# ArthurBrussee/brush

Measured on AMD Instinct MI355X. Metric: train views/sec @ 1M Gaussians, 1080p (fwd + L1/SSIM loss + bwd + Adam per view), higher is better.
Workload: dtype f32

## Files before the change

brush_amd/csrc/api.hip:

```cpp
#include <cmath>
#include <cstdlib>
#include <cstdio>
#include <algorithm>
#include <cstring>
#include <new>

#include "context.h"
#include "device_rng.h"

namespace bh {

int launch_image_loss_forward_strided(bh_ctx* ctx, const float* pred, uint32_t pix_stride, uint32_t ch_stride, const uint32_t* gt,
                                      uint32_t channels, uint32_t h, uint32_t w, const BhLossConfig& cfg, float* loss_map);
int launch_image_loss_backward_strided(bh_ctx* ctx, const float* pred, uint32_t pix_stride, uint32_t ch_stride, const uint32_t* gt,
                                       const float* dl_dmap, float dl_rgb, float dl_alpha, uint32_t channels, uint32_t h, uint32_t w,
                                       const BhLossConfig& cfg, float* dl_dpred);

int launch_image_loss_fused(bh_ctx* ctx, const float* img_hwc4, const uint32_t* gt, uint32_t h, uint32_t w, const BhLossConfig& cfg,
                            bool alpha_match, float dl_rgb, float dl_alpha, float* loss_out, float* v_output, float* loss_host = nullptr,
                            uint32_t* started_host = nullptr, uint32_t started_tag = 0);
int launch_image_loss_fused_window(bh_ctx* ctx, const float* img_hwc4, const uint32_t* gt, uint32_t h, uint32_t w, const BhLossConfig& cfg,
                                   bool alpha_match, float dl_rgb, float dl_alpha, uint32_t tile_y0, uint32_t tile_y1, float* loss_out,
                                   float* v_output, float* loss_host = nullptr, uint32_t* started_host = nullptr, uint32_t started_tag = 0);

// ... 19 lines not shown
}

static inline void cpu_relax() {
#if defined(__x86_64__) || defined(__i386__)
    __builtin_ia32_pause();
#elif defined(__aarch64__)
    __asm__ __volatile__("yield");
#endif
}
int wait_host_tag(bh_ctx* ctx, const volatile uint32_t* word, uint32_t want, const char* what) {
    for (uint64_t it = 1; it < (1ull << 21); ++it) {
        if (*word == want) return 0;
        if ((it & 0x3FFFull) == 0ull) {
            const hipError_t q = hipStreamQuery(ctx->stream);
            if (q == hipSuccess) break;
            if (q != hipErrorNotReady) return check_hip(ctx, q, what);
        }
        cpu_relax();
    }
    if (*word == want) return 0;
    BH_HIP(ctx, hipEventRecord(ctx->readback_ev, ctx->stream));
    BH_HIP(ctx, hipEventSynchronize(ctx->readback_ev));
    if (*word == want) return 0;
    return set_error(ctx, BH_ERR_STATE, std::string(what) + ": the kernel that signals the host never stored its tag");
}

void* ensure(bh_ctx* ctx, Slot s, size_t bytes) {
    Buffer& b = ctx->slots[s];
    if (bytes == 0) bytes = 16;
    if (b.cap >= bytes) return b.ptr;
    if (b.ptr) {
        (void)hipStreamSynchronize(ctx->stream);
        (void)hipFree(b.ptr);
        b.ptr = nullptr;
        b.cap = 0;
    }
    {
        int best = -1;
        for (size_t i = 0; i < ctx->pool.size(); ++i)
            if (ctx->pool[i].cap >= bytes && ctx->pool[i].cap <= 2 * bytes + 4096 && (best < 0 || ctx->pool[i].cap < ctx->pool[(size_t)best].cap)) best = (int)i;
        if (best >= 0) {
            b = ctx->pool[(size_t)best];
            ctx->pool.erase(ctx->pool.begin() + best);
            return b.ptr;
        }
    }
    size_t cap = bytes + bytes / 4;
    cap = (cap + 255) & ~(size_t)255;
    void* p = nullptr;
    hipError_t e = hipMalloc(&p, cap);
    if (e != hipSuccess) {
        (void)hipGetLastError();
        cap = (bytes + 255) & ~(size_t)255;
        e = hipMalloc(&p, cap);
    }
    if (e != hipSuccess) {
        char msg[160];
        snprintf(msg, sizeof msg, "hipMalloc(%zu bytes) for scratch slot %d failed: %s", cap, (int)s, hipGetErrorString(e));
        (void)hipGetLastError();
        set_error(ctx, BH_ERR_OOM, msg);
        return nullptr;
    }
    b.ptr = p;
    b.cap = cap;
    return p;
}

ViewUniforms make_uniforms(const BhCamera& c) {
    ViewUniforms u;
    for (int i = 0; i < 12; ++i) u.vm[i] = c.vm[i];
    u.fx = c.fx; u.fy = c.fy; u.cx = c.cx; u.cy = c.cy;
    u.lim_pos_x = c.lim_pos_x; u.lim_pos_y = c.lim_pos_y; u.lim_neg_x = c.lim_neg_x; u.lim_neg_y = c.lim_neg_y;
    u.cam_x = c.cam_pos[0]; u.cam_y = c.cam_pos[1]; u.cam_z = c.cam_pos[2];
    u.img_w = c.img_w; u.img_h = c.img_h;
    u.tile_bw = (c.img_w + TILE_WIDTH - 1) / TILE_WIDTH;
    u.tile_bh = (c.img_h + TILE_WIDTH - 1) / TILE_WIDTH;
    const bool whole = c.tile_row_begin == 0 && c.tile_row_end == 0;
    u.tile_y0 = whole ? 0u : c.tile_row_begin;
    u.tile_y1 = whole ? u.tile_bh : c.tile_row_end;
    u.model = c.model;
    for (int i = 0; i < 8; ++i) u.dist[i] = c.dist[i];
    u.half_fov = c.half_max_render_fov;
    return u;
}

static int prof_index(Profiler& p, const char* name) {
    for (int i = 0; i < p.count; ++i)
        if (p.names[i] == name || std::strcmp(p.names[i], name) == 0) return i;
    if (p.count >= MAX_PROF) return -1;
    p.names[p.count] = name;
    p.ms[p.count] = 0.0f;
    p.calls[p.count] = 0;
    return p.count++;
}
static hipEvent_t prof_event(Profiler& p) {
    if (!p.pool.empty()) {
        hipEvent_t e = p.pool.back();
        p.pool.pop_back();
        return e;
    }
    hipEvent_t e = nullptr;
    (void)hipEventCreate(&e);
    return e;
}
static void prof_resolve(bh_ctx* ctx) {
    Profiler& p = ctx->prof;
    for (auto& pe : p.pending) {
        (void)hipEventSynchronize(pe.b);
        float ms = 0.0f;
        if (hipEventElapsedTime(&ms, pe.a, pe.b) == hipSuccess && pe.idx >= 0) {
            p.ms[pe.idx] += ms;
            p.calls[pe.idx] += 1;
        }
        p.pool.push_back(pe.a);
        p.pool.push_back(pe.b);
    }
    p.pending.clear();
}

ProfScope::ProfScope(bh_ctx* c, const char* name, bool dominant) : ctx(c) {
    if (c->prof.level == 0 || (c->prof.level == 2 && !dominant)) return;
    idx = prof_index(c->prof, name);
    a = prof_event(c->prof);
    b = prof_event(c->prof);
    if (c->prof.level == 2) {
        c->prof.ext_a = a;
        c->prof.ext_b = b;
        return;
    }
    (void)hipEventRecord(a, c->stream);
}
ProfScope::~ProfScope() {
    if (!a) return;
    if (ctx->prof.level == 2) {
        const bool used = ctx->prof.ext_a == nullptr;
        ctx->prof.ext_a = ctx->prof.ext_b = nullptr;
        if (!used) {
            ctx->prof.pool.push_back(a);
            ctx->prof.pool.push_back(b);
            return;
        }
    } else {
        (void)hipEventRecord(b, ctx->stream);
    }
    ctx->prof.pending.push_back({idx, a, b});
}


}

using namespace bh;

extern "C" {

const char* bh_version(void) { return "brush_hip 0.1 (gfx950)"; }

uint32_t bh_abi_version(void) { return BH_ABI_VERSION; }

uint32_t bh_struct_size(uint32_t which) {
    switch (which) {
        case BH_STRUCT_CAMERA: return (uint32_t)sizeof(BhCamera);
        case BH_STRUCT_RENDER_OUT: return (uint32_t)sizeof(BhRenderOut);
        case BH_STRUCT_LOSS_CONFIG: return (uint32_t)sizeof(BhLossConfig);
        case BH_STRUCT_TRAIN_CONFIG: return (uint32_t)sizeof(BhTrainConfig);
        case BH_STRUCT_TRAIN_STATE: return (uint32_t)sizeof(BhTrainState);
        case BH_STRUCT_TRAIN_BATCH: return (uint32_t)sizeof(BhTrainBatch);
        case BH_STRUCT_TRAIN_STATS: return (uint32_t)sizeof(BhTrainStats);
        case BH_STRUCT_REFINE_CONFIG: return (uint32_t)sizeof(BhRefineConfig);
        case BH_STRUCT_REFINE_STATS: return (uint32_t)sizeof(BhRefineStats);
        case BH_STRUCT_PLY_INFO: return (uint32_t)sizeof(BhPlyInfo);
        default: return 0u;
    }
}

bh_ctx* bh_create(int device, void* stream, int own_stream) {
    bh_ctx* ctx = new (std::nothrow) bh_ctx();
    if (!ctx) return nullptr;
    ctx->device = device;
    if (hipSetDevice(device) != hipSuccess) {
        (void)hipGetLastError();
        delete ctx;
        return nullptr;
    }
    if (!own_stream) {
        ctx->stream = (hipStream_t)stream;
        ctx->owns_stream = false;
    } else {
        if (hipStreamCreateWithFlags(&ctx->stream, hipStreamNonBlocking) != hipSuccess) {
            (void)hipGetLastError();
            delete ctx;
            return nullptr;
        }
        ctx->owns_stream = true;
    }
    if (hipHostMalloc((void**)&ctx->host_counters, bh::HOST_COUNTERS_BYTES, hipHostMallocCoherent)    != hipSuccess) {
        (void)hipGetLastError();
        if (ctx->owns_stream) (void)hipStreamDestroy(ctx->stream);
        delete ctx;
        return nullptr;
    }
    std::memset(ctx->host_counters, 0, bh::HOST_COUNTERS_BYTES);
#ifdef BH_TEST_HOOKS
    ctx->knob_break_allreduce = getenv("BH_BREAK_ALLREDUCE") != nullptr;
    if (ctx->knob_break_allreduce)
        fprintf(stderr, "brush_hip: BH_BREAK_ALLREDUCE is set - every all-reduce of this context's communicator is deliberately CORRUPTED (test hook)\n");
    if (const char* e = getenv("BH_TEST_FAIL_LOSS_AT")) {
        ctx->knob_fail_loss_at = (uint32_t)atoi(e);
        if (ctx->knob_fail_loss_at) fprintf(stderr, "brush_hip: BH_TEST_FAIL_LOSS_AT=%u - that train step of this context will FAIL on purpose (test hook)\n", ctx->knob_fail_loss_at);
    }
#endif
    if (hipEventCreateWithFlags(&ctx->readback_ev, hipEventDisableTiming) != hipSuccess ||
        hipEventCreateWithFlags(&ctx->gate_ev, hipEventDisableTiming) != hipSuccess) {
        if (ctx->readback_ev) (void)hipEventDestroy(ctx->readback_ev);
        (void)hipGetLastError();
        (void)hipHostFree(ctx->host_counters);
        if (ctx->owns_stream) (void)hipStreamDestroy(ctx->stream);
        delete ctx;
        return nullptr;
    }
    return ctx;
}

void bh_destroy(bh_ctx* ctx) {
    if (!ctx) return;
    (void)hipSetDevice(ctx->device);
    (void)hipStreamSynchronize(ctx->stream);
    prof_resolve(ctx);
    for (hipEvent_t e : ctx->prof.pool) (void)hipEventDestroy(e);
    for (auto& b : ctx->slots)
        if (b.ptr) (void)hipFree(b.ptr);
    for (auto& kv : ctx->views)
        if (kv.second.zcut) (void)hipFree(kv.second.zcut);
    for (auto& rt : ctx->retained)
        for (auto& b : rt.blocks)
            if (b.ptr) (void)hipFree(b.ptr);
    for (auto& b : ctx->pool)
        if (b.ptr) (void)hipFree(b.ptr);
    if (ctx->host_counters) (void)hipHostFree(ctx->host_counters);
    if (ctx->dsort_spl) (void)hipFree(ctx->dsort_spl);
    if (ctx->readback_ev) (void)hipEventDestroy(ctx->readback_ev);
    if (ctx->gate_ev) (void)hipEventDestroy(ctx->gate_ev);
    if (ctx->image_tab_host) (void)hipHostFree(ctx->image_tab_host);
    if (ctx->image_tab_ev) (void)hipEventDestroy(ctx->image_tab_ev);
    if (ctx->comm) (void)bh_comm_destroy(ctx);
    if (ctx->owns_stream) (void)hipStreamDestroy(ctx->stream);
    delete ctx;
}

const char* bh_last_error(bh_ctx* ctx) { return ctx ? ctx->last_error.c_str() : "null context"; }

int bh_sync(bh_ctx* ctx) {
    if (!ctx) return BH_ERR_INVALID_ARG;
    if (ctx->far_job.pending) {
        BH_HIP(ctx, hipSetDevice(ctx->device));
        BH_TRY(finish_far_slice(ctx, nullptr));
    }
    BH_HIP(ctx, hipStreamSynchronize(ctx->stream));
    deliver_pending_loss(ctx);
    return 0;
}

int bh_profile_enable(bh_ctx* ctx, int on) {
    if (!ctx) return BH_ERR_INVALID_ARG;
    ctx->prof.level = on < 0 ? 0 : (on > 2 ? 1 : on);
    return 0;
}

int bh_profile_fetch(bh_ctx* ctx, const char** names, float* ms, uint32_t* calls, int cap) {
    if (!ctx) return BH_ERR_INVALID_ARG;
    prof_resolve(ctx);
    Profiler& p = ctx->prof;
    const int n = p.count < cap ? p.count : cap;
    for (int i = 0; i < n; ++i) {
        names[i] = p.names[i];
        ms[i] = p.ms[i];
        calls[i] = p.calls[i];
    }
    p.count = 0;
    return n;
}

namespace {
struct OptionKey { const char* name; const char* help; };
const OptionKey kOptionKeys[] = {
    {"cut_min_pairs", "u32: a view whose last frame had fewer pairs keeps complete lists (= bh_set_list_cut_threshold)"},
    {"cut_margin_pct", "0..10000: base margin behind a tile's last useful splat, % of its depth rank (default 150)"},
    {"cut_margin_fixed", "0|1: the margin is cut_margin_pct for every frame instead of adaptive"},
    {"cut_ctrl", "up:down:floor:gap_exp — the margin controller's constants (default 1.5:0.998:0.5:0.3333)"},
    {"cut_sort_all", "0|1: with per-tile cuts, still depth-sort every visible splat"},
    {"auto_exact_share", "0..1: a view whose last cut frame listed more than this share of its pairs renders complete lists (default 0.9; 0 = never)"},
    {"no_view_hash", "0|1: frames without a view id share ONE table instead of being keyed by their camera"},
    {"k16_order", "0 index order | 1 by the view's last per-tile work | 2 dealt: the forward blend's tile order"},
    {"band_mode", "0|1: XCD bands of the blend kernels — contiguous eighths of the tile range, or dealt in chunks of 8 adjacent tiles (default 1)"},
    {"k16_waves", "0..8: forward blend: resident one-wave tiles per SIMD (0 = 8 = all resident at once; fewer: the lighter tiles are dispatched as the heavier ones finish)"},
    {"k16_split", "0..1000: forward blend: a tile whose forecast work is at least max(256, k16_split / 100 x its band's mean) is blended by four quadrant waves (default 250; 0: no tile is split)"},
    {"k16_split_of_max", "0..100: ... and at least this many percent of its band's heaviest tile (default 45)"},
    {"k16_split_min", "1..1023: a tile below this many blended splats (forecast) is never split (default 256)"},
    {"k5_exact_spw", "16|32|64: splats per wave of the list builder for complete lists"},
    {"bwd_jobs", "0|1: the blend backward works on checkpointed 128-entry segments of the tiles' lists (default 1) or on whole tiles"},
    {"no_lpt", "0|1: the blend backward takes its tiles in index order"},
    {"lpt_classes", "log|linear: work classes of the backward's longest-first tile order — two per octave of blended splats, or 1/64 of the mean list length wide"},
    {"generic_depth_sort", "0|1: depth order by the generic radix sort + scan instead of the fused split sort"},
    {"dsort_splitters", "0|1: the fused depth sort splits at the 254 depth quantiles of the view's previous frame (default 1) or always linearly over the frame's key range"},
    {"tile_sort", "auto|bucket|lsd: the forward's tile sort (auto: bucket sort unless the view's pairs are concentrated in few tiles)"},
    {"spec_k5", "0|1: queue the list builder before the host has read the frame's counts (default 1; 0: behind the count readback)"},
    {"event_waits", "0|1: the host's mid-step waits use events behind the kernels instead of polled tag words"},
    {"readback_copy", "0|1: counts and gate word reach the host through copy launches"},
    {"force_exchange", "0|1: a one-rank communicator still walks the whole gradient-exchange path (overhead measurement)"},
    {"zero_grads", "0|1: the single-GPU train step zero-fills its gradient span like the exchange path"},
    {"loss_bands", "0|1: the fused loss's blocks take their tiles by XCD column bands (1) or row-major (0)"},
    {"update_rows", "0|64|128|256: splats per block of the update kernel (0 = default)"},
    {"update_early", "0|1: the update kernel's blocks issue all their loads up front"},
    {"no_dormant", "0|1: the update kernel fetches and updates dormant splats like everyone else"},
    {"sort_kpt", "0|4|8|16: keys per thread of the generic radix sort (0 = default)"},
    {"grad_allreduce", "ring|direct: the dense gradient block's collective — ncclAllReduce, or reduce-scatter + all-gather over grouped send/recv"},
};
bool parse_u32(const char* v, uint32_t lo, uint32_t hi, uint32_t* out) {
    if (!v || !*v) return false;
    char* end = nullptr;
    const unsigned long long x = strtoull(v, &end, 10);
    if (*end != '\0' || x < lo || x > hi) return false;
    *out = (uint32_t)x;
    return true;
}
bool parse_flag(const char* v, bool* out) {
    uint32_t x = 0;
    if (!parse_u32(v, 0, 1, &x)) return false;
    *out = x != 0;
    return true;
}
}

extern "C" int bh_option_count(void) { return (int)(sizeof(kOptionKeys) / sizeof(kOptionKeys[0])); }
extern "C" const char* bh_option_name(int i) { return i >= 0 && i < bh_option_count() ? kOptionKeys[i].name : nullptr; }
extern "C" const char* bh_option_help(int i) { return i >= 0 && i < bh_option_count() ? kOptionKeys[i].help : nullptr; }

extern "C" int bh_set_option(bh_ctx* ctx, const char* key, const char* value) {
    if (!ctx) return BH_ERR_INVALID_ARG;
    if (!key || !value) return set_error(ctx, BH_ERR_INVALID_ARG, "set_option: null key or value");
    const std::string k(key);
    bool ok = false;
    uint32_t u = 0;
    if (k == "cut_min_pairs") { if ((ok = parse_u32(value, 0, 0xFFFFFFFFu, &u))) ctx->cut_min_pairs = u; }
    else if (k == "cut_margin_pct") { if ((ok = parse_u32(value, 0, 10000, &u))) ctx->knob_cut_margin_pct = u; }
    else if (k == "cut_margin_fixed") ok = parse_flag(value, &ctx->knob_fixed_margin);
    else if (k == "cut_ctrl") {
        float a = 0, b = 0, c = 0, d = 0;
        if (sscanf(value, "%f:%f:%f:%f", &a, &b, &c, &d) == 4 && a >= 1.0f && b > 0.0f && b <= 1.0f && c > 0.0f && d >= 0.0f && d <= 1.0f) {
            ctx->ctrl_up = a; ctx->ctrl_down = b; ctx->ctrl_floor = c; ctx->ctrl_gap_exp = d;
            ok = true;
        }
    }
    else if (k == "cut_sort_all") ok = parse_flag(value, &ctx->knob_cut_sort_all);
    else if (k == "auto_exact_share") {
        char* end = nullptr;
        const float f = strtof(value, &end);
        if (end != value && *end == '\0' && f >= 0.0f && f <= 1.0f) { ctx->auto_exact_share = f; ok = true; }
    }
    else if (k == "no_view_hash") ok = parse_flag(value, &ctx->knob_no_view_hash);
    else if (k == "k16_order") { if ((ok = parse_u32(value, 0, 2, &u))) ctx->knob_k16_order = u; }
    else if (k == "band_mode") { if ((ok = parse_u32(value, 0, 1, &u))) ctx->knob_band_mode = u; }
    else if (k == "k16_waves") { if ((ok = parse_u32(value, 0, 8, &u))) ctx->knob_k16_waves = u; }
    else if (k == "k16_split") { if ((ok = parse_u32(value, 0, 1000, &u))) ctx->knob_k16_split = u; }
    else if (k == "k16_split_of_max") { if ((ok = parse_u32(value, 0, 100, &u))) ctx->knob_k16_split_of_max = u; }
    else if (k == "k16_split_min") { if ((ok = parse_u32(value, 1, 1023, &u))) ctx->knob_k16_split_min = u; }
    else if (k == "k5_exact_spw") { if ((ok = parse_u32(value, 16, 64, &u) && (u == 16 || u == 32 || u == 64))) ctx->knob_k5_exact_spw = u; }
    else if (k == "bwd_jobs") ok = parse_flag(value, &ctx->knob_bwd_jobs);
    else if (k == "no_lpt") ok = parse_flag(value, &ctx->knob_no_lpt);
    else if (k == "lpt_classes") {
        const std::string v(value);
        if (v == "log") { ctx->knob_lpt_linear = false; ok = true; }
        else if (v == "linear") { ctx->knob_lpt_linear = true; ok = true; }
    }
    else if (k == "generic_depth_sort") ok = parse_flag(value, &ctx->knob_generic_depth_sort);
    else if (k == "dsort_splitters") ok = parse_flag(value, &ctx->knob_dsort_splitters);
    else if (k == "tile_sort") {
        const std::string v(value);
        if (v == "auto") { ctx->knob_tile_sort = 0; ok = true; }
        else if (v == "bucket") { ctx->knob_tile_sort = 1; ok = true; }
        else if (v == "lsd") { ctx->knob_tile_sort = 2; ok = true; }
    }
    else if (k == "spec_k5") ok = parse_flag(value, &ctx->knob_spec_k5);
    else if (k == "event_waits") ok = parse_flag(value, &ctx->knob_event_waits);
    else if (k == "readback_copy") ok = parse_flag(value, &ctx->knob_readback_copy);
    else if (k == "force_exchange") ok = parse_flag(value, &ctx->knob_force_exchange);
    else if (k == "zero_grads") ok = parse_flag(value, &ctx->knob_zero_grads);
    else if (k == "loss_bands") { if ((ok = parse_u32(value, 0, 1, &u))) ctx->knob_loss_bands = u; }
    else if (k == "update_rows") { if ((ok = parse_u32(value, 0, 256, &u) && (u == 0 || u == 64 || u == 128 || u == 256))) ctx->knob_update_rows = u; }
    else if (k == "update_early") ok = parse_flag(value, &ctx->knob_update_early);
    else if (k == "no_dormant") ok = parse_flag(value, &ctx->knob_no_dormant);
    else if (k == "sort_kpt") { if ((ok = parse_u32(value, 0, 16, &u) && (u == 0 || u == 4 || u == 8 || u == 16))) ctx->knob_sort_kpt = u; }
    else if (k == "grad_allreduce") {
        const std::string v(value);
        if (v == "ring") { ctx->knob_direct_allreduce = false; ok = true; }
        else if (v == "direct") { ctx->knob_direct_allreduce = true; ok = true; }
    }
    else return set_error(ctx, BH_ERR_INVALID_ARG, "set_option: unknown key '" + k + "' (bh_option_name lists the keys)");
    if (!ok) return set_error(ctx, BH_ERR_INVALID_ARG, "set_option: bad value '" + std::string(value) + "' for '" + k + "'");
    return 0;
}

namespace {
struct Kb4Law {
    double k[4];
    explicit Kb4Law(const float* d) { for (int i = 0; i < 4; ++i) k[i] = d ? (double)d[i] : 0.0; }
    double value(double th) const {
        const double t2 = th * th, t3 = t2 * th, t5 = t3 * t2, t7 = t5 * t2, t9 = t7 * t2;
        return th + k[0] * t3 + k[1] * t5 + k[2] * t7 + k[3] * t9;
    }
    double slope(double th) const {
        const double t2 = th * th, t4 = t2 * t2, t6 = t4 * t2, t8 = t6 * t2;
        return 1.0 + 3.0 * k[0] * t2 + 5.0 * k[1] * t4 + 7.0 * k[2] * t6 + 9.0 * k[3] * t8;
    }
    double invert(double target) const {
        if (target <= 0.0) return 0.0;
        const double pi = 3.14159265358979323846;
        double th = target < pi - 1e-6 ? target : pi - 1e-6;
        for (int it = 0; it < 50; ++it) {
            const double fp = slope(th);
            if (std::fabs(fp) < 1e-12) break;
            double next = th - (value(th) - target) / fp;
            next = next < 0.0 ? 0.0 : (next > pi ? pi : next);
            const bool done = std::fabs(next - th) < 1e-12;
            th = next;
            if (done) break;
        }
        return th;
    }
};
struct Rt8Law {
    double k[6];
    explicit Rt8Law(const float* d) { for (int i = 0; i < 6; ++i) k[i] = d ? (double)d[i] : 0.0; }
    double radial(double r) const {
        const double r2 = r * r, r4 = r2 * r2, r6 = r4 * r2;
        return (1.0 + k[0] * r2 + k[1] * r4 + k[2] * r6) / (1.0 + k[3] * r2 + k[4] * r4 + k[5] * r6);
    }
    double undistort(double r_d) const {
        double r = r_d;
        for (int it = 0; it < 30; ++it) {
            const double f = radial(r);
            if (std::fabs(f) < 1e-12) break;
            const double rn = r_d / f;
            const bool done = std::fabs(rn - r) < 1e-12;
            r = rn;
            if (done) break;
        }
        return r;
    }
};
}

double bh_fov_to_focal(double fov, uint32_t pixels, uint32_t model, const float* dist) {
    const double half = fov / 2.0, r_pix = (double)pixels / 2.0;
    switch (model) {
        case BH_CAMERA_PINHOLE: return r_pix / std::tan(half);
        case BH_CAMERA_KANNALA_BRANDT_4:
        case BH_CAMERA_THIN_PRISM_FISHEYE: return r_pix / Kb4Law(dist).value(half);
        case BH_CAMERA_RADIAL_TANGENTIAL_8: { const double r = std::tan(half); return r_pix / (r * Rt8Law(dist).radial(r)); }
        default: return std::nan("");
    }
}

double bh_focal_to_fov(double focal, uint32_t pixels, uint32_t model, const float* dist) {
    const double r_norm = ((double)pixels / 2.0) / focal;
    switch (model) {
        case BH_CAMERA_PINHOLE: return 2.0 * std::atan(r_norm);
        case BH_CAMERA_KANNALA_BRANDT_4:
        case BH_CAMERA_THIN_PRISM_FISHEYE: return 2.0 * Kb4Law(dist).invert(r_norm);
        case BH_CAMERA_RADIAL_TANGENTIAL_8: return 2.0 * std::atan(Rt8Law(dist).undistort(r_norm));
        default: return std::nan("");
    }
}

int bh_camera_setup_model(const float* pos, const float* rot_xyzw, double fov_x, double fov_y, float center_u, float center_v,
                          uint32_t img_w, uint32_t img_h, uint32_t model, const float* dist, BhCamera* out) {
    if (!pos || !rot_xyzw || !out || img_w == 0 || img_h == 0 || model > BH_CAMERA_THIN_PRISM_FISHEYE) return BH_ERR_INVALID_ARG;
    const float x = rot_xyzw[0], y = rot_xyzw[1], z = rot_xyzw[2], w = rot_xyzw[3];
    const float x2 = x + x, y2 = y + y, z2 = z + z;
    const float xx = x * x2, xy = x * y2, xz = x * z2;
    const float yy = y * y2, yz = y * z2, zz = z * z2;
    const float wx = w * x2, wy = w * y2, wz = w * z2;
    const float ax[3] = {1.0f - (yy + zz), xy + wz, xz - wy};
    const float ay[3] = {xy - wz, 1.0f - (xx + zz), yz + wx};
    const float az[3] = {xz + wy, yz - wx, 1.0f - (xx + yy)};
    auto cross = [](const float* a, const float* b, float* o) {
        o[0] = a[1] * b[2] - b[1] * a[2];
        o[1] = a[2] * b[0] - b[2] * a[0];
        o[2] = a[0] * b[1] - b[0] * a[1];
    };
    float t0[3], t1[3], t2[3];
    cross(ay, az, t0);
    cross(az, ax, t1);
    cross(ax, ay, t2);
    const float det = (az[0] * t2[0]) + (az[1] * t2[1]) + (az[2] * t2[2]);
    const float inv_det = 1.0f / det;
    float r0[3], r1[3], r2[3];
    for (int i = 0; i < 3; ++i) { r0[i] = t0[i] * inv_det; r1[i] = t1[i] * inv_det; r2[i] = t2[i] * inv_det; }
    const float c0[3] = {r0[0], r1[0], r2[0]}, c1[3] = {r0[1], r1[1], r2[1]}, c2[3] = {r0[2], r1[2], r2[2]};
    for (int i = 0; i < 3; ++i) {
        out->vm[i] = c0[i];
        out->vm[3 + i] = c1[i];
        out->vm[6 + i] = c2[i];
        const float ip = (c0[i] * pos[0] + c1[i] * pos[1]) + c2[i] * pos[2];
        out->vm[9 + i] = -ip;
    }
    out->model = model;
    for (int i = 0; i < 8; ++i) out->dist[i] = (model != BH_CAMERA_PINHOLE && dist) ? dist[i] : 0.0f;
    out->fx = (float)bh_fov_to_focal(fov_x, img_w, model, out->dist);
    out->fy = (float)bh_fov_to_focal(fov_y, img_h, model, out->dist);
    out->cx = center_u * (float)img_w;
    out->cy = center_v * (float)img_h;
    const float wf = (float)img_w, hf = (float)img_h;
    float lim[4] = {(1.15f * wf - out->cx) / out->fx, (1.15f * hf - out->cy) / out->fy,
                    (-0.15f * wf - out->cx) / out->fx, (-0.15f * hf - out->cy) / out->fy};
    if (model == BH_CAMERA_RADIAL_TANGENTIAL_8) {
        const Rt8Law law(out->dist);
        for (float& e : lim) {
            const float mag = (float)law.undistort(std::fabs((double)e));
            e = (e != e) ? e : (std::signbit(e) ? -mag : mag);
        }
    } else if (model != BH_CAMERA_PINHOLE) {
        for (float& e : lim) e = 0.0f;
    }
    out->lim_pos_x = lim[0]; out->lim_pos_y = lim[1]; out->lim_neg_x = lim[2]; out->lim_neg_y = lim[3];
    const float full = hypotf((float)fov_x, (float)fov_y) * 1.05f;
    const float cap = 2.0f * 3.14159265358979323846f - 1e-6f;
    out->half_max_render_fov = (full < cap ? full : cap) * 0.5f;
    out->cam_pos[0] = pos[0]; out->cam_pos[1] = pos[1]; out->cam_pos[2] = pos[2];
    out->img_w = img_w;
    out->img_h = img_h;
    out->tile_row_begin = 0;
    out->tile_row_end = 0;
    return 0;
}

int bh_camera_setup(const float* pos, const float* rot_xyzw, double fov_x, double fov_y, float center_u, float center_v,
                    uint32_t img_w, uint32_t img_h, BhCamera* out) {
    return bh_camera_setup_model(pos, rot_xyzw, fov_x, fov_y, center_u, center_v, img_w, img_h, BH_CAMERA_PINHOLE, nullptr, out);
}

}

static int render_forward(bh_ctx* ctx, const ForwardRequest& req, BhRenderOut* out) {
    const BhCamera& cam = req.cam;
    if (cam.img_w == 0 || cam.img_h == 0) return set_error(ctx, BH_ERR_INVALID_ARG, "Can't render images with 0 size.");
    if (req.sh_degree > 4) return set_error(ctx, BH_ERR_INVALID_ARG, "sh_degree must be 0..4");
    if (cam.model > BH_CAMERA_THIN_PRISM_FISHEYE) return set_error(ctx, BH_ERR_INVALID_ARG, "unknown camera model");
    if (cam.img_w > 65520 || cam.img_h > 65520) return set_error(ctx, BH_ERR_UNSUPPORTED, "images larger than 65520 px per side are not supported (tile grid <= 4095 x 4095)");
    if (req.n > 0 && (!req.transforms || !req.sh_coeffs || !req.raw_opacities)) return set_error(ctx, BH_ERR_INVALID_ARG, "render_forward: null splat tensor");
    if ((req.flags & BH_FLAG_SMOOTH_CUTOFF) && !(req.flags & BH_FLAG_BWD_INFO)) return set_error(ctx, BH_ERR_INVALID_ARG, "smooth cutoff requires the backward pass flag");
    BH_HIP(ctx, hipSetDevice(ctx->device));
    if (ctx->far_job.pending) BH_TRY(finish_far_slice(ctx, nullptr));
    return forward_impl(ctx, req, out);
}

extern "C" int bh_render_forward(bh_ctx* ctx, const BhCamera* cam, uint32_t n, uint32_t sh_degree, const float* transforms,
                                 const float* sh_coeffs, const float* raw_opacities, const float* background, uint32_t flags,
                                 BhRenderOut* out) {
    if (!ctx) return BH_ERR_INVALID_ARG;
    if (!cam || !out || !background) return set_error(ctx, BH_ERR_INVALID_ARG, "render_forward: null argument");
    ForwardRequest req;
    req.cam = *cam;
    req.n = n; req.sh_degree = sh_degree; req.flags = flags;
    req.transforms = transforms; req.sh_coeffs = sh_coeffs; req.raw_opacities = raw_opacities;
    req.bg[0] = background[0]; req.bg[1] = background[1]; req.bg[2] = background[2];
    req.view_id = ctx->view_id;
    return render_forward(ctx, req, out);
}

int bh::forward_impl(bh_ctx* ctx, const ForwardRequest& req, BhRenderOut* out) {
    const uint32_t n = req.n, sh_degree = req.sh_degree, flags = req.flags;
    const float* transforms = req.transforms;
    const float* sh_coeffs = req.sh_coeffs;
    const float* raw_opacities = req.raw_opacities;
    const float* background = req.bg;
    ctx->have_forward = false;
    ctx->clears.begin_forward();
    const bool mip = flags & BH_FLAG_MIP, bwd_info = flags & BH_FLAG_BWD_INFO, smooth = flags & BH_FLAG_SMOOTH_CUTOFF;
    const ViewUniforms u = make_uniforms(req.cam);
    if (u.tile_y0 >= u.tile_y1 || u.tile_y1 > u.tile_bh) return set_error(ctx, BH_ERR_INVALID_ARG, "tile_row window must satisfy begin < end <= ceil(img_h / 16)");
    const uint32_t num_tiles = u.tile_bw * u.tile_bh;
    const size_t npad = n ? n : 1;

    constexpr size_t counter_set_bytes = COUNTER_SET_BYTES, counter_set_words = COUNTER_SET_BYTES / 4, counter_read_bytes = COUNTER_READ_BYTES;
    auto* counter_pairs = (uint32_t*)ensure(ctx, SLOT_COUNTERS, 2 * counter_set_bytes + 64);
    uint32_t* dev_sums = counter_pairs ? counter_pairs + 2 * counter_set_words : nullptr;
    uint32_t* counters = counter_pairs ? counter_pairs + counter_set_words * (ctx->counter_phase & 1u) : nullptr;
    auto* depth_keys = (uint32_t*)ensure(ctx, SLOT_DEPTH_KEYS, npad * 4);
    auto* isect_counts = (uint32_t*)ensure(ctx, SLOT_ISECT_COUNTS, npad * 4);
    auto* max_radius = req.max_radius ? req.max_radius : (float*)ensure(ctx, SLOT_MAX_RADIUS, npad * 4);
    auto* proj_by_gid = (float*)ensure(ctx, SLOT_PROJECTED_BY_GID, npad * 9 * 4);
    if (!counters || !depth_keys || !isect_counts || !max_radius || !proj_by_gid) return BH_ERR_OOM;

    auto* gfc = (uint32_t*)ensure(ctx, SLOT_GLOBAL_FROM_COMPACT, npad * 4);
    auto* depths_sorted = (uint32_t*)ensure(ctx, SLOT_DEPTHS_SORTED, npad * 4);
    if (!gfc || !depths_sorted) return BH_ERR_OOM;
    const bool bwd_jobs = bwd_info && ctx->knob_bwd_jobs && !ctx->knob_no_lpt && !((flags & BH_FLAG_SLICED_LISTS) && ctx->slice_fraction > 0.0f);
    const size_t lpt_words = LPT_HEADER_WORDS + (size_t)8 * LPT_CLASSES * band_slots(num_tiles);
    auto* tile_offsets = (uint32_t*)ensure(ctx, SLOT_TILE_OFFSETS, ((size_t)num_tiles * 2 + lpt_words) * 4);
    auto* visible = (bwd_info && req.visible) ? req.visible : (float*)ensure(ctx, SLOT_VISIBLE, (bwd_info ? npad : 1) * 4);
    if (!tile_offsets || !visible) return BH_ERR_OOM;
    const size_t visible_words = bwd_info ? ((req.visible && req.visible_floats) ? req.visible_floats : npad) : 0;
    const bool want_sliced = (flags & BH_FLAG_SLICED_LISTS) != 0;
    const size_t slice_bit_words = ((size_t)num_tiles + 31) / 32;
    const size_t slice_group_words = (size_t)n / (256 * FAR_GROUP_BLOCKS) + 2;
    const size_t slice_words = want_sliced ? SLICE_CTRL_WORDS + slice_bit_words + (size_t)num_tiles * 2 + slice_group_words : 0;
    uint32_t* slice_tab = nullptr;
    if (want_sliced) {
        slice_tab = (uint32_t*)ensure(ctx, SLOT_SLICE, slice_words * 4);
        if (!slice_tab) return BH_ERR_OOM;
    }
    ViewState* view = nullptr;
    bool cut_active = false;
    const bool auto_cuts = want_sliced && !(ctx->slice_fraction > 0.0f);
    const bool order_only = !want_sliced && ctx->knob_k16_order != 0u && n >= 8u * 256u;
    if (n > 0 && (auto_cuts || order_only)) {
        view = frame_view(ctx, req, u.tile_bw, u.tile_bh, order_only && !bwd_info);
        if (!view && auto_cuts) return set_error(ctx, BH_ERR_OOM, "hipMalloc for the per-view tile table failed");
        if (!view) (void)hipGetLastError();
        cut_active = auto_cuts && view && cut_this_frame(ctx, view, req.allow_cut);
    }
    uint32_t* const vtab = view_table(view);
    uint32_t* near_counts = nullptr;
    uint32_t* tile_order = nullptr;
    uint32_t* tile_split = nullptr;
    if (cut_active) {
        near_counts = (uint32_t*)ensure(ctx, SLOT_NEAR_COUNTS, npad * 4);
        if (!near_counts) return BH_ERR_OOM;
    }

    uint32_t nv = 0, ni = 0, near_total = 0, nv_true = 0;
    bool fused_scan = false;
    uint32_t* cum_early = nullptr;
    bool k5_queued = false;
    uint32_t spec_pair_cap = 0;
    float* spec_projected = nullptr;
    float4* spec_vc = nullptr;
    uint32_t *spec_tile_ids = nullptr, *spec_isect_gids = nullptr;
    if (n > 0) {
        {
            ProfScope ps(ctx, "ProjectSplats");
            if (!ctx->counters_ready) BH_HIP(ctx, hipMemsetAsync(counter_pairs, 0, 2 * counter_set_bytes, ctx->stream));
            ctx->counters_ready = false;
            ForwardPrep prep;
            prep.next_counters = reinterpret_cast<unsigned long long*>(counter_pairs + counter_set_words * ((ctx->counter_phase & 1u) ^ 1u));
            prep.visible = visible_words ? reinterpret_cast<uint32_t*>(visible) : nullptr;
            prep.visible_words = (uint32_t)visible_words;
            prep.tile_table = tile_offsets;
            prep.tile_words = num_tiles * 2 + LPT_HEADER_WORDS;
            prep.slice_table = slice_tab;
            prep.slice_words = (uint32_t)slice_words;
            prep.list_all_visible = ctx->knob_cut_sort_all;
            if (view && ctx->knob_k16_order && n >= 8u * 256u) {
                const uint32_t win_t = u.tile_bw * (u.tile_y1 - u.tile_y0);
                tile_order = (uint32_t*)ensure(ctx, SLOT_TILE_ORDER, ((size_t)8 * band_slots(win_t) + SPLIT_TAIL_WORDS) * 4);
                if (!tile_order) return BH_ERR_OOM;
                prep.order_work = vtab + (size_t)num_tiles;
                prep.order_out = tile_order;
                prep.order_tiles = win_t;
                prep.order_tile_begin = u.tile_bw * u.tile_y0;
                prep.order_mode = ctx->knob_k16_order;
                prep.band_mode = ctx->knob_band_mode;
                if (ctx->knob_k16_split && ctx->knob_k16_order == 1u) {
                    tile_split = tile_order + (size_t)8 * band_slots(win_t);
                    prep.split_out = tile_split;
                    prep.split_factor = (float)ctx->knob_k16_split * 0.01f;
                    prep.split_min = ctx->knob_k16_split_min;
                    prep.split_of_max = (float)ctx->knob_k16_split_of_max * 0.01f;
                }
            }
            if (bwd_info && req.grad_begin && req.grad_floats && (req.grad_floats & 3u) == 0 &&
                (reinterpret_cast<uintptr_t>(req.grad_begin) & 15u) == 0 && req.grad_floats / 4 <= 0xFFFFFFFFull) {
                prep.span = reinterpret_cast<float4*>(req.grad_begin);
                prep.span_f4 = (uint32_t)(req.grad_floats / 4);
                ctx->clears.k1_cleared_span();
            }
            BH_TRY(launch_project_forward(ctx, u, n, mip, sh_degree, transforms, sh_coeffs, raw_opacities, depth_keys, isect_counts, max_radius,
                                          proj_by_gid, counters, prep, cut_active ? vtab : nullptr, near_counts));
            ctx->counter_phase ^= 1u;
            ctx->counters_ready = true;
        }
        auto* hslots = reinterpret_cast<unsigned long long*>(ctx->host_counters + 16);
        fused_scan = depth_sort_supported(n) && !ctx->knob_generic_depth_sort;
        const bool sums_on_device = fused_scan && !ctx->knob_readback_copy;
        const bool poll_tag = sums_on_device && !ctx->knob_event_waits;
        if (!sums_on_device) {
            BH_HIP(ctx, hipMemcpyAsync(hslots, counters, counter_read_bytes, hipMemcpyDeviceToHost, ctx->stream));
            BH_HIP(ctx, hipEventRecord(ctx->readback_ev, ctx->stream));
        }
        {
            ProfScope ps(ctx, "DepthSort");
            if (fused_scan) {
                cum_early = (uint32_t*)ensure(ctx, SLOT_CUM_TILES_HIT, npad * 4);
                if (!cum_early) return BH_ERR_OOM;
                if (poll_tag && ++ctx->readback_tag == 0u) ctx->readback_tag = 1u;
                bool* spl_written = nullptr;
                uint32_t* spl = view_splitters(view, cut_active, &spl_written);
                BH_TRY(depth_sort_scan(ctx, depth_keys, counters + COUNTER_MINMAX_WORD, cut_active ? near_counts : isect_counts, n, depths_sorted, gfc, cum_early,
                                       sums_on_device ? counters : nullptr, ctx->host_counters + 16, ctx->readback_ev, poll_tag ? ctx->readback_tag : 0u,
                                       sums_on_device ? dev_sums : nullptr, spl, spl_written));
            } else {
                BH_TRY(radix_argsort(ctx, depth_keys, nullptr, n, 32, depths_sorted, gfc));
            }
        }
        if (poll_tag && ctx->knob_spec_k5 && !(want_sliced && ctx->slice_fraction > 0.0f)) {
            const size_t cap_pairs = std::min(ctx->slots[SLOT_TILE_IDS].cap, ctx->slots[SLOT_ISECT_GIDS].cap) / 4;
            if (cap_pairs >= 4096) {
                spec_projected = (float*)ensure(ctx, SLOT_PROJECTED, npad * 9 * 4);
                spec_vc = bwd_info ? (float4*)ensure(ctx, SLOT_V_COMBINED, npad * 10 * 4 + 16) : nullptr;
                if (!spec_projected || (bwd_info && !spec_vc)) return BH_ERR_OOM;
                spec_tile_ids = (uint32_t*)ctx->slots[SLOT_TILE_IDS].ptr;
                spec_isect_gids = (uint32_t*)ctx->slots[SLOT_ISECT_GIDS].ptr;
                spec_pair_cap = (uint32_t)std::min<size_t>(cap_pairs, 0xFFFFFFFEull);
                ProfScope ps(ctx, "MapGaussiansToIntersect");
                BH_TRY(launch_map_gaussians(ctx, n, u, proj_by_gid, gfc, spec_projected, cum_early, spec_tile_ids, spec_isect_gids, spec_vc,
                                            spec_vc ? (uint32_t)(((size_t)n * 10 + 3) / 4) : 0u, 0xFFFFFFFFu, cut_active ? slice_tab : nullptr,
                                            cut_active ? vtab : nullptr, cut_active ? depths_sorted : nullptr, dev_sums + (cut_active ? 3 : 0), spec_pair_cap));
                k5_queued = true;
            }
        }
        if (poll_tag) BH_TRY(wait_host_tag(ctx, reinterpret_cast<const volatile uint32_t*>(hslots) + HOST_SUM_WORDS - 1u, ctx->readback_tag, "count readback"));
        else BH_HIP(ctx, hipEventSynchronize(ctx->readback_ev));
        if (ctx->gate_learn) {
            ctx->gate_learn = false;
            ctx->far_direct = reinterpret_cast<const volatile uint32_t*>(ctx->host_counters)[HOST_GATE_WORD] != 0u;
        }
        unsigned long long hc[4] = {0ull, 0ull, 0ull, 0ull};
        if (sums_on_device) {
            const volatile unsigned long long* hs = hslots;
            for (uint32_t c = 0; c < COUNTER_K1_U64; ++c) hc[c] = hs[c];
        } else {
            for (uint32_t k = 0; k < COUNTER_SLOTS; ++k)
                for (uint32_t c = 0; c < COUNTER_K1_U64; ++c) hc[c] += hslots[COUNTER_K1_U64 * k + c];
        }
        if (hc[1] > 0xFFFFFFFFull) return set_error(ctx, BH_ERR_UNSUPPORTED, "more than 2^32-1 tile intersections");
        nv_true = (uint32_t)hc[0];
        ni = (uint32_t)hc[1];
        near_total = cut_active ? (uint32_t)hc[2] : ni;
        nv = cut_active ? (uint32_t)hc[3] : nv_true;
    } else {
        BH_HIP(ctx, hipMemsetAsync(tile_offsets, 0, ((size_t)num_tiles * 2 + LPT_HEADER_WORDS) * 4, ctx->stream));
        if (visible_words) BH_HIP(ctx, hipMemsetAsync(visible, 0, visible_words * 4, ctx->stream));
    }

    const size_t nvpad = nv ? nv : 1, nipad = ni ? ni : 1;
    auto* cum = fused_scan ? cum_early : (uint32_t*)ensure(ctx, SLOT_CUM_TILES_HIT, nvpad * 4);
    auto* projected = (float*)ensure(ctx, SLOT_PROJECTED, nvpad * 9 * 4);
    auto* tile_ids = (uint32_t*)ensure(ctx, SLOT_TILE_IDS, nipad * 4);
    auto* isect_gids = (uint32_t*)ensure(ctx, SLOT_ISECT_GIDS, nipad * 4);
    auto* tile_ids_sorted = (uint32_t*)ensure(ctx, SLOT_TILE_IDS_SORTED, nipad * 4);
    auto* isect_gids_sorted = (uint32_t*)ensure(ctx, SLOT_ISECT_GIDS_SORTED, nipad * 4);
    const size_t pixels = (size_t)u.img_w * u.img_h;
    void* out_img = ensure(ctx, SLOT_OUT_IMG, pixels * (bwd_info ? 16 : 4));
    if (!cum || !projected || !tile_ids || !isect_gids || !tile_ids_sorted || !isect_gids_sorted || !out_img)
        return BH_ERR_OOM;
    if (k5_queued && ((cut_active ? near_total : ni) > spec_pair_cap || projected != spec_projected || tile_ids != spec_tile_ids || isect_gids != spec_isect_gids))
        k5_queued = false;

    const uint32_t budget = want_sliced && ni > 0 ? list_budget(ctx, cut_active ? view : nullptr, near_total, ni) : ni;
    const bool sliced = budget < ni;
    const bool by_cut = cut_active && sliced;
    const uint32_t* zcut_lists = cut_active ? vtab : nullptr;
    uint32_t* slice_info = slice_tab;
    uint32_t* done_bits = slice_tab ? slice_tab + SLICE_CTRL_WORDS : nullptr;
    uint32_t* tile_offsets_far = slice_tab ? slice_tab + SLICE_CTRL_WORDS + slice_bit_words : nullptr;
    uint32_t* far_group_totals = slice_tab ? slice_tab + SLICE_CTRL_WORDS + slice_bit_words + (size_t)num_tiles * 2 : nullptr;
    uint32_t tile_bits = 0;
    while (tile_bits < 32 && (num_tiles >> tile_bits) != 0) tile_bits++;
    RasterSlice rs;
    ctx->jobs = BwdJobs{};
    if (bwd_jobs) {
        const uint32_t listed = cut_active ? near_total : ni;
        const uint32_t ckpt_cap = (uint32_t)std::min<uint64_t>((uint64_t)listed / BWD_SEG + num_tiles + 1u, BWD_CKPT_MAX_SLOTS);
        rs.jobs.ckpt = (float4*)ensure(ctx, SLOT_BWD_CKPT, (size_t)ckpt_cap * 256 * sizeof(float4));
        rs.jobs.ckpt_cap = ckpt_cap;
        rs.jobs.top_cap = band_slots(num_tiles) + ckpt_cap;
        rs.jobs.top_list = (uint32_t*)ensure(ctx, SLOT_BWD_TOPLIST, (size_t)8 * rs.jobs.top_cap * 4);
        if (!rs.jobs.ckpt || !rs.jobs.top_list) return BH_ERR_OOM;
        ctx->jobs = rs.jobs;
    }
    if (view) {
        rs.zcut = vtab;
        rs.depth_keys_sorted = depths_sorted;
        rs.nv = nv;
        rs.cut_active = by_cut;
        rs.margin_pct = cut_margin_pct(ctx, view);
        rs.work = vtab + (size_t)num_tiles;
        rs.order = tile_order;
        rs.order_mode = ctx->knob_k16_order;
        rs.split = tile_split;
#ifdef BH_TEST_HOOKS
        ctx->last_split = tile_split;
#endif
    }
    const uint32_t win_tiles = u.tile_bw * (u.tile_y1 - u.tile_y0);
    const float class_width_raw = (float)ni / (float)(win_tiles ? win_tiles : 1u) / 64.0f;
    const float class_width = ctx->knob_lpt_linear ? (class_width_raw < 8.0f ? 8.0f : class_width_raw) : 0.0f;
    ctx->lpt = (bwd_info && !ctx->knob_no_lpt) ? tile_offsets + (size_t)num_tiles * 2 : nullptr;
    float* out_f32 = bwd_info ? (float*)out_img : nullptr;
    uint32_t* out_u8 = bwd_info ? nullptr : (uint32_t*)out_img;

    bool offsets_done = false;
    if (nv > 0) {
        if (!fused_scan) {
            ProfScope ps(ctx, "PrefixSumGaussHits");
            BH_TRY(prefix_sum(ctx, cut_active ? near_counts : isect_counts, gfc, nv, cum, false));
        }
        if (ni == 0) {
            ProfScope ps(ctx, "ProjectVisible");
            BH_TRY(launch_project_visible(ctx, nv, proj_by_gid, gfc, projected));
        }
        if (ni > 0) {
            {
                ProfScope ps(ctx, "MapGaussiansToIntersect");
                float4* vc = nullptr;
                if (bwd_info) {
                    vc = (float4*)ensure(ctx, SLOT_V_COMBINED, (size_t)nv * 10 * 4 + 16);
                    if (!vc) return BH_ERR_OOM;
                }
                if (zcut_lists && near_total == 0u) {
                } else if (k5_queued && (!bwd_info || vc == spec_vc)) {
                    ctx->clears.k5_cleared_accum(vc != nullptr);
                } else {
                    ctx->clears.k5_cleared_accum(vc != nullptr);
                    BH_TRY(launch_map_gaussians(ctx, nv, u, proj_by_gid, gfc, projected, cum, tile_ids, isect_gids, vc, vc ? (uint32_t)(((size_t)nv * 10 + 3) / 4) : 0u,
                                                (sliced && !by_cut) ? budget : 0xFFFFFFFFu, (sliced || zcut_lists) ? slice_info : nullptr, zcut_lists,
                                                zcut_lists ? depths_sorted : nullptr));
                }
            }
            {
                ProfScope ps(ctx, "TileSort");
                if ((zcut_lists || !sliced) && tile_sort_supported(tile_bits, zcut_lists ? near_total : ni) && !(ctx->knob_tile_sort == 2u)) {
                    BH_TRY(tile_sort_offsets(ctx, tile_ids, isect_gids, zcut_lists ? near_total : ni, tile_bits, num_tiles, tile_ids_sorted, isect_gids_sorted,
                                             tile_offsets, ni));
                    offsets_done = true;
                } else
                if (zcut_lists) BH_TRY(radix_argsort_dev(ctx, tile_ids, isect_gids, near_total, nullptr, nullptr, nullptr, tile_bits, tile_ids_sorted, isect_gids_sorted, ni));
                else if (sliced) BH_TRY(radix_argsort_dev(ctx, tile_ids, isect_gids, budget, slice_info + 1, nullptr, nullptr, tile_bits, tile_ids_sorted, isect_gids_sorted, ni));
                else BH_TRY(radix_argsort(ctx, tile_ids, isect_gids, ni, tile_bits, tile_ids_sorted, isect_gids_sorted));
            }
        }
    }
    if (!offsets_done) {
        ProfScope ps(ctx, "GetTileOffsets");
        if (zcut_lists) BH_TRY(launch_tile_offsets(ctx, tile_ids_sorted, near_total, num_tiles, tile_offsets, true));
        else if (sliced) BH_TRY(launch_tile_offsets_dev(ctx, tile_ids_sorted, budget, slice_info + 1, nullptr, nullptr, num_tiles, tile_offsets));
        else BH_TRY(launch_tile_offsets(ctx, tile_ids_sorted, ni, num_tiles, tile_offsets, true));
    }
    if (!sliced) {
        ProfScope ps(ctx, "Rasterize");
        BH_TRY(launch_rasterize(ctx, u, background, bwd_info, smooth, isect_gids_sorted, tile_offsets, projected, gfc, out_f32, out_u8, visible, ctx->lpt,
                                class_width, 0, &rs));
    } else {
        auto* state = (float*)ensure(ctx, SLOT_SLICE_STATE, pixels * 16);
        auto* far_counts = (uint32_t*)ensure(ctx, SLOT_SLICE_COUNTS, nvpad * 4);
        auto* far_block_totals = (uint32_t*)ensure(ctx, SLOT_SLICE_CUM, (nvpad / 256 + 2) * 4);
        if (!state || !far_counts || !far_block_totals) return BH_ERR_OOM;
        rs.done_bits = done_bits;
        rs.unsat_count = slice_info + 2;
        if (!ctx->knob_readback_copy) {
            rs.gate_host = ctx->host_counters + HOST_GATE_WORD;
            *reinterpret_cast<volatile uint32_t*>(rs.gate_host) = 0u;
        }
        rs.state = state;
        rs.offsets_near = tile_offsets;
        rs.live_bands = slice_info + 4;
        {
            ProfScope ps(ctx, "Rasterize");
            BH_TRY(launch_rasterize(ctx, u, background, bwd_info, smooth, isect_gids_sorted, tile_offsets, projected, gfc, out_f32, out_u8, visible, ctx->lpt,
                                    class_width, 1, &rs));
        }
        FarJob& j = ctx->far_job;
        j.u = u;
        j.bg[0] = background[0]; j.bg[1] = background[1]; j.bg[2] = background[2];
        j.bwd_info = bwd_info; j.smooth = smooth;
        j.nv = nv; j.ni = ni; j.budget = budget; j.num_tiles = num_tiles; j.tile_bits = tile_bits;
        j.proj_by_gid = proj_by_gid; j.gfc = gfc; j.projected = projected; j.cum = cum;
        j.slice_info = slice_info; j.done_bits = done_bits; j.tile_offsets_far = tile_offsets_far;
        j.far_counts = far_counts; j.far_block_totals = far_block_totals; j.far_group_totals = far_group_totals;
        j.tile_ids = tile_ids; j.isect_gids = isect_gids; j.tile_ids_sorted = tile_ids_sorted; j.isect_gids_sorted = isect_gids_sorted;
        j.out_f32 = out_f32; j.out_u8 = out_u8; j.visible = visible; j.lpt = ctx->lpt; j.class_width = class_width; j.rs = rs;
        j.by_cut = by_cut;
        j.view = by_cut ? view : nullptr;
        j.view_shared = req.view_id == 0u && ctx->knob_no_view_hash;
        if (by_cut) j.req = req;
        if (ctx->knob_readback_copy)
            BH_HIP(ctx, hipMemcpyAsync(ctx->host_counters + HOST_GATE_WORD, slice_info + 2, 4, hipMemcpyDeviceToHost, ctx->stream));
        if (ctx->far_direct && !by_cut) {
            BH_TRY(enqueue_far_slice(ctx, j));
            ctx->gate_learn = true;
        } else {
            if (++ctx->gate_tag == 0u) ctx->gate_tag = 1u;
            j.gate_tag = ctx->gate_tag;
            ctx->gate_signal_queued = false;
            j.gate_event_recorded = !(req.defer_decision && !ctx->knob_event_waits && !ctx->knob_readback_copy);
            if (j.gate_event_recorded) BH_HIP(ctx, hipEventRecord(ctx->gate_ev, ctx->stream));
            j.pending = true;
            if (!req.defer_decision) {
                bool again = false;
                BH_TRY(finish_far_slice(ctx, &again));
                if (by_cut && again) {
                    *out = ctx->last;
                    return 0;
                }
            }
        }
    }

    BhRenderOut r{};
    r.num_visible = nv_true;
    r.num_listed_splats = nv;
    r.num_intersections = ni;
    r.num_tiles = num_tiles;
    r.tile_bw = u.tile_bw;
    r.tile_bh = u.tile_bh;
    r.flags = flags;
    r.out_img = bwd_info ? (float*)out_img : nullptr;
    r.out_img_packed = bwd_info ? nullptr : (uint32_t*)out_img;
    r.visible = bwd_info ? visible : nullptr;
    r.max_radius = max_radius;
    r.tile_offsets = tile_offsets;
    r.projected = projected;
    r.compact_gid_from_isect = isect_gids_sorted;
    r.tile_id_from_isect = tile_ids_sorted;
    r.global_from_compact_gid = gfc;
    r.cum_tiles_hit = cum;
    r.intersect_counts = isect_counts;
    r.depths_sorted = (float*)depths_sorted;
    r.tile_offsets_far = sliced ? tile_offsets_far : nullptr;
    r.list_budget = budget;
    r.generation = ++ctx->generation;
    ctx->clears.stamp(r.generation);
    *out = r;
    ctx->last = r;
    ctx->last_listed_splats = nv;
    ctx->cam = req.cam;
    ctx->uniforms = u;
    ctx->n = n;
    ctx->sh_degree = sh_degree;
    ctx->flags = flags;
    ctx->bg[0] = background[0]; ctx->bg[1] = background[1]; ctx->bg[2] = background[2];
    ctx->have_forward = true;
    if (view) view_rendered(view, ni);
    return 0;
}

extern "C" {

int bh_set_list_slicing(bh_ctx* ctx, float near_share) {
    if (!ctx) return BH_ERR_INVALID_ARG;
    if (near_share != near_share || near_share > 1.0f) return set_error(ctx, BH_ERR_INVALID_ARG, "set_list_slicing: the near slice's share must be <= 1 (<= 0: automatic)");
    ctx->slice_fraction = near_share > 0.0f ? near_share : 0.0f;
    return 0;
}

int bh_set_list_cut_threshold(bh_ctx* ctx, uint32_t min_pairs) {
    if (!ctx) return BH_ERR_INVALID_ARG;
    ctx->cut_min_pairs = min_pairs;
    return 0;
}

int bh_set_view_id(bh_ctx* ctx, uint32_t view_id) {
    if (!ctx) return BH_ERR_INVALID_ARG;
    ctx->view_id = view_id;
    return 0;
}

int bh_forget_views(bh_ctx* ctx) {
    if (!ctx) return BH_ERR_INVALID_ARG;
    BH_HIP(ctx, hipSetDevice(ctx->device));
    if (ctx->far_job.pending) BH_TRY(finish_far_slice(ctx, nullptr));
    if (ctx->dsort_spl) { BH_HIP(ctx, hipMemsetAsync(ctx->dsort_spl, 0, DSORT_SPL_STRIDE * 4, ctx->stream)); ctx->dsort_spl_written = false; }
    if (ctx->views.empty()) return 0;
    BH_HIP(ctx, hipStreamSynchronize(ctx->stream));
    deliver_pending_loss(ctx);
    for (auto& kv : ctx->views)
        if (kv.second.zcut) (void)hipFree(kv.second.zcut);
    ctx->views.clear();
    ctx->casual_views = 0;
    for (uint64_t& k : ctx->seen_keys) k = 0ull;
    ctx->far_job.view = nullptr;
    ctx->margin_scale = 1.0f;
    return 0;
}

float bh_last_list_share(bh_ctx* ctx) { return ctx ? ctx->last_slice_share : 0.0f; }
uint32_t bh_far_slices_queued(bh_ctx* ctx) { return ctx ? ctx->far_launches : 0u; }
uint32_t bh_view_table_count(bh_ctx* ctx) { return ctx ? (uint32_t)ctx->views.size() : 0u; }

}

namespace bh {

static ForwardState latest_forward(const bh_ctx* ctx) {
    ForwardState fs;
    fs.out = ctx->last;
    fs.uniforms = ctx->uniforms;
    fs.n = ctx->n; fs.sh_degree = ctx->sh_degree; fs.flags = ctx->flags;
    fs.bg[0] = ctx->bg[0]; fs.bg[1] = ctx->bg[1]; fs.bg[2] = ctx->bg[2];
    fs.lpt = ctx->lpt;
    fs.jobs = ctx->jobs;
    return fs;
}

int backward_impl(bh_ctx* ctx, const ForwardState& fs, const float* v_output, const float* transforms, const float* sh_coeffs,
                  const float* raw_opacities, float* v_transforms, float* v_sh_coeffs, float* v_raw_opacities, float* v_refine_weight,
                  size_t span_floats, bool want_refine, const DepthTerm* depth) {
    const BhRenderOut& r = fs.out;
    const uint32_t n = fs.n, nv = r.num_listed_splats, C = (fs.sh_degree + 1) * (fs.sh_degree + 1);
    const size_t nvpad = nv ? nv : 1;
    auto* v_combined = (float*)ensure(ctx, SLOT_V_COMBINED, nvpad * 10 * 4 + 16);
    if (!v_combined) return BH_ERR_OOM;
    bool row_marks = false;
    {
        ProfScope ps(ctx, "ZeroGradBuffers");
        const bool one_span = n > 0 && span_floats;
        const bool vc_done = ctx->clears.take_accum(r.generation);
        const GradClears::Span span = ctx->clears.take_span(r.generation);
        row_marks = span == GradClears::ROW_MARKS;
        if (row_marks && !one_span) return set_error(ctx, BH_ERR_STATE, "internal: row-marked gradients without the train step's gradient span");
        const bool span_done = one_span && span != GradClears::NONE;
        if (one_span && (span_floats & 3u) == 0 && (reinterpret_cast<uintptr_t>(v_transforms) & 15u) == 0) {
            const size_t na = vc_done ? 0 : (nvpad * 10 + 3) / 4, nb = span_done ? 0 : span_floats / 4;
            if (na + nb) {
                hipLaunchKernelGGL(zero_two_kernel, dim3(2048), dim3(256), 0, ctx->stream, reinterpret_cast<float4*>(v_combined), na,
                                   reinterpret_cast<float4*>(v_transforms), nb);
                BH_LAUNCH_CHECK(ctx, "zero_two_kernel");
            }
        } else {
            if (!vc_done) BH_HIP(ctx, hipMemsetAsync(v_combined, 0, nvpad * 10 * 4, ctx->stream));
            if (n > 0) {
                if (one_span) {
                    BH_HIP(ctx, hipMemsetAsync(v_transforms, 0, span_floats * 4, ctx->stream));
                } else {
                    BH_HIP(ctx, hipMemsetAsync(v_transforms, 0, (size_t)n * 10 * 4, ctx->stream));
                    BH_HIP(ctx, hipMemsetAsync(v_sh_coeffs, 0, (size_t)n * C * 3 * 4, ctx->stream));
                    BH_HIP(ctx, hipMemsetAsync(v_raw_opacities, 0, (size_t)n * 4, ctx->stream));
                    BH_HIP(ctx, hipMemsetAsync(v_refine_weight, 0, (size_t)n * 4, ctx->stream));
                }
            }
        }
    }
// ... 527 lines not shown
```

brush_amd/csrc/context.h:

```cpp
#pragma once
#include <hip/hip_runtime.h>
#include <stdint.h>

#include <memory>
#include <string>
#include <unordered_map>
#include <vector>

#include "../../include/brush_hip.h"
#include "../../include/brush_hip_lpips.h"
#include "../../include/brush_hip_image.h"
#include "device_math.h"

namespace bh {

enum Slot : int {
    SLOT_COUNTERS = 0,
    SLOT_DEPTH_KEYS,
    SLOT_ISECT_COUNTS,
    SLOT_MAX_RADIUS,
    SLOT_SORT_KEYS_A,
    SLOT_SORT_KEYS_B,
    SLOT_SORT_VALS_A,
    SLOT_SORT_VALS_B,
    SLOT_SORT_HIST,
    SLOT_COMM_SCRATCH,
    SLOT_BWD_CKPT,
    SLOT_BWD_TOPLIST,
    SLOT_SORT_PARTS,
    SLOT_SCAN_SUMS,
    SLOT_GLOBAL_FROM_COMPACT,
    SLOT_DEPTHS_SORTED,
    SLOT_CUM_TILES_HIT,
    SLOT_PROJECTED,
    SLOT_TILE_IDS,
    SLOT_ISECT_GIDS,
    SLOT_TILE_IDS_SORTED,
    SLOT_ISECT_GIDS_SORTED,
    SLOT_TILE_OFFSETS,
    SLOT_OUT_IMG,
    SLOT_VISIBLE,
    SLOT_V_COMBINED,
    SLOT_LOSS_PRED,
    SLOT_LOSS_MAP,
    SLOT_LOSS_GRAD,
    SLOT_V_OUTPUT,
    SLOT_GRADS,
    SLOT_STATS,
    SLOT_LOSS_SCALAR,
    SLOT_COL_SCALE,
    SLOT_MISC,
    SLOT_REFINE,
    SLOT_REFINE_BOUNDS,
    SLOT_FOLDED_TRANSFORMS,
    SLOT_FOLDED_RAW_OPAC,
    SLOT_PLY_ROWS,
    SLOT_EXCH_BLOCKS,
    SLOT_EXCH_IDX,
    SLOT_EXCH_COMPACT,
    SLOT_PROJECTED_BY_GID,
    SLOT_SLICE,
    SLOT_SLICE_STATE,
    SLOT_SLICE_COUNTS,
    SLOT_SLICE_CUM,
    SLOT_NEAR_COUNTS,
    SLOT_TILE_ORDER,
    SLOT_LOD_GRADS,
    SLOT_LOD_FOLDED,
    SLOT_LOD_LOSS,
    SLOT_LOD_SORT,
    SLOT_KNN,
    SLOT_EVAL,
    SLOT_LPIPS,
    SLOT_PLY_COMPRESS,
    SLOT_IMAGE,
    SLOT_DEPTH,
    SLOT_COUNT
};

struct Buffer {
    void* ptr = nullptr;
    size_t cap = 0;
};

constexpr int MAX_PROF = 32;

constexpr uint32_t COUNTER_SLOTS = 128;
constexpr uint32_t COUNTER_K1_U64 = 4;
constexpr size_t COUNTER_SET_BYTES = COUNTER_SLOTS * 8 * COUNTER_K1_U64 + COUNTER_SLOTS * 8;
constexpr uint32_t COUNTER_SET_U64 = (uint32_t)(COUNTER_SET_BYTES / 8);
constexpr uint32_t COUNTER_MINMAX_WORD = COUNTER_SLOTS * 2 * COUNTER_K1_U64;
constexpr uint32_t SLICE_CTRL_WORDS = 8;
constexpr uint32_t FAR_GROUP_BLOCKS = 64;
constexpr size_t COUNTER_READ_BYTES = COUNTER_SLOTS * 8 * COUNTER_K1_U64;
constexpr uint32_t HOST_SUM_WORDS = 2 * COUNTER_K1_U64 + 1;
constexpr size_t HOST_LOSS_WORD = 16 + COUNTER_READ_BYTES / 4;
constexpr size_t HOST_GATE_WORD = HOST_LOSS_WORD + 16;
constexpr size_t HOST_GATE_TAG_WORD = HOST_GATE_WORD + 1;
constexpr size_t HOST_COUNTERS_BYTES = 64 + COUNTER_READ_BYTES + 64 + 64;

struct Profiler {
    int level = 0;
    const char* names[MAX_PROF];
    float ms[MAX_PROF];
    uint32_t calls[MAX_PROF];
    int count = 0;
    struct Pending { int idx; hipEvent_t a, b; };
    std::vector<Pending> pending;
    std::vector<hipEvent_t> pool;
    hipEvent_t ext_a = nullptr, ext_b = nullptr;
};

constexpr uint32_t ZCUT_ALL = 0xFFFFFFFEu;
BH_DEV bool zcut_near(uint32_t key, uint32_t cut) { return (key >> 1) <= (cut >> 1); }
struct ViewState {
    uint32_t* zcut = nullptr;
    uint32_t tile_bw = 0, tile_bh = 0;
    bool seeded = false;
    uint32_t exact_frames = 0;
    uint32_t penalty = 0;
    uint64_t last_used = 0;
    uint32_t gap = 0;
    uint32_t last_pairs = 0;
    uint32_t complete_frames = 0;
    bool spl_written[2] = {false, false};
    bool casual = false;
};
constexpr uint32_t CUT_MIN_PAIRS = 1500000u;
constexpr uint32_t LPT_CLASSES = 64;
constexpr uint32_t LPT_HEADER_WORDS = 8 * LPT_CLASSES + 64;
constexpr uint32_t BWD_SEG = 128;
constexpr uint32_t BWD_MAX_SEGS = 64;
struct BwdJobs {
    float4* ckpt = nullptr;
    uint32_t ckpt_cap = 0;
    uint32_t* top_list = nullptr;
    uint32_t top_cap = 0;
};
constexpr uint32_t BAND_CHUNK = 4;
inline __host__ __device__ uint32_t band_slots(uint32_t num_tiles) {
    const uint32_t p = (num_tiles + 7u) / 8u;
    return ((p + BAND_CHUNK - 1u) / BAND_CHUNK) * BAND_CHUNK;
}
inline __host__ __device__ uint32_t band_tile(uint32_t band, uint32_t i, uint32_t per, uint32_t mode) {
    return mode ? ((i / BAND_CHUNK) * 8u + band) * BAND_CHUNK + (i % BAND_CHUNK) : band * per + i;
}
constexpr uint32_t SPLIT_MAX = 128;
constexpr uint32_t SPLIT_MIN_WORK = 256;
constexpr uint32_t SPLIT_TAIL_WORDS = 8u + 8u * SPLIT_MAX * 4u;
constexpr uint32_t BWD_CKPT_MAX_SLOTS = 96u * 1024u;
constexpr uint32_t DSORT_SPL_STRIDE = 260;
constexpr uint32_t VIEW_SPL_WORDS = 2 * DSORT_SPL_STRIDE;
constexpr size_t MAX_VIEW_STATES = 4096;
constexpr uint64_t DIRECT_ALLREDUCE_MIN_FLOATS = 1u << 16;
constexpr uint32_t AUTO_EXACT_FRAMES = 12;
constexpr size_t CASUAL_VIEW_STATES = 32;
constexpr size_t SEEN_KEYS = 64;
constexpr size_t VIEW_TABLE_BYTES = (size_t)256 << 20;

struct RasterSlice {
    uint32_t* done_bits = nullptr;
    uint32_t* unsat_count = nullptr;
    uint32_t* gate_host = nullptr;
    float* state = nullptr;
    const uint32_t* offsets_near = nullptr;
    uint32_t* zcut = nullptr;
    const uint32_t* depth_keys_sorted = nullptr;
    uint32_t nv = 0;
    bool cut_active = false;
    uint32_t* live_bands = nullptr;
    uint32_t* work = nullptr;
    const uint32_t* order = nullptr;
    uint32_t order_mode = 1;
    uint32_t* split = nullptr;
    uint32_t margin_pct = 150;
    BwdJobs jobs{};
};

struct ForwardRequest {
    BhCamera cam{};
    uint32_t n = 0, sh_degree = 0, flags = 0;
    const float* transforms = nullptr;
    const float* sh_coeffs = nullptr;
    const float* raw_opacities = nullptr;
    float bg[3] = {0, 0, 0};
    uint32_t view_id = 0;
    float* visible = nullptr;
    float* max_radius = nullptr;
    size_t visible_floats = 0;
    float* grad_begin = nullptr;
    size_t grad_floats = 0;
    bool defer_decision = false;
    bool allow_cut = true;
};

struct FarJob {
    bool pending = false;
    ViewUniforms u{};
    float bg[3] = {0, 0, 0};
    bool bwd_info = false, smooth = false;
    uint32_t nv = 0, ni = 0, budget = 0, num_tiles = 0, tile_bits = 0;
    const float* proj_by_gid = nullptr;
    const uint32_t* gfc = nullptr;
    float* projected = nullptr;
    const uint32_t* cum = nullptr;
    uint32_t* slice_info = nullptr;
    uint32_t* done_bits = nullptr;
    uint32_t* tile_offsets_far = nullptr;
    uint32_t* far_counts = nullptr;
    uint32_t* far_block_totals = nullptr;
    uint32_t* far_group_totals = nullptr;
    uint32_t* tile_ids = nullptr;
    uint32_t* isect_gids = nullptr;
    uint32_t* tile_ids_sorted = nullptr;
    uint32_t* isect_gids_sorted = nullptr;
    float* out_f32 = nullptr;
    uint32_t* out_u8 = nullptr;
    float* visible = nullptr;
    uint32_t* lpt = nullptr;
    float class_width = 8.0f;
    RasterSlice rs{};
    bool gate_event_recorded = false;
    uint32_t gate_tag = 0;
    bool by_cut = false;
    ViewState* view = nullptr;
    bool view_shared = false;
    ForwardRequest req{};
};

struct GradClears {
    enum Span : uint8_t { NONE = 0, ZEROED, ROW_MARKS };
    Span span = NONE;
    bool accum = false;
    uint64_t generation = 0;
    void begin_forward() { span = NONE; accum = false; generation = 0; }
    void k1_cleared_span() { span = ZEROED; }
    void k5_cleared_accum(bool yes) { accum = yes; }
    void stamp(uint64_t gen) { generation = gen; }
    void mark_rows() { span = ROW_MARKS; }
    bool valid_for(uint64_t gen) const { return generation != 0 && generation == gen; }
    Span take_span(uint64_t gen) { const Span s = valid_for(gen) ? span : NONE; span = NONE; return s; }
    bool take_accum(uint64_t gen) { const bool a = valid_for(gen) && accum; accum = false; return a; }
};

struct ForwardState {
    BhRenderOut out{};
    ViewUniforms uniforms{};
    uint32_t n = 0, sh_degree = 0, flags = 0;
    float bg[3] = {0, 0, 0};
    uint32_t* lpt = nullptr;
    BwdJobs jobs{};
};
constexpr int RETAIN_SLOTS = 14;
struct Retained {
    ForwardState fs;
    Buffer blocks[RETAIN_SLOTS];
};

struct DepthTerm {
    const float* v_depth = nullptr;
    uint32_t mode = 0;
};

}


struct bh_ctx {
    int device = 0;
    hipStream_t stream = nullptr;
    bool owns_stream = false;
    std::string last_error;
    bh::Buffer slots[bh::SLOT_COUNT];
    uint32_t* host_counters = nullptr;
    hipEvent_t readback_ev = nullptr;
    hipEvent_t gate_ev = nullptr;
    bool counters_ready = false;
    uint32_t counter_phase = 0;
    bool have_forward = false;
    BhCamera cam{};
    bh::ViewUniforms uniforms{};
    uint32_t n = 0, sh_degree = 0, flags = 0;
    float bg[3] = {0, 0, 0};
    BhRenderOut last{};
    uint64_t generation = 0;
    std::vector<bh::Retained> retained;
    std::vector<bh::Buffer> pool;
    bh::GradClears clears;
    float* pending_loss_dst = nullptr;
    void* image_tab_host = nullptr;
    size_t image_tab_cap = 0;
    hipEvent_t image_tab_ev = nullptr;
    const bh_lpips* lpips = nullptr;
    float lpips_weight = 0.0f;
    void* comm = nullptr;
    hipStream_t comm_stream = nullptr;
    hipEvent_t comm_ev = nullptr;
    int comm_rank = 0, comm_world = 1;
    uint32_t* lpt = nullptr;
    float slice_fraction = 0.0f;
    float last_slice_share = 1.0f;
    bool far_direct = false;
    uint32_t readback_tag = 0;
    uint32_t gate_tag = 0;
    bool gate_signal_queued = false;
    bool gate_learn = false;
    uint32_t far_launches = 0;
    uint32_t last_listed_splats = 0;
    std::unordered_map<uint64_t, bh::ViewState> views;
    uint64_t seen_keys[bh::SEEN_KEYS] = {};
    uint32_t seen_pos = 0;
    uint32_t casual_views = 0;
    uint32_t view_id = 0;
    uint64_t view_clock = 0;
    float margin_scale = 1.0f;
    float ctrl_up = 1.5f, ctrl_down = 0.998f, ctrl_floor = 0.5f, ctrl_gap_exp = 1.0f / 3.0f;
    uint32_t cut_min_pairs = bh::CUT_MIN_PAIRS;
    bool knob_spec_k5 = true;
    bool knob_event_waits = false;
    bool knob_readback_copy = false;
    bool knob_no_view_hash = false;
    bool knob_fixed_margin = false;
    bool knob_cut_sort_all = false;
    uint32_t knob_band_mode = 1;
    uint32_t knob_k16_waves = 0;
    uint32_t knob_k16_split = 250;
    uint32_t knob_k16_split_min = bh::SPLIT_MIN_WORK;
    uint32_t knob_k16_split_of_max = 45;
    const uint32_t* last_split = nullptr;
    uint32_t knob_k16_order = 1;
    uint32_t knob_cut_margin_pct = 150;
    bh::FarJob far_job;
    uint32_t refine_n = 0, refine_new_n = 0;
    bool dsort_lds_raised = false;
    uint32_t* dsort_spl = nullptr;
    bool dsort_spl_written = false;
    bool knob_dsort_splitters = true;
    bool adam_lds_raised = false;
    bool knob_no_lpt = false;
    bool knob_bwd_jobs = true;
    bh::BwdJobs jobs{};
    bool knob_lpt_linear = false;
    bool knob_force_exchange = false;
    bool knob_break_allreduce = false;
    bool knob_generic_depth_sort = false;
    bool knob_zero_grads = false;
    uint32_t knob_fail_loss_at = 0;
    uint32_t train_steps_seen = 0;
    uint32_t knob_loss_bands = 1;
    uint32_t knob_tile_sort = 0;
    float auto_exact_share = 0.9f;
    bool knob_direct_allreduce = false;
    uint32_t knob_k5_exact_spw = 32;
    bool knob_no_dormant = false;
    bool knob_update_early = false;
    uint32_t knob_update_rows = 0;
    uint32_t knob_sort_kpt = 0;
    const void* marks_m2_sh = nullptr; const void* marks_m1_t = nullptr; uint32_t marks_n = 0, marks_step = 0;
    bh::Profiler prof;
};

namespace bh {

int set_error(bh_ctx* ctx, int code, const std::string& msg);
int forward_impl(bh_ctx* ctx, const ForwardRequest& req, BhRenderOut* out);
int wait_host_tag(bh_ctx* ctx, const volatile uint32_t* word, uint32_t want, const char* what);
int find_saved_forward(bh_ctx* ctx, const BhRenderOut* saved, const char* who, ForwardState* latest, const ForwardState** fs);
int backward_impl(bh_ctx* ctx, const ForwardState& fs, const float* v_output, const float* transforms, const float* sh_coeffs,
                  const float* raw_opacities, float* v_transforms, float* v_sh_coeffs, float* v_raw_opacities, float* v_refine_weight,
                  size_t span_floats, bool want_refine, const DepthTerm* depth = nullptr);
int launch_depth_backward(bh_ctx* ctx, const ForwardState& fs, const DepthTerm& term, float* v_combined);
int launch_depth_vz_scatter(bh_ctx* ctx, const ForwardState& fs, float* v_transforms);

ViewState* frame_view(bh_ctx* ctx, const ForwardRequest& req, uint32_t tile_bw, uint32_t tile_bh, bool casual);
bool cut_this_frame(const bh_ctx* ctx, ViewState* vs, bool allow_cut);
uint32_t* view_table(const ViewState* vs);
uint32_t* view_splitters(ViewState* vs, bool cut, bool** written);
uint32_t cut_margin_pct(const bh_ctx* ctx, const ViewState* vs);
uint32_t list_budget(bh_ctx* ctx, ViewState* cut_view, uint32_t near_total, uint32_t ni);
void view_rendered(ViewState* vs, uint32_t ni);
int enqueue_far_slice(bh_ctx* ctx, const FarJob& j);
int finish_far_slice(bh_ctx* ctx, bool* launched);
bool far_job_decides_first(const bh_ctx* ctx);
void drop_far_job(bh_ctx* ctx);
inline void deliver_pending_loss(bh_ctx* ctx) {
    if (ctx->pending_loss_dst) {
        *ctx->pending_loss_dst = reinterpret_cast<const volatile float*>(ctx->host_counters)[HOST_LOSS_WORD];
        ctx->pending_loss_dst = nullptr;
    }
}
int check_hip(bh_ctx* ctx, hipError_t e, const char* what);
int lpips_train_term(bh_ctx* ctx, const float* img_hwc4, const uint32_t* gt_packed, uint32_t h, uint32_t w, const float* bg, float* v_output,
                     float* loss, float* loss_host);
std::string ply_header_comments(uint32_t sh_degree, bool render_mip, const float* up_axis);
enum ResizeOut : int { RESIZE_OUT_U8 = 0, RESIZE_OUT_PACKED = 1, RESIZE_OUT_PACKED_PREMUL = 2 };
size_t resize_table_bytes(uint32_t src, uint32_t dst, uint32_t filter);
void build_resize_table(uint32_t src, uint32_t dst, uint32_t filter, void* host);
using ResizeTable = std::shared_ptr<const std::vector<uint8_t>>;
ResizeTable resize_table(uint32_t src, uint32_t dst, uint32_t filter);
hipError_t enqueue_resize(hipStream_t st, const uint8_t* src, uint32_t w, uint32_t h, uint32_t channels, uint32_t nw, uint32_t nh,
                          const int32_t* vtab, const int32_t* htab, float* tmp, void* out, int mode);
hipError_t enqueue_mask_merge(hipStream_t st, const uint8_t* img, uint32_t channels, const uint8_t* mask, uint64_t pixels, int invert,
                              int premultiply, uint32_t* out);
void* ensure(bh_ctx* ctx, Slot s, size_t bytes);

struct ProfScope {
    bh_ctx* ctx;
    int idx = -1;
    hipEvent_t a = nullptr, b = nullptr;
    ProfScope(bh_ctx* c, const char* name, bool dominant = false);
    ~ProfScope();
};

#define BH_HIP(ctx, expr)                                            \
    do {                                                             \
        hipError_t _e = (expr);                                      \
        if (_e != hipSuccess) return bh::check_hip(ctx, _e, #expr);  \
    } while (0)
#define BH_TRY(expr)            \
    do {                        \
        int _rc = (expr);       \
        if (_rc != 0) return _rc; \
    } while (0)
#define BH_LAUNCH_CHECK(ctx, what)                                      \
    do {                                                                \
        hipError_t _e = hipGetLastError();                              \
        if (_e != hipSuccess) return bh::check_hip(ctx, _e, what);      \
    } while (0)

ViewUniforms make_uniforms(const BhCamera& c);


struct ForwardPrep {
    unsigned long long* next_counters = nullptr;
    uint32_t* visible = nullptr;
    uint32_t visible_words = 0;
    uint32_t* tile_table = nullptr;
    uint32_t tile_words = 0;
    float4* span = nullptr;
    uint32_t span_f4 = 0;
    uint32_t* slice_table = nullptr;
    uint32_t slice_words = 0;
    const uint32_t* order_work = nullptr;
    uint32_t* order_out = nullptr;
    uint32_t order_tiles = 0, order_tile_begin = 0;
    uint32_t order_mode = 1;
    uint32_t band_mode = 0;
    uint32_t* split_out = nullptr;
    float split_factor = 2.5f;
    uint32_t split_min = SPLIT_MIN_WORK;
    float split_of_max = 0.45f;
    bool list_all_visible = false;
};
int launch_project_forward(bh_ctx* ctx, const ViewUniforms& u, uint32_t n, bool mip, uint32_t sh_degree, const float* transforms,
                           const float* sh, const float* raw_opac, uint32_t* depth_keys, uint32_t* isect_counts, float* max_radius,
                           float* projected_by_gid, uint32_t* counters, const ForwardPrep& prep, uint32_t* zcut = nullptr,
                           uint32_t* near_counts = nullptr);
int launch_project_visible(bh_ctx* ctx, uint32_t nv, const float* projected_by_gid, const uint32_t* gid, float* projected);
int launch_map_gaussians(bh_ctx* ctx, uint32_t nv, const ViewUniforms& u, const float* projected_by_gid, const uint32_t* gid,
                         float* projected, const uint32_t* cum_tiles_hit, uint32_t* tile_ids, uint32_t* isect_gids,
                         float4* zero_span = nullptr, uint32_t zero_f4 = 0, uint32_t budget = 0xFFFFFFFFu, uint32_t* slice_info = nullptr,
                         const uint32_t* zcut = nullptr, const uint32_t* depth_keys_sorted = nullptr, const uint32_t* nv_dev = nullptr, uint32_t pair_cap = 0xFFFFFFFFu);
int launch_map_gaussians_far(bh_ctx* ctx, uint32_t nv, const ViewUniforms& u, const float* projected_by_gid, const uint32_t* gid,
                             float* projected, const uint32_t* cum_tiles_hit, uint32_t budget, const uint32_t* done_bits, const uint32_t* gate,
                             uint32_t* counts, uint32_t* block_totals, uint32_t* group_totals, uint32_t* slice_info, uint32_t* tile_ids, uint32_t* isect_gids);
int launch_project_backward(bh_ctx* ctx, const ViewUniforms& u, uint32_t nv, bool mip, uint32_t sh_degree,
                            const float* transforms, const float* sh, const float* raw_opac, const uint32_t* gid,
                            float* v_combined, float* v_transforms, float* v_sh, float* v_raw_opac,
                            float* v_refine, bool mark_written = false, const float* projected = nullptr);
int radix_argsort(bh_ctx* ctx, const uint32_t* keys, const uint32_t* vals, uint32_t n, uint32_t bits,
                  uint32_t* out_keys, uint32_t* out_vals);
int radix_argsort_dev(bh_ctx* ctx, const uint32_t* keys, const uint32_t* vals, uint32_t n_max, const uint32_t* n_dev, const uint32_t* gate,
                      const uint32_t* out_base, uint32_t bits, uint32_t* out_keys, uint32_t* out_vals, uint32_t alloc_n = 0);
bool tile_sort_supported(uint32_t bits, uint32_t n);
int tile_sort_offsets(bh_ctx* ctx, const uint32_t* keys, const uint32_t* vals, uint32_t n, uint32_t bits, uint32_t num_tiles,
                      uint32_t* out_keys, uint32_t* out_vals, uint32_t* tile_offsets, uint32_t alloc_n = 0);
bool depth_sort_supported(uint32_t n);
int depth_sort_scan(bh_ctx* ctx, const uint32_t* keys, const uint32_t* minmax, const uint32_t* counts, uint32_t n, uint32_t* out_keys,
                    uint32_t* out_vals, uint32_t* cum, const uint32_t* rb_set = nullptr, uint32_t* rb_host = nullptr, hipEvent_t rb_done = nullptr,
                    uint32_t rb_tag = 0, uint32_t* rb_dev = nullptr, uint32_t* spl = nullptr, bool* spl_written = nullptr);
int prefix_sum(bh_ctx* ctx, const uint32_t* in, const uint32_t* gather, uint32_t n, uint32_t* out, bool exclusive, const uint32_t* gate = nullptr);
int launch_tile_offsets(bh_ctx* ctx, const uint32_t* tile_ids_sorted, uint32_t num_isect, uint32_t num_tiles,
                        uint32_t* tile_offsets, bool pre_zeroed = false);
int launch_tile_offsets_dev(bh_ctx* ctx, const uint32_t* tile_ids_sorted, uint32_t n_max, const uint32_t* n_dev, const uint32_t* gate,
                            const uint32_t* base, uint32_t num_tiles, uint32_t* tile_offsets);

int launch_rasterize(bh_ctx* ctx, const ViewUniforms& u, const float bg[3], bool bwd_info, bool smooth,
                     const uint32_t* isect_gids, uint32_t* tile_offsets, const float* projected,
                     const uint32_t* global_from_compact, float* out_img, uint32_t* out_packed, float* visible,
                     uint32_t* lpt, float class_width, int phase = 0, const RasterSlice* slice = nullptr);
int launch_rasterize_backward(bh_ctx* ctx, const ViewUniforms& u, const float bg[3], bool smooth,
                              const uint32_t* isect_gids, const uint32_t* tile_offsets, const float* projected,
                              const float* out_img, const float* v_output, float* v_combined, const uint32_t* lpt,
                              const uint32_t* tile_offsets_far = nullptr, bool want_refine = true, const BwdJobs* jobs = nullptr);
int launch_image_loss_forward(bh_ctx* ctx, const float* pred, const uint32_t* gt, uint32_t channels, uint32_t h,
                              uint32_t w, const BhLossConfig& cfg, float* loss_map);
int launch_image_loss_backward(bh_ctx* ctx, const float* pred, const uint32_t* gt, const float* dl_dmap,
                               float dl_const, uint32_t channels, uint32_t h, uint32_t w, const BhLossConfig& cfg,
                               float* dl_dpred);
int launch_hwc4_to_chw(bh_ctx* ctx, const float* img_hwc4, uint32_t channels, uint32_t h, uint32_t w, float* chw);
int launch_chw_to_hwc4(bh_ctx* ctx, const float* chw, uint32_t channels, uint32_t h, uint32_t w, float* hwc4);
int launch_sum(bh_ctx* ctx, const float* x, uint64_t n, float scale, float* out_scalar, bool accumulate);
int launch_adam(bh_ctx* ctx, float* param, const float* grad, float* m1, float* m2, uint64_t rows, uint32_t row_len,
                const float* col_scale, float lr, uint32_t t, bool reduce_m2, float beta1, float beta2, float eps);
struct NoiseArgs { uint64_t seed; uint32_t step; float scale, clamp_abs; };
int launch_train_update(bh_ctx* ctx, const BhTrainState* st, const float* g_t, const float* g_sh, const float* g_o,
                        const float* refine_weight, const float* visible, const float* screen_radius, float gscale,
                        bool vis_clamp, const float* tab_t, float lr_sh, float sh_rest_scale, float lr_opac, uint32_t t,
                        float beta1, float beta2, float eps, const NoiseArgs* noise = nullptr, bool masked_rows = false);
int launch_gather_stats(bh_ctx* ctx, float* refine_weight_norm, float* vis_weight, float* max_screen_size,
                        const float* refine_weight, const float* visible, const float* screen_radius, uint64_t n);
int launch_mean_noise(bh_ctx* ctx, float* transforms, const float* raw_opac, const float* visible,
                      const float* samples, uint64_t n, float noise_scale, float clamp_abs, uint64_t seed = 0, uint32_t step = 0);
int launch_normal_samples(bh_ctx* ctx, float* out, uint64_t n, uint64_t seed, uint32_t step);

int launch_fold_min_scale(bh_ctx* ctx, const float* transforms, const float* raw_opac, const float* min_scale, uint32_t n,
                          float* out_transforms, float* out_raw_opac);
int launch_fold_min_scale_backward(bh_ctx* ctx, const float* transforms, const float* raw_opac, const float* min_scale, uint32_t n,
                                   float* v_transforms, float* v_raw_opac);
int launch_compute_min_scale(bh_ctx* ctx, const float* transforms, uint32_t n, const float* view_cams, uint32_t k, float factor, float* out);

int comm_allreduce(bh_ctx* ctx, float* buf, uint64_t count, bool max_op);
int comm_exchange_strip_halos(bh_ctx* ctx, float* img, uint32_t h, uint32_t w, uint32_t row_begin_px, uint32_t row_end_px);

int launch_union_index(bh_ctx* ctx, const float* visible_sum, uint32_t n, uint32_t* block_scratch , uint32_t* count_dev,
                       uint32_t* idx);
int launch_exchange_rows(bh_ctx* ctx, bool gather, const uint32_t* idx, uint32_t count, uint32_t c3, float* g_tr, float* g_sh, float* g_op,
                         float* g_ref , float* compact);

}
```

brush_amd/csrc/depth_sort.hip:

```cpp
#include <cstddef>

#include "context.h"

namespace bh {

constexpr int DS_WG = 256;
constexpr int DS_WAVES = DS_WG / 64;
#define BH_DS_KPT 8
constexpr int DS_KPT = BH_DS_KPT;
constexpr int DS_TILE = DS_WG * DS_KPT;
constexpr int DS_RADIX = 256;
constexpr uint32_t CULLED_KEY = 0xFFFFFFFFu;

struct DepthSplit {
    uint32_t kmin, kmax;
    uint32_t scale;
    bool any_visible;
    const uint32_t* spl;
};
constexpr uint32_t SPL_WORDS = 258;
static_assert(SPL_WORDS <= DSORT_SPL_STRIDE, "context.h reserves the table");
constexpr uint32_t SPL_MIN_KEYS = 16384;
constexpr uint32_t SPL_SAMPLE_STRIDE = 64;
constexpr uint32_t SPL_SAMPLE_MIN_N = 1u << 17;
constexpr uint32_t SPL_SAMPLE_MIN_KEYS = 1024;
BH_DEV DepthSplit make_split(uint32_t kmax, uint32_t nmin) {
    DepthSplit sp;
    sp.any_visible = nmin != 0u;
    sp.kmin = ~nmin;
    sp.kmax = kmax;
    const uint32_t range = sp.any_visible ? kmax - sp.kmin : 0u;
    sp.scale = (uint32_t)min((unsigned long long)0xFFFFFFFFull, (255ull << 32) / ((unsigned long long)range + 1ull));
    if ((((unsigned long long)range * sp.scale) >> 32) > 254ull) sp.scale -= 1u;
    sp.spl = nullptr;
    return sp;
}

BH_DEV DepthSplit depth_split(const uint32_t* __restrict__ minmax, uint32_t* s_red , const uint32_t* __restrict__ spl_in ,
                              uint32_t* s_spl ) {
    const int tid = threadIdx.x, lane = tid & 63, wave = tid >> 6;
    uint32_t a = 0, b = 0;
    if (tid < (int)COUNTER_SLOTS) {
        a = minmax[2 * tid];
        b = minmax[2 * tid + 1];
    }
    if (spl_in != nullptr) {
        s_spl[tid] = spl_in[tid];
        if (tid < (int)SPL_WORDS - DS_WG) s_spl[DS_WG + tid] = spl_in[DS_WG + tid];
    }
#pragma unroll
    for (int off = 32; off > 0; off >>= 1) {
        a = max(a, (uint32_t)__shfl_xor((int)a, off));
        b = max(b, (uint32_t)__shfl_xor((int)b, off));
    }
    if (lane == 0) { s_red[wave] = a; s_red[DS_WAVES + wave] = b; }
    __syncthreads();
    uint32_t kmax = 0, nmin = 0;
#pragma unroll
    for (int w = 0; w < DS_WAVES; ++w) { kmax = max(kmax, s_red[w]); nmin = max(nmin, s_red[DS_WAVES + w]); }
    __syncthreads();
    DepthSplit sp = make_split(kmax, nmin);
    if (spl_in != nullptr && sp.any_visible && s_spl[255] != 0u) {
        const uint32_t tmin = s_spl[256], tmax = s_spl[257], tol = (tmax - tmin) >> 4;
        const uint32_t dmin = sp.kmin > tmin ? sp.kmin - tmin : tmin - sp.kmin, dmax = sp.kmax > tmax ? sp.kmax - tmax : tmax - sp.kmax;
        if (dmin <= tol && dmax <= tol) sp.spl = s_spl;
    }
    return sp;
}
BH_DEV uint32_t depth_digit(uint32_t key, const DepthSplit& sp) {
    if (key == CULLED_KEY) return 255u;
    if (sp.spl != nullptr) {
        uint32_t d = 0;
#pragma unroll
        for (uint32_t step = 128u; step != 0u; step >>= 1) d += sp.spl[d + step - 1u] <= key ? step : 0u;
        return d;
    }
    return min(254u, (uint32_t)(((unsigned long long)(key - sp.kmin) * sp.scale) >> 32));
}

BH_DEV unsigned long long ds_match(uint32_t d) {
    uint32_t lo = 0xFFFFFFFFu, hi = 0xFFFFFFFFu;
#pragma unroll
    for (int b = 0; b < 8; ++b) {
        const uint32_t bit = (d >> b) & 1u;
        const unsigned long long bal = __ballot(bit);
        const uint32_t flip = bit - 1u;
        lo &= (uint32_t)bal ^ flip;
        hi &= (uint32_t)(bal >> 32) ^ flip;
    }
    return ((unsigned long long)hi << 32) | lo;
}

BH_DEV void counter_sums_to_host(const uint32_t* __restrict__ set, uint32_t* __restrict__ host_sums, int lane, uint32_t tag, uint32_t* __restrict__ dev_sums) {
    const unsigned long long* c64 = reinterpret_cast<const unsigned long long*>(set);
    unsigned long long tot[COUNTER_K1_U64];
#pragma unroll
    for (uint32_t c = 0; c < COUNTER_K1_U64; ++c) tot[c] = 0ull;
    for (uint32_t k = (uint32_t)lane; k < COUNTER_SLOTS; k += 64u) {
#pragma unroll
        for (uint32_t c = 0; c < COUNTER_K1_U64; ++c) tot[c] += c64[COUNTER_K1_U64 * k + c];
    }
#pragma unroll
    for (int off = 32; off > 0; off >>= 1) {
#pragma unroll
        for (uint32_t c = 0; c < COUNTER_K1_U64; ++c) tot[c] += __shfl_down(tot[c], off);
    }
    if (lane == 0) {
        if (dev_sums) {
#pragma unroll
            for (uint32_t c = 0; c < COUNTER_K1_U64; ++c) dev_sums[c] = tot[c] > 0xFFFFFFFFull ? 0xFFFFFFFFu : (uint32_t)tot[c];
        }
        volatile unsigned long long* h64 = reinterpret_cast<volatile unsigned long long*>(host_sums);
#pragma unroll
        for (uint32_t c = 0; c < COUNTER_K1_U64; ++c) h64[c] = tot[c];
        if (tag) {
            __threadfence_system();
            reinterpret_cast<volatile uint32_t*>(host_sums)[HOST_SUM_WORDS - 1u] = tag;
        }
    }
}

__global__ __launch_bounds__(DS_WG) void dsort_hist_kernel(const uint32_t* __restrict__ keys, const uint32_t* __restrict__ counts,
                                                          uint32_t n, uint32_t nblocks, const uint32_t* __restrict__ minmax,
                                                          uint32_t* __restrict__ hist, uint32_t* __restrict__ csum,
                                                          const uint32_t* __restrict__ rb_set, uint32_t* __restrict__ rb_host, uint32_t rb_tag, uint32_t* __restrict__ rb_dev,
                                                          const uint32_t* __restrict__ spl_in, uint8_t* __restrict__ digits ) {
    __shared__ uint32_t s_hist[DS_WAVES][DS_RADIX];
    __shared__ uint32_t s_csum[DS_WAVES][DS_RADIX];
    __shared__ uint32_t s_red[2 * DS_WAVES];
    __shared__ uint32_t s_spl[SPL_WORDS];
    const int tid = threadIdx.x, wave = tid >> 6;
    if (blockIdx.x == nblocks) {
        if (wave == 0) counter_sums_to_host(rb_set, rb_host, tid, rb_tag, rb_dev);
        return;
    }
    for (int i = tid; i < DS_WAVES * DS_RADIX; i += DS_WG) { (&s_hist[0][0])[i] = 0; (&s_csum[0][0])[i] = 0; }
    const DepthSplit sp = depth_split(minmax, s_red, spl_in, s_spl);
    const uint32_t base = blockIdx.x * DS_TILE;
    auto count_one = [&](uint32_t key, uint32_t cnt) {
        const uint32_t d = depth_digit(key, sp);
        if (d != 255u) {
            atomicAdd(&s_hist[wave][d], 1u);
            atomicAdd(&s_csum[wave][d], cnt);
        }
        return d;
    };
    if (base + (uint32_t)DS_TILE <= n && ((reinterpret_cast<uintptr_t>(keys) | reinterpret_cast<uintptr_t>(counts)) & 15u) == 0) {
        const uint4* k4 = reinterpret_cast<const uint4*>(keys + base);
        const uint4* c4 = reinterpret_cast<const uint4*>(counts + base);
        uint4 kv[DS_KPT / 4], cv[DS_KPT / 4];
#pragma unroll
        for (int k = 0; k < DS_KPT / 4; ++k) { kv[k] = k4[k * DS_WG + tid]; cv[k] = c4[k * DS_WG + tid]; }
        uint32_t* d4 = reinterpret_cast<uint32_t*>(digits + base);
#pragma unroll
        for (int k = 0; k < DS_KPT / 4; ++k) {
            const uint32_t d0 = count_one(kv[k].x, cv[k].x);
            const uint32_t d1 = count_one(kv[k].y, cv[k].y);
            const uint32_t d2 = count_one(kv[k].z, cv[k].z);
            const uint32_t d3 = count_one(kv[k].w, cv[k].w);
            d4[k * DS_WG + tid] = d0 | (d1 << 8) | (d2 << 16) | (d3 << 24);
        }
    } else {
#pragma unroll
        for (int k = 0; k < DS_KPT; ++k) {
            const uint32_t idx = base + k * DS_WG + tid;
            if (idx < n) digits[idx] = (uint8_t)count_one(keys[idx], counts[idx]);
        }
    }
    __syncthreads();
    uint32_t t = 0, c = 0;
#pragma unroll
    for (int w = 0; w < DS_WAVES; ++w) { t += s_hist[w][tid]; c += s_csum[w][tid]; }
    hist[(size_t)tid * nblocks + blockIdx.x] = t;
    csum[(size_t)tid * nblocks + blockIdx.x] = c;
}

constexpr int DS_ROW_EPT = 16;
__global__ __launch_bounds__(DS_WG) void dsort_rowscan_kernel(uint32_t* __restrict__ hist, const uint32_t* __restrict__ csum, uint32_t nblocks,
                                                             uint32_t* __restrict__ digit_totals ) {
    const int tid = threadIdx.x, lane = tid & 63, wave = tid >> 6;
    const uint32_t d = blockIdx.x;
    uint32_t* row = hist + (size_t)d * nblocks;
    const uint32_t* crow = csum + (size_t)d * nblocks;
    uint32_t v[DS_ROW_EPT], incl[DS_ROW_EPT];
    __shared__ uint32_t s_chunk[DS_ROW_EPT][DS_WAVES];
    __shared__ uint32_t s_c[DS_WAVES];
    uint32_t cacc = 0;
#pragma unroll
    for (int k = 0; k < DS_ROW_EPT; ++k) {
        const uint32_t i = (uint32_t)k * DS_WG + tid;
        v[k] = i < nblocks ? row[i] : 0u;
        cacc += i < nblocks ? crow[i] : 0u;
    }
#pragma unroll
    for (int off = 32; off > 0; off >>= 1) cacc += __shfl_down(cacc, off);
    if (lane == 0) s_c[wave] = cacc;
#pragma unroll
    for (int k = 0; k < DS_ROW_EPT; ++k) {
        uint32_t x = v[k];
#pragma unroll
        for (int off = 1; off < 64; off <<= 1) {
            const uint32_t t = __shfl_up(x, off);
            if (lane >= off) x += t;
        }
        incl[k] = x;
        if (lane == 63) s_chunk[k][wave] = x;
    }
    __syncthreads();
    uint32_t run = 0;
#pragma unroll
    for (int k = 0; k < DS_ROW_EPT; ++k) {
        uint32_t before = 0, total = 0;
#pragma unroll
        for (int w = 0; w < DS_WAVES; ++w) {
            const uint32_t c = s_chunk[k][w];
            before += w < wave ? c : 0u;
            total += c;
        }
        const uint32_t i = (uint32_t)k * DS_WG + tid;
        if (i < nblocks) row[i] = run + before + incl[k] - v[k];
        run += total;
    }
    if (tid == 0) {
        digit_totals[d] = run;
        digit_totals[DS_RADIX + d] = (s_c[0] + s_c[1]) + (s_c[2] + s_c[3]);
    }
}

template <int WG>
struct ChunkLds {
    uint32_t cnt[WG / 64][DS_RADIX];
    uint32_t dbase[DS_RADIX];
    uint32_t gofs[DS_RADIX];
    uint32_t wsum[WG / 64];
    uint32_t keys[DS_TILE];
    uint32_t vals[DS_TILE];
    uint8_t digs[DS_TILE];
};
template <int WG, class DigitFn>
BH_DEV void scatter_chunk(ChunkLds<WG>& L, uint32_t* __restrict__ s_base , const uint32_t* __restrict__ src_k,
                          const uint32_t* __restrict__ src_v , uint32_t first, uint32_t count, uint32_t* __restrict__ dst_k,
                          uint32_t* __restrict__ dst_v, DigitFn digit, uint32_t* __restrict__ alt_k = nullptr, uint32_t* __restrict__ alt_v = nullptr,
                          const uint8_t* __restrict__ pre_dig = nullptr ) {
    constexpr int WAVES = WG / 64, KPT = DS_TILE / WG;
    const int tid = threadIdx.x, lane = tid & 63, wave = tid >> 6;
    for (int i = tid; i < WAVES * DS_RADIX; i += WG) (&L.cnt[0][0])[i] = 0;
    __syncthreads();
    const uint32_t wave_first = wave * (64 * KPT);
    uint32_t key[KPT], val[KPT], rank[KPT], dig[KPT];
    const unsigned long long lt_mask = (1ull << lane) - 1ull;
    if (count == (uint32_t)DS_TILE) {
#pragma unroll
        for (int k = 0; k < KPT; ++k) {
            const uint32_t e = wave_first + k * 64 + lane;
            key[k] = src_k[first + e];
            val[k] = src_v ? src_v[first + e] : first + e;
        }
        if (pre_dig) {
#pragma unroll
            for (int k = 0; k < KPT; ++k) dig[k] = pre_dig[first + wave_first + k * 64 + lane];
        } else {
#pragma unroll
            for (int k = 0; k < KPT; ++k) dig[k] = digit(key[k]);
        }
    } else {
#pragma unroll
        for (int k = 0; k < KPT; ++k) {
            const uint32_t e = wave_first + k * 64 + lane;
            const bool valid = e < count;
            key[k] = valid ? src_k[first + e] : 0u;
            val[k] = valid ? (src_v ? src_v[first + e] : first + e) : 0u;
            dig[k] = valid ? (pre_dig ? (uint32_t)pre_dig[first + e] : digit(key[k])) : 255u;
        }
    }
#pragma unroll
    for (int k = 0; k < KPT; ++k) {
        const unsigned long long peers = ds_match(dig[k]);
        const uint32_t prior = L.cnt[wave][dig[k]];
        rank[k] = prior + (uint32_t)__popcll(peers & lt_mask);
        if ((peers & lt_mask) == 0ull) L.cnt[wave][dig[k]] = prior + (uint32_t)__popcll(peers);
    }
    __syncthreads();
    uint32_t total = 0;
    if (tid < DS_RADIX) {
        uint32_t run = 0;
#pragma unroll
        for (int w = 0; w < WAVES; ++w) {
            const uint32_t c = L.cnt[w][tid];
            L.cnt[w][tid] = run;
            run += c;
        }
        total = run;
    }
    {
        uint32_t incl = total;
#pragma unroll
        for (int off = 1; off < 64; off <<= 1) {
            const uint32_t t = __shfl_up(incl, off);
            if (lane >= off) incl += t;
        }
        if (lane == 63) L.wsum[wave] = incl;
        __syncthreads();
        if (tid < DS_RADIX) {
            uint32_t wofs = 0;
#pragma unroll
            for (int w = 0; w < DS_RADIX / 64; ++w) wofs += (w < wave) ? L.wsum[w] : 0u;
            const uint32_t excl = incl - total + wofs;
            L.dbase[tid] = excl;
            const uint32_t dst0 = s_base[tid];
            L.gofs[tid] = dst0 - excl;
            const uint32_t tail = (uint32_t)DS_TILE - count;
            s_base[tid] = dst0 + total - (tid == 255 ? tail : 0u);
        }
    }
    __syncthreads();
#pragma unroll
    for (int k = 0; k < KPT; ++k) {
        const uint32_t lpos = L.dbase[dig[k]] + L.cnt[wave][dig[k]] + rank[k];
        L.keys[lpos] = key[k];
        L.vals[lpos] = val[k];
        if (pre_dig) L.digs[lpos] = (uint8_t)dig[k];
    }
    __syncthreads();
#pragma unroll
    for (int k = 0; k < KPT; ++k) {
        const uint32_t e = k * WG + tid;
        if (e < count) {
            const uint32_t kk = L.keys[e];
            const uint32_t d = pre_dig ? (uint32_t)L.digs[e] : digit(kk);
            const uint32_t pos = L.gofs[d] + e;
            if (alt_k != nullptr && d == 255u) continue;
            dst_k[pos] = kk;
            dst_v[pos] = L.vals[e];
        }
    }
    __syncthreads();
}

__global__ __launch_bounds__(DS_WG) void dsort_split_kernel(const uint32_t* __restrict__ keys, uint32_t n, uint32_t nblocks,
                                                           const uint32_t* __restrict__ offsets ,
                                                           const uint32_t* __restrict__ digit_totals, uint32_t* __restrict__ out_keys,
                                                           uint32_t* __restrict__ out_vals, uint32_t* __restrict__ fin_keys, uint32_t* __restrict__ fin_vals,
                                                           const uint8_t* __restrict__ digits ) {
    __shared__ ChunkLds<DS_WG> L;
    __shared__ uint32_t s_base[DS_RADIX];
    __shared__ uint32_t s_red[2 * DS_WAVES];
    const int tid = threadIdx.x, lane = tid & 63, wave = tid >> 6;
    {
        const uint32_t gt = digit_totals[tid];
        uint32_t gincl = gt;
#pragma unroll
        for (int off = 1; off < 64; off <<= 1) {
            const uint32_t g = __shfl_up(gincl, off);
            if (lane >= off) gincl += g;
        }
        if (lane == 63) s_red[wave] = gincl;
        __syncthreads();
        uint32_t gofs = 0;
#pragma unroll
        for (int w = 0; w < DS_WAVES; ++w) gofs += (w < wave) ? s_red[w] : 0u;
        s_base[tid] = gincl - gt + gofs + offsets[(size_t)tid * nblocks + blockIdx.x];
    }
    __syncthreads();
    const uint32_t first = blockIdx.x * DS_TILE;
    const uint32_t count = n - first < (uint32_t)DS_TILE ? n - first : (uint32_t)DS_TILE;
    scatter_chunk<DS_WG>(L, s_base, keys, nullptr, first, count, out_keys, out_vals, [](uint32_t) { return 0u; }, fin_keys, fin_vals, digits);
}

#define BH_BK_WG 1024
constexpr int BK_WG = BH_BK_WG;
constexpr int BK_WAVES = BK_WG / 64;
constexpr int BK_KPT = DS_TILE / BK_WG;
constexpr int FAST_CAP = BK_WG <= 512 ? 8192 : 7168;
constexpr int FAST_NDIG = 512;
constexpr size_t FAST_LDS_WORDS = 4 * FAST_CAP + (BK_WAVES + 1) * FAST_NDIG;
static_assert(FAST_LDS_WORDS * 4 >= sizeof(ChunkLds<BK_WG>), "the dynamic LDS block holds either path's arrays");
static_assert(offsetof(ChunkLds<BK_WG>, vals) == offsetof(ChunkLds<BK_WG>, keys) + sizeof(uint32_t) * DS_TILE, "scan staging spans keys[] and vals[]");

BH_DEV uint32_t bk_excl_scan(uint32_t v, uint32_t& total, uint32_t* s_w) {
    const int lane = threadIdx.x & 63, wave = threadIdx.x >> 6;
    uint32_t incl = v;
#pragma unroll
    for (int off = 1; off < 64; off <<= 1) {
        const uint32_t x = __shfl_up(incl, off);
        if (lane >= off) incl += x;
    }
    if (lane == 63) s_w[wave] = incl;
    __syncthreads();
    uint32_t wofs = 0, tot = 0;
#pragma unroll
    for (int w = 0; w < BK_WAVES; ++w) { wofs += (w < wave) ? s_w[w] : 0u; tot += s_w[w]; }
    total = tot;
    __syncthreads();
    return incl - v + wofs;
}

BH_DEV void bk_scan_counts(const uint32_t* vals, uint32_t size, const uint32_t* __restrict__ counts, uint32_t carry, uint32_t* __restrict__ cum_out,
                           uint32_t* stage, uint32_t* s_w) {
    const int tid = threadIdx.x;
    const uint32_t nch = (size + DS_TILE - 1) / DS_TILE;
    for (uint32_t c = 0; c < nch; ++c) {
        const uint32_t first = c * DS_TILE;
        const uint32_t count = size - first < (uint32_t)DS_TILE ? size - first : (uint32_t)DS_TILE;
#pragma unroll
        for (int k = 0; k < BK_KPT; ++k) {
            const uint32_t e = k * BK_WG + tid;
            stage[e + e / BK_KPT] = e < count ? counts[vals[first + e]] : 0u;
        }
        __syncthreads();
        uint32_t v[BK_KPT], tsum = 0;
#pragma unroll
        for (int k = 0; k < BK_KPT; ++k) { v[k] = stage[tid * (BK_KPT + 1) + k]; tsum += v[k]; }
        uint32_t total;
        uint32_t run = carry + bk_excl_scan(tsum, total, s_w);
#pragma unroll
        for (int k = 0; k < BK_KPT; ++k) { run += v[k]; stage[tid * (BK_KPT + 1) + k] = run; }
        __syncthreads();
#pragma unroll
        for (int k = 0; k < BK_KPT; ++k) {
            const uint32_t e = k * BK_WG + tid;
            if (e < count) cum_out[first + e] = stage[e + e / BK_KPT];
        }
        carry += total;
        __syncthreads();
    }
}

BH_DEV uint32_t bk_key_bits(uint32_t& lo, uint32_t hi, uint32_t* s_w) {
    const int lane = threadIdx.x & 63, wave = threadIdx.x >> 6;
#pragma unroll
    for (int off = 32; off > 0; off >>= 1) {
        lo = min(lo, (uint32_t)__shfl_xor((int)lo, off));
        hi = max(hi, (uint32_t)__shfl_xor((int)hi, off));
    }
    if (lane == 0) { s_w[wave] = lo; s_w[BK_WAVES + wave] = hi; }
    __syncthreads();
#pragma unroll
    for (int w = 0; w < BK_WAVES; ++w) { lo = min(lo, s_w[w]); hi = max(hi, s_w[BK_WAVES + w]); }
    __syncthreads();
    return hi > lo ? 32u - (uint32_t)__clz(hi - lo) : 0u;
}

BH_DEV void bk_write_splitters(const uint32_t* sorted , uint32_t start, uint32_t size, uint32_t nv,
                               uint32_t* __restrict__ spl_out, uint32_t spl_min_keys) {
    const uint32_t j = threadIdx.x;
    if (spl_out == nullptr || nv < spl_min_keys || j >= 254u) return;
    const uint32_t r = (uint32_t)(((unsigned long long)(j + 1u) * nv) / 255ull);
    if (r >= start && r - start < size) spl_out[j] = sorted[r - start];
}

__global__ __launch_bounds__(BK_WG) void dsort_bucket_kernel(uint32_t* __restrict__ a_keys, uint32_t* __restrict__ a_vals ,
                                                            uint32_t* __restrict__ out_keys, uint32_t* __restrict__ out_vals,
                                                            const uint32_t* __restrict__ minmax, const uint32_t* __restrict__ digit_totals,
                                                            const uint32_t* __restrict__ counts, uint32_t* __restrict__ cum ,
                                                            uint32_t* __restrict__ spl_out , uint32_t spl_min_keys) {
    extern __shared__ __attribute__((aligned(16))) uint32_t s_dyn[];
    __shared__ uint32_t s_base[DS_RADIX];
    __shared__ uint32_t s_hist[DS_RADIX];
    __shared__ uint32_t s_red[2 * BK_WAVES];
    const int tid = threadIdx.x, lane = tid & 63, wave = tid >> 6;
    const uint32_t b = blockIdx.x;
    uint32_t start, size, tiles_before, nv;
    {
        const uint32_t gt = tid < DS_RADIX ? digit_totals[tid] : 0u;
        const uint32_t ct = tid < 255 ? digit_totals[DS_RADIX + tid] : 0u;
        uint32_t tot;
        const uint32_t gex = bk_excl_scan(gt, nv, s_red);
        const uint32_t cex = bk_excl_scan(ct, tot, s_red);
        if (tid < DS_RADIX) { s_base[tid] = gex; s_hist[tid] = cex; }
        __syncthreads();
        start = s_base[b];
        size = s_base[b + 1u] - start;
        tiles_before = s_hist[b];
        __syncthreads();
    }
    if (b == 0u && spl_out != nullptr) {
        uint32_t x = 0, y = 0;
        if (tid < (int)COUNTER_SLOTS) { x = minmax[2 * tid]; y = minmax[2 * tid + 1]; }
#pragma unroll
        for (int off = 32; off > 0; off >>= 1) {
            x = max(x, (uint32_t)__shfl_xor((int)x, off));
            y = max(y, (uint32_t)__shfl_xor((int)y, off));
        }
        if (lane == 0) { s_red[wave] = x; s_red[BK_WAVES + wave] = y; }
        __syncthreads();
        if (tid == 0) {
            uint32_t kmax = 0, nmin = 0;
            for (int w = 0; w < BK_WAVES; ++w) { kmax = max(kmax, s_red[w]); nmin = max(nmin, s_red[BK_WAVES + w]); }
            spl_out[254] = 0xFFFFFFFFu;
            spl_out[255] = nv >= spl_min_keys ? 1u : 0u;
            spl_out[256] = ~nmin;
            spl_out[257] = kmax;
        }
        __syncthreads();
    }
    if (size == 0u) return;
    if (size <= (uint32_t)FAST_CAP) {
        uint32_t* fcnt = s_dyn + 4 * FAST_CAP;
        uint32_t* fdb = fcnt + BK_WAVES * FAST_NDIG;
        uint32_t lo = 0xFFFFFFFFu, hi = 0u;
        for (uint32_t i = tid; i < size; i += BK_WG) {
            const uint32_t k = a_keys[start + i];
            s_dyn[i] = k;
            s_dyn[FAST_CAP + i] = a_vals[start + i];
            lo = min(lo, k);
            hi = max(hi, k);
        }
        const uint32_t bits = bk_key_bits(lo, hi, s_red);
        const uint32_t passes = (bits + 8u) / 9u;
        const uint32_t base_w = passes ? bits / passes : 0u, wide = passes ? bits % passes : 0u;
        const unsigned long long lt_mask = (1ull << lane) - 1ull;
        const uint32_t steps = (size + (uint32_t)BK_WG - 1u) / (uint32_t)BK_WG;
        const uint32_t wave_first = wave * steps * 64u;
        uint32_t cur = 0;
        for (uint32_t p = 0; p < passes; ++p) {
            const uint32_t width = base_w + (p < wide ? 1u : 0u);
            const uint32_t pshift = p * base_w + (p < wide ? p : wide);
            const uint32_t mask = (1u << width) - 1u;
            const uint32_t* sk = s_dyn + cur * (2 * FAST_CAP); const uint32_t* sv = sk + FAST_CAP;
            uint32_t* dk = s_dyn + (cur ^ 1u) * (2 * FAST_CAP); uint32_t* dv = dk + FAST_CAP;
            for (int i = tid; i < BK_WAVES * FAST_NDIG; i += BK_WG) fcnt[i] = 0;
            __syncthreads();
            for (uint32_t r = 0; r < steps; ++r) {
                const uint32_t e = wave_first + r * 64u + lane;
                if (e < size) atomicAdd(&fcnt[wave * FAST_NDIG + (((sk[e] - lo) >> pshift) & mask)], 1u);
            }
            __syncthreads();
            {
                uint32_t run = 0;
                if (tid < FAST_NDIG) {
#pragma unroll
                    for (int w = 0; w < BK_WAVES; ++w) {
                        const uint32_t c = fcnt[w * FAST_NDIG + tid];
                        fcnt[w * FAST_NDIG + tid] = run;
                        run += c;
                    }
                }
                uint32_t tot;
                const uint32_t ex = bk_excl_scan(run, tot, s_red);
                if (tid < FAST_NDIG) fdb[tid] = ex;
            }
            __syncthreads();
            for (uint32_t r = 0; r < steps; ++r) {
                const uint32_t e = wave_first + r * 64u + lane;
                const bool valid = e < size;
                const uint32_t key = valid ? sk[e] : 0u, val = valid ? sv[e] : 0u;
                const uint32_t d = valid ? ((key - lo) >> pshift) & mask : mask;
                uint32_t plo = 0xFFFFFFFFu, phi = 0xFFFFFFFFu;
                for (uint32_t bb = 0; bb < width; ++bb) {
                    const uint32_t bit = (d >> bb) & 1u;
                    const unsigned long long bal = __ballot(bit);
                    const uint32_t flip = bit - 1u;
                    plo &= (uint32_t)bal ^ flip;
                    phi &= (uint32_t)(bal >> 32) ^ flip;
                }
                const unsigned long long peers = ((unsigned long long)phi << 32) | plo;
                const uint32_t cursor = fcnt[wave * FAST_NDIG + d];
                const uint32_t pos = fdb[d] + cursor + (uint32_t)__popcll(peers & lt_mask);
                if ((peers & lt_mask) == 0ull) fcnt[wave * FAST_NDIG + d] = cursor + (uint32_t)__popcll(peers);
                if (valid) { dk[pos] = key; dv[pos] = val; }
            }
            __syncthreads();
            cur ^= 1u;
        }
        const uint32_t* fk = s_dyn + cur * (2 * FAST_CAP); const uint32_t* fv = fk + FAST_CAP;
        uint32_t* spare = s_dyn + (cur ^ 1u) * (2 * FAST_CAP);
        bk_write_splitters(fk, start, size, nv, spl_out, spl_min_keys);
        for (uint32_t i = tid; i < size; i += BK_WG) {
            const uint32_t v = fv[i];
            out_keys[start + i] = fk[i];
            out_vals[start + i] = v;
            if (cum != nullptr) { const uint32_t e = i; spare[e + e / BK_KPT] = counts[v]; }
        }
        if (cum == nullptr) return;
        __syncthreads();
        {
            uint32_t carry = tiles_before;
            const uint32_t nch = (size + DS_TILE - 1) / DS_TILE;
            for (uint32_t c = 0; c < nch; ++c) {
                const uint32_t first = c * DS_TILE;
                uint32_t v[BK_KPT], tsum = 0;
#pragma unroll
                for (int k = 0; k < BK_KPT; ++k) {
                    const uint32_t e = first + tid * BK_KPT + k;
                    v[k] = e < size ? spare[e + e / BK_KPT] : 0u;
                    tsum += v[k];
                }
                uint32_t total;
                uint32_t run = carry + bk_excl_scan(tsum, total, s_red);
#pragma unroll
                for (int k = 0; k < BK_KPT; ++k) {
                    const uint32_t e = first + tid * BK_KPT + k;
                    run += v[k];
                    if (e < size) spare[e + e / BK_KPT] = run;
                }
                carry += total;
            }
            __syncthreads();
            for (uint32_t i = tid; i < size; i += BK_WG) cum[start + i] = spare[i + i / BK_KPT];
        }
        return;
    }
    ChunkLds<BK_WG>& L = *reinterpret_cast<ChunkLds<BK_WG>*>(s_dyn);
    uint32_t lo = 0xFFFFFFFFu, hi = 0u;
    for (uint32_t i = tid; i < size; i += BK_WG) {
        const uint32_t k = a_keys[start + i];
        lo = min(lo, k);
        hi = max(hi, k);
    }
    const uint32_t bits = bk_key_bits(lo, hi, s_red);
    const uint32_t passes = bits <= 8u ? 1u : (bits <= 24u ? 3u : 5u);
    const uint32_t base_w = bits / passes, wide = bits % passes;
    uint32_t* src_k = a_keys; uint32_t* src_v = a_vals;
    uint32_t* dst_k = out_keys; uint32_t* dst_v = out_vals;
    const uint32_t nchunks = (size + DS_TILE - 1) / DS_TILE;
    for (uint32_t p = 0; p < passes; ++p) {
        const uint32_t width = base_w + (p < wide ? 1u : 0u);
        const uint32_t pshift = p * base_w + (p < wide ? p : wide);
        const uint32_t mask = (1u << width) - 1u;
        auto digit = [=](uint32_t k) { return ((k - lo) >> pshift) & mask; };
        if (tid < DS_RADIX) s_hist[tid] = 0;
        __syncthreads();
        if (width != 0u) {
            for (uint32_t i = tid; i < size; i += BK_WG) atomicAdd(&s_hist[digit(src_k[start + i])], 1u);
        } else if (tid == 0) {
            s_hist[0] = size;
        }
        __syncthreads();
        {
            uint32_t tot;
            const uint32_t ex = bk_excl_scan(tid < DS_RADIX ? s_hist[tid] : 0u, tot, s_red);
            if (tid < DS_RADIX) s_base[tid] = start + ex;
        }
        __syncthreads();
        for (uint32_t c = 0; c < nchunks; ++c) {
            const uint32_t first = start + c * DS_TILE;
            const uint32_t count = size - c * DS_TILE < (uint32_t)DS_TILE ? size - c * DS_TILE : (uint32_t)DS_TILE;
            scatter_chunk<BK_WG>(L, s_base, src_k, src_v, first, count, dst_k, dst_v, digit);
        }
        __threadfence_block();
        __syncthreads();
        uint32_t* tk = src_k; src_k = dst_k; dst_k = tk;
        uint32_t* tv = src_v; src_v = dst_v; dst_v = tv;
    }
    bk_write_splitters(out_keys + start, start, size, nv, spl_out, spl_min_keys);
    if (cum != nullptr) bk_scan_counts(out_vals + start, size, counts, tiles_before, cum + start, &L.keys[0], s_red);
}

#define BH_DSORT_MAX_N (16u << 20)
constexpr uint32_t DSORT_MAX_N = BH_DSORT_MAX_N;
bool depth_sort_supported(uint32_t n) { return n > 0 && n <= DSORT_MAX_N && (n + DS_TILE - 1) / DS_TILE <= (uint32_t)DS_ROW_EPT * DS_WG; }

__global__ __launch_bounds__(256) void dsort_sample_kernel(const uint32_t* __restrict__ keys, uint32_t stride, uint32_t m, uint32_t* __restrict__ out) {
    const uint32_t i = blockIdx.x * 256u + threadIdx.x;
    if (i < m) out[i] = keys[(size_t)i * stride];
}

static int dsort_launches(bh_ctx* ctx, const uint32_t* keys, const uint32_t* minmax, const uint32_t* counts, uint32_t n, uint32_t* out_keys, uint32_t* out_vals,
                          uint32_t* cum, const uint32_t* rb_set, uint32_t* rb_host, hipEvent_t rb_done, uint32_t rb_tag, uint32_t* rb_dev, uint32_t* totals,
                          uint32_t* a_keys, uint32_t* a_vals, const uint32_t* spl_in, uint32_t* spl_out, uint32_t spl_min_keys) {
    const uint32_t nblocks = (n + DS_TILE - 1) / DS_TILE;
    uint32_t* hist = totals + 2 * DS_RADIX;
    uint32_t* csum = hist + (size_t)DS_RADIX * nblocks;
    uint8_t* digits = reinterpret_cast<uint8_t*>(csum + (size_t)DS_RADIX * nblocks);
    hipLaunchKernelGGL(dsort_hist_kernel, dim3(nblocks + (rb_set ? 1u : 0u)), dim3(DS_WG), 0, ctx->stream, keys, counts, n, nblocks, minmax, hist, csum,
                       rb_set, rb_host, rb_tag, rb_dev, spl_in, digits);
    BH_LAUNCH_CHECK(ctx, "dsort_hist_kernel");
    if (rb_set && !rb_tag) BH_HIP(ctx, hipEventRecord(rb_done, ctx->stream));
    hipLaunchKernelGGL(dsort_rowscan_kernel, dim3(DS_RADIX), dim3(DS_WG), 0, ctx->stream, hist, csum, nblocks, totals);
    BH_LAUNCH_CHECK(ctx, "dsort_rowscan_kernel");
    hipLaunchKernelGGL(dsort_split_kernel, dim3(nblocks), dim3(DS_WG), 0, ctx->stream, keys, n, nblocks, hist, totals, a_keys, a_vals, out_keys, out_vals, digits);
    BH_LAUNCH_CHECK(ctx, "dsort_split_kernel");
    if (!ctx->dsort_lds_raised) {
        BH_HIP(ctx, hipFuncSetAttribute((const void*)dsort_bucket_kernel, hipFuncAttributeMaxDynamicSharedMemorySize, (int)(FAST_LDS_WORDS * 4)));
        ctx->dsort_lds_raised = true;
    }
    hipLaunchKernelGGL(dsort_bucket_kernel, dim3(DS_RADIX - 1), dim3(BK_WG), FAST_LDS_WORDS * 4, ctx->stream, a_keys, a_vals, out_keys, out_vals, minmax, totals, counts, cum, spl_out,
                       spl_min_keys);
    BH_LAUNCH_CHECK(ctx, "dsort_bucket_kernel");
    return 0;
}

int depth_sort_scan(bh_ctx* ctx, const uint32_t* keys, const uint32_t* minmax, const uint32_t* counts, uint32_t n, uint32_t* out_keys,
                    uint32_t* out_vals, uint32_t* cum, const uint32_t* rb_set, uint32_t* rb_host, hipEvent_t rb_done, uint32_t rb_tag, uint32_t* rb_dev, uint32_t* spl,
                    bool* spl_written) {
    if (n == 0) return 0;
    const uint32_t nblocks = (n + DS_TILE - 1) / DS_TILE;
    if (!ctx->knob_dsort_splitters) spl = nullptr;
    else if (spl == nullptr) {
        if (ctx->dsort_spl == nullptr) {
            if (hipMalloc((void**)&ctx->dsort_spl, DSORT_SPL_STRIDE * 4) != hipSuccess) { (void)hipGetLastError(); ctx->dsort_spl = nullptr; return BH_ERR_OOM; }
            BH_HIP(ctx, hipMemsetAsync(ctx->dsort_spl, 0, DSORT_SPL_STRIDE * 4, ctx->stream));
            ctx->dsort_spl_written = false;
        }
        spl = ctx->dsort_spl;
        spl_written = &ctx->dsort_spl_written;
    }
    uint32_t* totals = (uint32_t*)ensure(ctx, SLOT_SORT_HIST, ((size_t)2 * DS_RADIX * nblocks + 2 * DS_RADIX) * 4 + (size_t)nblocks * DS_TILE);
    uint32_t* a_keys = (uint32_t*)ensure(ctx, SLOT_SORT_KEYS_A, (size_t)n * 4);
    uint32_t* a_vals = (uint32_t*)ensure(ctx, SLOT_SORT_VALS_A, (size_t)n * 4);
    if (!totals || !a_keys || !a_vals) return BH_ERR_OOM;
    if (spl && spl_written && !*spl_written && n >= SPL_SAMPLE_MIN_N) {
        const uint32_t m = n / SPL_SAMPLE_STRIDE;
        uint32_t* sample = (uint32_t*)ensure(ctx, SLOT_SORT_KEYS_B, (size_t)m * 4);
        if (!sample) return BH_ERR_OOM;
        hipLaunchKernelGGL(dsort_sample_kernel, dim3((m + 255u) / 256u), dim3(256), 0, ctx->stream, keys, SPL_SAMPLE_STRIDE, m, sample);
        BH_LAUNCH_CHECK(ctx, "dsort_sample_kernel");
        BH_TRY(dsort_launches(ctx, sample, minmax, sample, m, out_keys, out_vals, nullptr, nullptr, nullptr, nullptr, 0u, nullptr, totals, a_keys, a_vals, nullptr, spl,
                              SPL_SAMPLE_MIN_KEYS));
    }
    BH_TRY(dsort_launches(ctx, keys, minmax, counts, n, out_keys, out_vals, cum, rb_set, rb_host, rb_done, rb_tag, rb_dev, totals, a_keys, a_vals, spl, spl, SPL_MIN_KEYS));
    if (spl && spl_written) *spl_written = true;
    return 0;
}

}
```

brush_amd/csrc/project.hip:

```cpp
#include "context.h"
#include "device_camera.h"
#include "device_sh.h"

namespace bh {

constexpr int PROJ_WG = 256;
constexpr int PROJ_WAVES = PROJ_WG / 64;
constexpr uint32_t ORDER_BINS = 1024;

struct WalkLds {
    uint32_t count[64];
    float mx[64], my[64], c00[64], c01[64], c11[64], pt[64];
    uint32_t magic[64];
    uint32_t box[64];
    uint32_t boxw[64];
    uint32_t start[64];
    uint32_t lane_of[64];
    uint32_t zkey[64];
    uint32_t near[64];
    uint8_t flags[64];
};

BH_DEV uint32_t walk_magic(uint32_t bw, uint32_t nb) {
    if (bw < 2u || (unsigned long long)nb * bw >= (1ull << 32)) return 0u;
    return 0xFFFFFFFFu / bw + 1u;
}
BH_DEV uint32_t walk_row(uint32_t i, uint32_t bw, uint32_t magic) {
    if (magic) return __umulhi(i, magic);
    if (bw < 2u) return i;
    uint32_t row = (uint32_t)(((float)i + 0.5f) / (float)bw);
    if (row * bw > i) --row;
    else if ((row + 1u) * bw <= i) ++row;
    return row;
}

BH_DEV uint32_t wave_inclusive_scan_u32(uint32_t v, int lane) {
#pragma unroll
    for (int off = 1; off < 64; off <<= 1) {
        const uint32_t t = __shfl_up(v, off);
        if (lane >= off) v += t;
    }
    return v;
}

struct KeepAllTiles { static constexpr bool EAGER = false; BH_DEV bool operator()(const WalkLds&, uint32_t, uint32_t, uint32_t) const { return true; } };
struct KeepLiveTiles {
    static constexpr bool EAGER = false;
    const uint32_t* done_bits;
    uint32_t tile_bw;
    BH_DEV bool operator()(const WalkLds&, uint32_t, uint32_t tx, uint32_t ty) const {
        const uint32_t t = tx + ty * tile_bw;
        return ((done_bits[t >> 5] >> (t & 31u)) & 1u) == 0u;
    }
};
struct KeepNearOfCut {
    const uint32_t* zcut;
    uint32_t tile_bw;
    static constexpr bool EAGER = true;
    BH_DEV uint32_t fetch(uint32_t tx, uint32_t ty) const { return zcut[tx + ty * tile_bw]; }
    BH_DEV bool decide(const WalkLds& w, uint32_t r, uint32_t cut) const { return zcut_near(w.zkey[r], cut); }
    BH_DEV bool operator()(const WalkLds& w, uint32_t r, uint32_t tx, uint32_t ty) const { return decide(w, r, fetch(tx, ty)); }
};

struct NoPrefetch { BH_DEV uint32_t operator()(uint32_t, uint32_t) const { return 0u; } };
template <class OnHit, class Keep = KeepAllTiles, class Pre = NoPrefetch>
BH_DEV uint32_t flat_tile_walk(WalkLds& w, int lane, uint32_t nb, float mx, float my, Sym2 conic, float pt, TileBbox bb,
                               OnHit on_hit, Keep keep = Keep{}, uint32_t zkey = 0u, Pre pre = Pre{}) {
    const uint32_t incl = wave_inclusive_scan_u32(nb, lane);
    const uint32_t start = incl - nb;
    const bool nz = nb > 0u;
    const unsigned long long nzmask = __ballot(nz);
    const unsigned long long below = (1ull << lane) - 1ull;
    const uint32_t rank = (uint32_t)__popcll(nzmask & below);
    const uint32_t bb_w = bb.max_x - bb.min_x;
    if (nz) {
        w.count[rank] = 0;
        w.near[rank] = 0;
        w.zkey[rank] = zkey;
        w.mx[rank] = mx; w.my[rank] = my;
        w.c00[rank] = conic.c00; w.c01[rank] = conic.c01; w.c11[rank] = conic.c11;
        w.pt[rank] = pt;
        w.magic[rank] = walk_magic(bb_w, nb);
        w.box[rank] = bb.min_x | (bb.min_y << 16);
        w.boxw[rank] = bb_w;
        w.start[rank] = start;
        w.lane_of[rank] = (uint32_t)lane;
    }
    __builtin_amdgcn_fence(__ATOMIC_SEQ_CST, "wavefront");
    uint8_t* flags = w.flags;
    const uint32_t tot = __shfl(incl, 63);
    const unsigned long long le = below | (1ull << lane);
    uint32_t before = 0;
    for (uint32_t base = 0; base < tot; base += 64) {
        flags[lane] = 0;
        const uint32_t rel = start - base;
        if (nz && rel < 64u) flags[rel] = 1;
        asm volatile("" ::: "memory");
        const unsigned long long marks = __ballot(flags[lane] != 0);
        asm volatile("" ::: "memory");
        const uint32_t c = base + (uint32_t)lane;
        if (c < tot) {
            const uint32_t r = before + (uint32_t)__popcll(marks & le) - 1u;
            const uint32_t i = c - w.start[r];
            const uint32_t box = w.box[r];
            const uint32_t bw = w.boxw[r];
            const uint32_t row = walk_row(i, bw, w.magic[r]);
            const uint32_t tx = (box & 0xFFFFu) + (i - __umul24(row, bw));
            const uint32_t ty = (box >> 16) + row;
            const uint32_t fetched = pre(tx, ty);
            if (keep(w, r, tx, ty) && will_primitive_contribute(tx, ty, w.mx[r], w.my[r], Sym2{w.c00[r], w.c01[r], w.c11[r]}, w.pt[r])) on_hit(r, tx, ty, fetched);
        }
        before += (uint32_t)__popcll(marks);
    }
    __builtin_amdgcn_fence(__ATOMIC_SEQ_CST, "wavefront");
    return rank;
}

template <class Keep = KeepAllTiles>
BH_DEV uint32_t flat_tile_walk_emit(WalkLds& w, int lane, uint32_t nb, float mx, float my, Sym2 conic, float pt, TileBbox bb,
                                    uint32_t wave_base, uint32_t wave_total, uint32_t tile_bw, uint32_t cg0, uint32_t* __restrict__ tile_ids,
                                    uint32_t* __restrict__ isect_gids, Keep keep = Keep{}, uint32_t zkey = 0u) {
    const uint32_t incl = wave_inclusive_scan_u32(nb, lane);
    const uint32_t start = incl - nb;
    const bool nz = nb > 0u;
    const unsigned long long nzmask = __ballot(nz);
    const unsigned long long below = (1ull << lane) - 1ull;
    const uint32_t rank = (uint32_t)__popcll(nzmask & below);
    const uint32_t bb_w = bb.max_x - bb.min_x;
    if (nz) {
        w.zkey[rank] = zkey;
        w.mx[rank] = mx; w.my[rank] = my;
        w.c00[rank] = conic.c00; w.c01[rank] = conic.c01; w.c11[rank] = conic.c11;
        w.pt[rank] = pt;
        w.magic[rank] = walk_magic(bb_w, nb);
        w.box[rank] = bb.min_x | (bb.min_y << 16);
        w.boxw[rank] = bb_w;
        w.start[rank] = start;
        w.lane_of[rank] = (uint32_t)lane;
    }
    __builtin_amdgcn_fence(__ATOMIC_SEQ_CST, "wavefront");
    uint8_t* flags = w.flags;
    const uint32_t tot = __shfl(incl, 63);
    const unsigned long long le = below | (1ull << lane);
    uint32_t before = 0;
    uint32_t emitted = 0;
    for (uint32_t base = 0; base < tot; base += 64) {
        flags[lane] = 0;
        const uint32_t rel = start - base;
        if (nz && rel < 64u) flags[rel] = 1;
        asm volatile("" ::: "memory");
        const unsigned long long marks = __ballot(flags[lane] != 0);
        asm volatile("" ::: "memory");
        const uint32_t c = base + (uint32_t)lane;
        bool hit = false;
        uint32_t tile = 0, owner = 0;
        if (c < tot) {
            const uint32_t r = before + (uint32_t)__popcll(marks & le) - 1u;
            const uint32_t i = c - w.start[r];
            const uint32_t box = w.box[r];
            const uint32_t bw = w.boxw[r];
            const uint32_t row = walk_row(i, bw, w.magic[r]);
            const uint32_t tx = (box & 0xFFFFu) + (i - __umul24(row, bw));
            const uint32_t ty = (box >> 16) + row;
            if constexpr (Keep::EAGER) {
                const uint32_t cut = keep.fetch(tx, ty);
                uint32_t contributes = will_primitive_contribute(tx, ty, w.mx[r], w.my[r], Sym2{w.c00[r], w.c01[r], w.c11[r]}, w.pt[r]) ? 1u : 0u;
                asm volatile("" : "+v"(contributes));
                hit = contributes != 0u && keep.decide(w, r, cut);
            } else {
                hit = keep(w, r, tx, ty) && will_primitive_contribute(tx, ty, w.mx[r], w.my[r], Sym2{w.c00[r], w.c01[r], w.c11[r]}, w.pt[r]);
            }
            tile = tx + ty * tile_bw;
            owner = cg0 + w.lane_of[r];
        }
        const unsigned long long hits = __ballot(hit);
        if (hit) {
            const uint32_t local = emitted + (uint32_t)__popcll(hits & below);
            if (local < wave_total) {
                tile_ids[wave_base + local] = tile;
                isect_gids[wave_base + local] = owner;
            }
        }
        emitted += (uint32_t)__popcll(hits);
        before += (uint32_t)__popcll(marks);
    }
    for (uint32_t k = emitted + (uint32_t)lane; k < wave_total; k += 64u) {
        tile_ids[wave_base + k] = 0xFFFFFFFFu;
        isect_gids[wave_base + k] = 0u;
    }
    return emitted;
}

template <bool MIP, bool PINHOLE, int DEG>
__global__ __launch_bounds__(PROJ_WG) void project_forward_kernel(
    ViewUniforms u, uint32_t n, const float* __restrict__ transforms, const float* __restrict__ coeffs,
    const float* __restrict__ raw_opacities, uint32_t* __restrict__ depth_keys, uint32_t* __restrict__ isect_counts,
    float* __restrict__ max_radius, float* __restrict__ projected_by_gid, unsigned long long* __restrict__ counters, ForwardPrep prep,
    uint32_t* __restrict__ zcut, uint32_t* __restrict__ near_counts) {
    __shared__ WalkLds s_walk[PROJ_WAVES];
    __shared__ uint32_t s_vis[PROJ_WAVES];
    __shared__ uint32_t s_hit[PROJ_WAVES];
    __shared__ uint32_t s_near[PROJ_WAVES];
    __shared__ uint32_t s_listed[PROJ_WAVES];
    __shared__ uint32_t s_kmax[PROJ_WAVES];
    __shared__ uint32_t s_nmax[PROJ_WAVES];
    const uint32_t gid = blockIdx.x * PROJ_WG + threadIdx.x;
    if (prep.order_out && blockIdx.x < 8u) {
        __shared__ uint32_t s_bins[ORDER_BINS];
        const uint32_t per = band_slots(prep.order_tiles);
        __shared__ uint32_t s_band_work, s_band_cnt, s_band_tail, s_band_max;
        for (uint32_t i = threadIdx.x; i < ORDER_BINS; i += PROJ_WG) s_bins[i] = 0u;
        if (threadIdx.x == 0) s_band_work = s_band_cnt = s_band_tail = s_band_max = 0u;
        __syncthreads();
        uint32_t my_work = 0u, my_cnt = 0u, my_max = 0u;
        for (uint32_t i = threadIdx.x; i < per; i += PROJ_WG) {
            const uint32_t lt = band_tile(blockIdx.x, i, per, prep.band_mode);
            if (lt >= prep.order_tiles) continue;
            const uint32_t wk = prep.order_work[prep.order_tile_begin + lt];
            atomicAdd(&s_bins[ORDER_BINS - 1u - (wk < ORDER_BINS ? wk : ORDER_BINS - 1u)], 1u);
            my_work += wk < ORDER_BINS ? wk : ORDER_BINS - 1u;
            my_max = max(my_max, wk < ORDER_BINS ? wk : ORDER_BINS - 1u);
            my_cnt++;
        }
        if (prep.split_out && my_work) atomicAdd(&s_band_work, my_work);
        if (my_cnt) atomicAdd(&s_band_cnt, my_cnt);
        if (prep.split_out && my_max) atomicMax(&s_band_max, my_max);
        __syncthreads();
        const uint32_t cnt = s_band_cnt;
        {
            __shared__ uint32_t s_part[PROJ_WG];
            const uint32_t b0 = threadIdx.x * (ORDER_BINS / PROJ_WG);
            uint32_t loc[ORDER_BINS / PROJ_WG], sum = 0;
#pragma unroll
            for (uint32_t k = 0; k < ORDER_BINS / PROJ_WG; ++k) { loc[k] = sum; sum += s_bins[b0 + k]; }
            s_part[threadIdx.x] = sum;
            __syncthreads();
            if (threadIdx.x == 0) {
                uint32_t run = 0;
                for (uint32_t k = 0; k < (uint32_t)PROJ_WG; ++k) { const uint32_t t = s_part[k]; s_part[k] = run; run += t; }
            }
            __syncthreads();
#pragma unroll
            for (uint32_t k = 0; k < ORDER_BINS / PROJ_WG; ++k) s_bins[b0 + k] = s_part[threadIdx.x] + loc[k];
        }
        __syncthreads();
        if (prep.split_out) {
            if (threadIdx.x == 0) {
                const float mean = cnt ? (float)s_band_work / (float)cnt : 0.0f;
                const float thr_f = fmaxf(fmaxf((float)prep.split_min, prep.split_factor * mean), prep.split_of_max * (float)s_band_max);
                uint32_t h = 0u;
                if (prep.order_mode == 1u && thr_f < (float)(ORDER_BINS - 1u)) {
                    const uint32_t thr = (uint32_t)ceilf(thr_f);
                    h = s_bins[ORDER_BINS - thr];
                }
                prep.split_out[blockIdx.x] = h < SPLIT_MAX ? h : SPLIT_MAX;
            }
            uint32_t* scr = prep.split_out + 8u + blockIdx.x * (SPLIT_MAX * 4u);
            for (uint32_t i = threadIdx.x; i < SPLIT_MAX * 4u; i += PROJ_WG) scr[i] = 0u;
        }
        __syncthreads();
        for (uint32_t i = threadIdx.x; i < per; i += PROJ_WG) {
            const uint32_t lt = band_tile(blockIdx.x, i, per, prep.band_mode);
            if (lt < prep.order_tiles) {
                const uint32_t wk = prep.order_work[prep.order_tile_begin + lt];
                const uint32_t rank = atomicAdd(&s_bins[ORDER_BINS - 1u - (wk < ORDER_BINS ? wk : ORDER_BINS - 1u)], 1u);
                prep.order_out[blockIdx.x * per + rank] = lt;
            } else {
                prep.order_out[blockIdx.x * per + cnt + atomicAdd(&s_band_tail, 1u)] = 0xFFFFFFFFu;
            }
        }
        __syncthreads();
    }
    if (gid < prep.visible_words) prep.visible[gid] = 0u;
    if (gid < prep.tile_words) prep.tile_table[gid] = 0u;
    if (gid < prep.slice_words) prep.slice_table[gid] = 0u;
    if (gid < COUNTER_SET_U64 && prep.next_counters) prep.next_counters[gid] = 0ull;
    for (size_t i = gid; i < prep.span_f4; i += (size_t)gridDim.x * PROJ_WG) prep.span[i] = make_float4(0.0f, 0.0f, 0.0f, 0.0f);
    const int lane = threadIdx.x & 63, wave = threadIdx.x >> 6;
    uint32_t key = 0xFFFFFFFFu;
    float radius = 0.0f;
    bool visible = false;
    float mx = 0.0f, my = 0.0f, pt = 0.0f, opac = 0.0f;
    Sym2 conic = Sym2{0.0f, 0.0f, 0.0f};
    TileBbox bb = TileBbox{0, 0, 0, 0};
    Vec3A mean = v3(0.0f, 0.0f, 0.0f);
    const uint32_t gsafe = gid < n ? gid : (n ? n - 1u : 0u);
    float tr[10];
    {
        const float* trp = transforms + (size_t)gsafe * 10;
#pragma unroll
        for (int k = 0; k < 10; ++k) tr[k] = trp[k];
    }
    float raw_opac = raw_opacities[gsafe];
    constexpr int C_ALL = (DEG + 1) * (DEG + 1);
    float sh_dc[3];
#pragma unroll
    for (int k = 0; k < 3; ++k) sh_dc[k] = coeffs[(size_t)gsafe * C_ALL * 3 + k];
    asm volatile("" : "+v"(tr[0]), "+v"(tr[1]), "+v"(tr[2]), "+v"(tr[3]), "+v"(tr[4]), "+v"(tr[5]), "+v"(tr[6]), "+v"(tr[7]), "+v"(tr[8]), "+v"(tr[9]),
                      "+v"(raw_opac), "+v"(sh_dc[0]), "+v"(sh_dc[1]), "+v"(sh_dc[2]));
    if (gid < n) {
        do {
            mean = v3(tr[0], tr[1], tr[2]);
            const Vec3A mean_c = world_to_cam(mean, u);
            if (!(finite3(mean_c) && mean_c.z <= 1.0e10f)) break;
            if (!in_front_of_camera<PINHOLE>(mean_c, u)) break;
            const Vec3A scl = v3(bh_expf(tr[7]), bh_expf(tr[8]), bh_expf(tr[9]));
            if (!finite3(scl)) break;
            const Quat qu = Quat{tr[3], tr[4], tr[5], tr[6]};
            const float qn = qdot(qu, qu);
            if (!(qn >= 1.0e-6f && is_finite_f32(qn))) break;
            if (!is_finite_f32(raw_opac)) break;
            const Quat q = qnormalize(qu);
            const Sym2 raw_cov = calc_cov2d<PINHOLE>(scl, q, mean_c, u);
            float filter_comp;
            const Sym2 cov = compensate_cov2d<MIP>(raw_cov, filter_comp);
            opac = sigmoid(raw_opac) * filter_comp;
            if (!sym2_finite(cov)) break;
            project_point<PINHOLE>(mean_c, u, mx, my);
            if (!(opac >= 1.0f / 255.0f)) break;
            pt = bh_logf(opac * 255.0f);
            conic = sym2_inverse(cov);
            float ex, ey;
            compute_bbox_extent(conic, pt, ex, ey);
            if (!(ex >= 0.0f && ey >= 0.0f)) break;
            const float wf = (float)u.img_w, hf = (float)u.img_h;
            const bool on_screen = mx + ex > 0.0f && mx - ex < wf && my + ey > 0.0f && my - ey < hf;
            if (!on_screen) break;
            bb = get_tile_bbox(mx, my, ex, ey, u.tile_bw, u.tile_y0, u.tile_y1);
            const bool whole = u.tile_y0 == 0u && u.tile_y1 == u.tile_bh;
            if (!whole && (bb.max_y <= bb.min_y || bb.max_x <= bb.min_x)) break;
            radius = __builtin_fmaxf(ex / wf, ey / hf);
            key = f2u(mean_c.z);
            visible = true;
        } while (false);
    }
    const uint32_t nb = visible ? (bb.max_y - bb.min_y) * (bb.max_x - bb.min_x) : 0u;
    WalkLds& w = s_walk[wave];
    const uint32_t tile_bw = u.tile_bw;
    struct CutOfTile {
        const uint32_t* zcut;
        uint32_t tile_bw;
        BH_DEV uint32_t operator()(uint32_t tx, uint32_t ty) const { return zcut ? zcut[tx + ty * tile_bw] : 0u; }
    };
    const uint32_t wrank = flat_tile_walk(w, lane, nb, mx, my, conic, pt, bb, [&](uint32_t r, uint32_t tx, uint32_t ty, uint32_t cut) {
        atomicAdd(&w.count[r], 1u);
        if (zcut) {
            if (zcut_near(w.zkey[r], cut)) atomicAdd(&w.near[r], 1u);
            else if ((cut & 1u) == 0u) zcut[tx + ty * tile_bw] = cut | 1u;
        }
    }, KeepAllTiles{}, key, CutOfTile{zcut, tile_bw});
    const uint32_t tiles_hit = nb ? w.count[wrank] : 0u;
    const uint32_t near_hit = (nb && zcut) ? w.near[wrank] : 0u;
    const bool listed = visible && (!zcut || near_hit > 0u || prep.list_all_visible);
    if (listed) {
        const Vec3A v = normalize(sub(mean, camera_pos(u)));
        constexpr int C = (DEG + 1) * (DEG + 1);
        const Vec3A raw = sh_coeffs_to_color_dc<DEG>(coeffs + (size_t)gid * C * 3, v, sh_dc);
        const float cr = raw.x + 0.5f, cgc = raw.y + 0.5f, cb = raw.z + 0.5f;
        float* o = projected_by_gid + (size_t)gid * 9;
        o[0] = mx;
        o[1] = my;
        o[2] = conic.c00;
        o[3] = conic.c01;
        o[4] = conic.c11;
        o[5] = opac;
        o[6] = clampf(is_finite_f32(cr) ? cr : 0.0f, -100.0f, 100.0f);
        o[7] = clampf(is_finite_f32(cgc) ? cgc : 0.0f, -100.0f, 100.0f);
        o[8] = clampf(is_finite_f32(cb) ? cb : 0.0f, -100.0f, 100.0f);
    }
    if (gid < n) {
        depth_keys[gid] = listed ? key : 0xFFFFFFFFu;
        isect_counts[gid] = tiles_hit;
        max_radius[gid] = radius;
        if (zcut) near_counts[gid] = near_hit;
    }
    const unsigned long long ball = __ballot(visible);
    const unsigned long long lball = __ballot(listed);
    uint32_t wave_hits = tiles_hit;
#pragma unroll
    for (int off = 32; off > 0; off >>= 1) wave_hits += __shfl_down(wave_hits, off);
    uint32_t wave_near = 0;
    if (zcut) {
        wave_near = near_hit;
#pragma unroll
        for (int off = 32; off > 0; off >>= 1) wave_near += __shfl_down(wave_near, off);
    }
    uint32_t kmax = listed ? key : 0u, nmax = listed ? ~key : 0u;
#pragma unroll
    for (int off = 32; off > 0; off >>= 1) {
        kmax = max(kmax, (uint32_t)__shfl_xor((int)kmax, off));
        nmax = max(nmax, (uint32_t)__shfl_xor((int)nmax, off));
    }
    if (lane == 0) {
        s_vis[wave] = (uint32_t)__popcll(ball);
        s_hit[wave] = wave_hits;
        s_near[wave] = wave_near;
        s_listed[wave] = (uint32_t)__popcll(lball);
        s_kmax[wave] = kmax;
        s_nmax[wave] = nmax;
    }
    __syncthreads();
    if (threadIdx.x == 0) {
        uint32_t v = 0, h = 0, nh = 0, ls = 0, km = 0, nm = 0;
#pragma unroll
        for (int k = 0; k < PROJ_WAVES; ++k) { v += s_vis[k]; h += s_hit[k]; nh += s_near[k]; ls += s_listed[k]; km = max(km, s_kmax[k]); nm = max(nm, s_nmax[k]); }
        const uint32_t sl = blockIdx.x & (COUNTER_SLOTS - 1u);
        unsigned long long* slot = counters + COUNTER_K1_U64 * sl;
        if (v) atomicAdd(&slot[0], (unsigned long long)v);
        if (h) atomicAdd(&slot[1], (unsigned long long)h);
        if (nh) atomicAdd(&slot[2], (unsigned long long)nh);
        if (ls && zcut) atomicAdd(&slot[3], (unsigned long long)ls);
        if (ls) {
            uint32_t* mm = reinterpret_cast<uint32_t*>(counters) + COUNTER_MINMAX_WORD + 2u * sl;
            atomicMax(&mm[0], km);
            atomicMax(&mm[1], nm);
        }
    }
}

template <bool MIP, bool PINHOLE>
static int launch_pf_deg(bh_ctx* ctx, const ViewUniforms& u, uint32_t n, uint32_t deg, const float* t, const float* sh, const float* ro,
                         uint32_t* keys, uint32_t* counts, float* radius, float* proj, unsigned long long* c64, const ForwardPrep& prep,
                         uint32_t* zcut, uint32_t* near_counts) {
    const dim3 grid((n + PROJ_WG - 1) / PROJ_WG), block(PROJ_WG);
    switch (deg) {
        case 0: hipLaunchKernelGGL((project_forward_kernel<MIP, PINHOLE, 0>), grid, block, 0, ctx->stream, u, n, t, sh, ro, keys, counts, radius, proj, c64, prep, zcut, near_counts); break;
        case 1: hipLaunchKernelGGL((project_forward_kernel<MIP, PINHOLE, 1>), grid, block, 0, ctx->stream, u, n, t, sh, ro, keys, counts, radius, proj, c64, prep, zcut, near_counts); break;
        case 2: hipLaunchKernelGGL((project_forward_kernel<MIP, PINHOLE, 2>), grid, block, 0, ctx->stream, u, n, t, sh, ro, keys, counts, radius, proj, c64, prep, zcut, near_counts); break;
        case 3: hipLaunchKernelGGL((project_forward_kernel<MIP, PINHOLE, 3>), grid, block, 0, ctx->stream, u, n, t, sh, ro, keys, counts, radius, proj, c64, prep, zcut, near_counts); break;
        case 4: hipLaunchKernelGGL((project_forward_kernel<MIP, PINHOLE, 4>), grid, block, 0, ctx->stream, u, n, t, sh, ro, keys, counts, radius, proj, c64, prep, zcut, near_counts); break;
        default: return set_error(ctx, BH_ERR_INVALID_ARG, "sh_degree must be 0..4");
    }
    BH_LAUNCH_CHECK(ctx, "project_forward_kernel");
    return 0;
}

int launch_project_forward(bh_ctx* ctx, const ViewUniforms& u, uint32_t n, bool mip, uint32_t sh_degree, const float* transforms,
                           const float* sh, const float* raw_opac, uint32_t* depth_keys, uint32_t* isect_counts, float* max_radius,
                           float* projected_by_gid, uint32_t* counters, const ForwardPrep& want, uint32_t* zcut, uint32_t* near_counts) {
    if (zcut && !near_counts) return set_error(ctx, BH_ERR_INVALID_ARG, "project_forward: a depth-cut table needs the near-count output");
    ForwardPrep prep = want;
    const size_t covered = (size_t)((n + PROJ_WG - 1) / PROJ_WG) * PROJ_WG;
    if (prep.visible && prep.visible_words > covered) {
        BH_HIP(ctx, hipMemsetAsync(prep.visible, 0, (size_t)prep.visible_words * 4, ctx->stream));
        prep.visible_words = 0;
    }
    if (prep.next_counters && COUNTER_SET_U64 > covered) {
        BH_HIP(ctx, hipMemsetAsync(prep.next_counters, 0, COUNTER_SET_BYTES, ctx->stream));
        prep.next_counters = nullptr;
    }
    if (prep.tile_table && prep.tile_words > covered) {
        BH_HIP(ctx, hipMemsetAsync(prep.tile_table, 0, (size_t)prep.tile_words * 4, ctx->stream));
        prep.tile_words = 0;
    }
    if (prep.slice_table && prep.slice_words > covered) {
        BH_HIP(ctx, hipMemsetAsync(prep.slice_table, 0, (size_t)prep.slice_words * 4, ctx->stream));
        prep.slice_words = 0;
    }
    if (n == 0) {
        if (prep.next_counters) BH_HIP(ctx, hipMemsetAsync(prep.next_counters, 0, COUNTER_SET_BYTES, ctx->stream));
        if (prep.span && prep.span_f4) BH_HIP(ctx, hipMemsetAsync(prep.span, 0, (size_t)prep.span_f4 * 16, ctx->stream));
        return 0;
    }
    auto* c64 = reinterpret_cast<unsigned long long*>(counters);
    const bool pinhole = u.model == CAM_PINHOLE;
    if (mip && pinhole) return launch_pf_deg<true, true>(ctx, u, n, sh_degree, transforms, sh, raw_opac, depth_keys, isect_counts, max_radius, projected_by_gid, c64, prep, zcut, near_counts);
    if (pinhole) return launch_pf_deg<false, true>(ctx, u, n, sh_degree, transforms, sh, raw_opac, depth_keys, isect_counts, max_radius, projected_by_gid, c64, prep, zcut, near_counts);
    if (mip) return launch_pf_deg<true, false>(ctx, u, n, sh_degree, transforms, sh, raw_opac, depth_keys, isect_counts, max_radius, projected_by_gid, c64, prep, zcut, near_counts);
    return launch_pf_deg<false, false>(ctx, u, n, sh_degree, transforms, sh, raw_opac, depth_keys, isect_counts, max_radius, projected_by_gid, c64, prep, zcut, near_counts);
}

__global__ __launch_bounds__(PROJ_WG) void project_visible_kernel(uint32_t nv, const float* __restrict__ projected_by_gid,
                                                                 const uint32_t* __restrict__ global_from_compact_gid,
                                                                 float* __restrict__ projected) {
    const uint32_t e = blockIdx.x * PROJ_WG + threadIdx.x;
    if (e >= nv * 9u) return;
    const uint32_t cg = e / 9u, j = e - cg * 9u;
    projected[e] = projected_by_gid[(size_t)global_from_compact_gid[cg] * 9 + j];
}

int launch_project_visible(bh_ctx* ctx, uint32_t nv, const float* projected_by_gid, const uint32_t* gid, float* projected) {
    if (nv == 0) return 0;
    const uint64_t total = (uint64_t)nv * 9u;
    if (total > 0xFFFFFFFFull) return set_error(ctx, BH_ERR_UNSUPPORTED, "more than 2^32/9 visible splats");
    hipLaunchKernelGGL(project_visible_kernel, dim3((unsigned)((total + PROJ_WG - 1) / PROJ_WG)), dim3(PROJ_WG), 0, ctx->stream, nv,
                       projected_by_gid, gid, projected);
    BH_LAUNCH_CHECK(ctx, "project_visible_kernel");
    return 0;
}

template <bool FAR, int SPW>
__global__ __launch_bounds__(PROJ_WG) void map_gaussians_kernel(
    uint32_t nv, uint32_t tile_bw, uint32_t tile_bh, uint32_t tile_y0, uint32_t tile_y1, const float* __restrict__ projected_by_gid,
    const uint32_t* __restrict__ global_from_compact_gid, float* __restrict__ projected,
    const uint32_t* __restrict__ cum_tiles_hit, uint32_t* __restrict__ tile_id_from_isect,
    uint32_t* __restrict__ compact_gid_from_isect, float4* __restrict__ zero_span, uint32_t zero_f4, uint32_t budget,
    uint32_t* __restrict__ slice_info, const uint32_t* __restrict__ far_counts, const uint32_t* __restrict__ far_block_totals,
    const uint32_t* __restrict__ far_group_totals, const uint32_t* __restrict__ done_bits, const uint32_t* __restrict__ gate,
    const uint32_t* __restrict__ zcut, const uint32_t* __restrict__ depth_keys_sorted, const uint32_t* __restrict__ nv_dev, uint32_t pair_cap) {
    __shared__ WalkLds s_walk[PROJ_WAVES];
    __shared__ uint32_t s_far[2 * PROJ_WAVES];
    if (FAR && *gate == 0u) return;
    if (nv_dev) {
        const uint32_t live = *nv_dev;
        nv = live < nv ? live : nv;
        const size_t zf = ((size_t)nv * 10 + 3) / 4;
        zero_f4 = zf < (size_t)zero_f4 ? (uint32_t)zf : zero_f4;
    }
    const uint32_t tid_lin = blockIdx.x * PROJ_WG + threadIdx.x;
    for (size_t i = tid_lin; i < zero_f4; i += (size_t)gridDim.x * PROJ_WG) zero_span[i] = make_float4(0.0f, 0.0f, 0.0f, 0.0f);
    const int lane = threadIdx.x & 63, wave = threadIdx.x >> 6;
    const uint32_t cg0 = (blockIdx.x * PROJ_WAVES + (uint32_t)wave) * (uint32_t)SPW;
    const uint32_t cg = lane < SPW ? cg0 + (uint32_t)lane : 0xFFFFFFFFu;
    uint32_t far_base = 0, far_cnt = 0;
    if (FAR) {
        far_cnt = cg < nv ? far_counts[cg] : 0u;
        uint32_t ahead = 0;
        const uint32_t group = blockIdx.x / FAR_GROUP_BLOCKS;
        for (uint32_t g = threadIdx.x; g < group; g += PROJ_WG) ahead += far_group_totals[g];
        { const uint32_t b = group * FAR_GROUP_BLOCKS + threadIdx.x; if (threadIdx.x < FAR_GROUP_BLOCKS && b < blockIdx.x) ahead += far_block_totals[b]; }
        uint32_t incl = far_cnt;
#pragma unroll
        for (int off = 1; off < 64; off <<= 1) {
            const uint32_t t = __shfl_up(incl, off);
            if (lane >= off) incl += t;
        }
#pragma unroll
        for (int off = 32; off > 0; off >>= 1) ahead += __shfl_down(ahead, off);
        if (lane == 63) s_far[wave] = incl;
        if (lane == 0) s_far[PROJ_WAVES + wave] = ahead;
        __syncthreads();
        uint32_t before = 0, block_ahead = 0, block_total = 0;
#pragma unroll
        for (int w = 0; w < PROJ_WAVES; ++w) {
            before += w < wave ? s_far[w] : 0u;
            block_total += s_far[w];
            block_ahead += s_far[PROJ_WAVES + w];
        }
        far_base = block_ahead + before + incl - far_cnt;
        if (blockIdx.x == gridDim.x - 1u && threadIdx.x == 0) slice_info[3] = block_ahead + block_total;
    }
    float xy_x = 0.0f, xy_y = 0.0f, pt = 0.0f;
    Sym2 conic = Sym2{0.0f, 0.0f, 0.0f};
    TileBbox bb = TileBbox{0, 0, 0, 0};
    uint32_t base = 0, end = 0, nb = 0, zkey = 0;
    bool mine = false;
    if (cg < nv) {
        uint32_t cum_end = cum_tiles_hit[cg];
        uint32_t cum_prev = cum_tiles_hit[cg == 0u ? 0u : cg - 1u];
        uint32_t my_gid = global_from_compact_gid[cg];
        if (zcut) zkey = depth_keys_sorted[cg];
        asm volatile("" : "+v"(cum_end), "+v"(cum_prev), "+v"(my_gid), "+v"(zkey));
        if (cg == 0u) cum_prev = 0u;
        if (FAR) {
            base = far_base;
            end = far_base + far_cnt;
            mine = cum_end > budget && end > base;
        } else if (zcut) {
            base = cum_prev;
            end = cum_end;
            mine = end > base;
            if (slice_info && cg + 1u == nv) { slice_info[0] = nv; slice_info[1] = cum_end; }
        } else {
            base = cum_prev;
            end = cum_end;
            mine = cum_end <= budget;
            if (slice_info) {
                const uint32_t next_end = cg + 1u < nv ? cum_tiles_hit[cg + 1u] : 0xFFFFFFFFu;
                if (mine && (cg + 1u == nv || next_end > budget)) { slice_info[0] = cg + 1u; slice_info[1] = cum_end; }
                if (!mine && cg == 0u) { slice_info[0] = 0u; slice_info[1] = 0u; }
            }
        }
        if (mine) {
            const float* src = projected_by_gid + (size_t)my_gid * 9;
            float p[9];
#pragma unroll
            for (int k = 0; k < 9; ++k) p[k] = src[k];
            float* dst = projected + (size_t)cg * 9;
#pragma unroll
            for (int k = 0; k < 9; ++k) dst[k] = p[k];
            xy_x = p[0]; xy_y = p[1];
            conic = Sym2{p[2], p[3], p[4]};
            pt = bh_logf(p[5] * 255.0f);
            float ex, ey;
            compute_bbox_extent(conic, pt, ex, ey);
            bb = get_tile_bbox(xy_x, xy_y, ex, ey, tile_bw, tile_y0, tile_y1);
            nb = (bb.max_y - bb.min_y) * (bb.max_x - bb.min_x);
        }
    }
    const unsigned long long mine_mask = __ballot(mine);
    if (mine_mask == 0ull) return;
    WalkLds& w = s_walk[wave];
    const int first_lane = __builtin_ctzll(mine_mask), last_lane = 63 - __builtin_clzll(mine_mask);
    const uint32_t wave_base = __shfl(base, first_lane);
    const uint32_t wave_total = __shfl(end, last_lane) - wave_base;
    if (!FAR && (wave_base > pair_cap || wave_total > pair_cap - wave_base)) return;
    if (FAR) {
        (void)flat_tile_walk_emit(w, lane, nb, xy_x, xy_y, conic, pt, bb, wave_base, wave_total, tile_bw, cg0, tile_id_from_isect, compact_gid_from_isect, KeepLiveTiles{done_bits, tile_bw});
    } else {
        if (zcut) (void)flat_tile_walk_emit(w, lane, nb, xy_x, xy_y, conic, pt, bb, wave_base, wave_total, tile_bw, cg0, tile_id_from_isect, compact_gid_from_isect, KeepNearOfCut{zcut, tile_bw}, zkey);
        else (void)flat_tile_walk_emit(w, lane, nb, xy_x, xy_y, conic, pt, bb, wave_base, wave_total, tile_bw, cg0, tile_id_from_isect, compact_gid_from_isect);
    }
    (void)tile_bh;
}

BH_DEV uint32_t band_of(uint32_t t, uint32_t extent) { return (t * 32u) / extent; }
BH_DEV uint32_t band_mask(uint32_t lo, uint32_t hi, uint32_t extent) {
    const uint32_t b0 = band_of(lo, extent), b1 = band_of(hi - 1u, extent);
    return (0xFFFFFFFFu >> (31u - (b1 - b0))) << b0;
}

__global__ __launch_bounds__(PROJ_WG) void slice_count_kernel(uint32_t nv, uint32_t tile_bw, uint32_t tile_bh, uint32_t tile_y0, uint32_t tile_y1,
                                                             const float* __restrict__ projected_by_gid,
                                                             const uint32_t* __restrict__ global_from_compact_gid,
                                                             const uint32_t* __restrict__ cum_tiles_hit, uint32_t budget,
                                                             const uint32_t* __restrict__ done_bits, const uint32_t* __restrict__ gate,
                                                             uint32_t* __restrict__ counts, uint32_t* __restrict__ block_totals,
                                                             uint32_t* __restrict__ group_totals, const uint32_t* __restrict__ live_bands) {
    __shared__ WalkLds s_walk[PROJ_WAVES];
    __shared__ uint32_t s_tot[PROJ_WAVES];
    if (*gate == 0u) return;
    const uint32_t live_cols = live_bands[0], live_rows = live_bands[1];
    const uint32_t cg = blockIdx.x * PROJ_WG + threadIdx.x;
    const int lane = threadIdx.x & 63, wave = threadIdx.x >> 6;
    float xy_x = 0.0f, xy_y = 0.0f, pt = 0.0f;
    Sym2 conic = Sym2{0.0f, 0.0f, 0.0f};
    TileBbox bb = TileBbox{0, 0, 0, 0};
    uint32_t nb = 0;
    if (cg < nv && cum_tiles_hit[cg] > budget) {
        const float* src = projected_by_gid + (size_t)global_from_compact_gid[cg] * 9;
        xy_x = src[0]; xy_y = src[1];
        conic = Sym2{src[2], src[3], src[4]};
        pt = bh_logf(src[5] * 255.0f);
        float ex, ey;
        compute_bbox_extent(conic, pt, ex, ey);
        bb = get_tile_bbox(xy_x, xy_y, ex, ey, tile_bw, tile_y0, tile_y1);
        nb = (bb.max_y - bb.min_y) * (bb.max_x - bb.min_x);
        if (nb) {
            if ((band_mask(bb.min_x, bb.max_x, tile_bw) & live_cols) == 0u || (band_mask(bb.min_y, bb.max_y, tile_bh) & live_rows) == 0u) nb = 0u;
        }
    }
    WalkLds& w = s_walk[wave];
    uint32_t hits = 0;
    if (__ballot(nb > 0u) != 0ull) {
        const uint32_t wrank = flat_tile_walk(w, lane, nb, xy_x, xy_y, conic, pt, bb, [&](uint32_t r, uint32_t, uint32_t, uint32_t) { atomicAdd(&w.count[r], 1u); },
                                              KeepLiveTiles{done_bits, tile_bw});
        hits = nb ? w.count[wrank] : 0u;
    }
    if (cg < nv) counts[cg] = hits;
    uint32_t wsum = hits;
#pragma unroll
    for (int off = 32; off > 0; off >>= 1) wsum += __shfl_down(wsum, off);
    if (lane == 0) s_tot[wave] = wsum;
    __syncthreads();
    if (threadIdx.x == 0) {
        uint32_t t = 0;
#pragma unroll
        for (int w = 0; w < PROJ_WAVES; ++w) t += s_tot[w];
        block_totals[blockIdx.x] = t;
        if (t) atomicAdd(group_totals + blockIdx.x / FAR_GROUP_BLOCKS, t);
    }
}

int launch_map_gaussians(bh_ctx* ctx, uint32_t nv, const ViewUniforms& u, const float* projected_by_gid, const uint32_t* gid,
                         float* projected, const uint32_t* cum_tiles_hit, uint32_t* tile_ids, uint32_t* isect_gids,
                         float4* zero_span, uint32_t zero_f4, uint32_t budget, uint32_t* slice_info, const uint32_t* zcut,
                         const uint32_t* depth_keys_sorted, const uint32_t* nv_dev, uint32_t pair_cap) {
    if (nv == 0) return 0;
    if (zcut && (!slice_info || !depth_keys_sorted)) return set_error(ctx, BH_ERR_INVALID_ARG, "map_gaussians: a depth-cut table needs the slice words and the sorted keys");
    const dim3 grid((nv + PROJ_WG - 1) / PROJ_WG), block(PROJ_WG);
    const uint32_t* nul = nullptr;
    if (slice_info) {
#define BH_K5_SPW 16
        constexpr int SPW = BH_K5_SPW;
        const dim3 grid16((nv + PROJ_WAVES * SPW - 1) / (PROJ_WAVES * SPW));
        hipLaunchKernelGGL((map_gaussians_kernel<false, SPW>), grid16, block, 0, ctx->stream, nv, u.tile_bw, u.tile_bh, u.tile_y0, u.tile_y1, projected_by_gid, gid,
                           projected, cum_tiles_hit, tile_ids, isect_gids, zero_span, zero_f4, budget, slice_info, nul, nul, nul, nul, nul, zcut, depth_keys_sorted, nv_dev, pair_cap);
    } else if (ctx->knob_k5_exact_spw != 64u) {
        const uint32_t spw = ctx->knob_k5_exact_spw == 16u ? 16u : 32u;
        const dim3 gridn((nv + PROJ_WAVES * spw - 1) / (PROJ_WAVES * spw));
        if (spw == 16u)
            hipLaunchKernelGGL((map_gaussians_kernel<false, 16>), gridn, block, 0, ctx->stream, nv, u.tile_bw, u.tile_bh, u.tile_y0, u.tile_y1, projected_by_gid, gid,
                               projected, cum_tiles_hit, tile_ids, isect_gids, zero_span, zero_f4, budget, slice_info, nul, nul, nul, nul, nul, nul, nul, nv_dev, pair_cap);
        else
            hipLaunchKernelGGL((map_gaussians_kernel<false, 32>), gridn, block, 0, ctx->stream, nv, u.tile_bw, u.tile_bh, u.tile_y0, u.tile_y1, projected_by_gid, gid,
                               projected, cum_tiles_hit, tile_ids, isect_gids, zero_span, zero_f4, budget, slice_info, nul, nul, nul, nul, nul, nul, nul, nv_dev, pair_cap);
    } else {
        hipLaunchKernelGGL((map_gaussians_kernel<false, 64>), grid, block, 0, ctx->stream, nv, u.tile_bw, u.tile_bh, u.tile_y0, u.tile_y1, projected_by_gid, gid,
                           projected, cum_tiles_hit, tile_ids, isect_gids, zero_span, zero_f4, budget, slice_info, nul, nul, nul, nul, nul, nul, nul, nv_dev, pair_cap);
    }
    BH_LAUNCH_CHECK(ctx, "map_gaussians_kernel");
    return 0;
}

int launch_map_gaussians_far(bh_ctx* ctx, uint32_t nv, const ViewUniforms& u, const float* projected_by_gid, const uint32_t* gid,
                             float* projected, const uint32_t* cum_tiles_hit, uint32_t budget, const uint32_t* done_bits, const uint32_t* gate,
                             uint32_t* counts, uint32_t* block_totals, uint32_t* group_totals, uint32_t* slice_info, uint32_t* tile_ids,
                             uint32_t* isect_gids) {
    if (nv == 0) return 0;
    const dim3 grid((nv + PROJ_WG - 1) / PROJ_WG), block(PROJ_WG);
    hipLaunchKernelGGL(slice_count_kernel, grid, block, 0, ctx->stream, nv, u.tile_bw, u.tile_bh, u.tile_y0, u.tile_y1, projected_by_gid, gid, cum_tiles_hit,
                       budget, done_bits, gate, counts, block_totals, group_totals, (const uint32_t*)(slice_info + 4));
    BH_LAUNCH_CHECK(ctx, "slice_count_kernel");
    hipLaunchKernelGGL((map_gaussians_kernel<true, 64>), grid, block, 0, ctx->stream, nv, u.tile_bw, u.tile_bh, u.tile_y0, u.tile_y1, projected_by_gid, gid,
                       projected, cum_tiles_hit, tile_ids, isect_gids, (float4*)nullptr, 0u, budget, slice_info, (const uint32_t*)counts,
                       (const uint32_t*)block_totals, (const uint32_t*)group_totals, done_bits, gate, (const uint32_t*)nullptr, (const uint32_t*)nullptr, (const uint32_t*)nullptr, 0xFFFFFFFFu);
    BH_LAUNCH_CHECK(ctx, "map_gaussians_kernel<far>");
    return 0;
}

BH_DEV Quat apply_normalize_vjp(Quat q, Quat g) {
    const float lsq = qdot(q, q);
    const float l = __builtin_sqrtf(lsq);
    const float inv = 1.0f / (l * lsq);
    const float qw = q.w, qx = q.x, qy = q.y, qz = q.z;
    const float gw = g.w, gx = g.x, gy = g.y, gz = g.z;
    const float cc0 = -qw * qx, cc1 = -qx * qy, cc2 = -qy * qw;
    const float cs0 = -qw * qz, cs1 = -qx * qz, cs2 = -qy * qz;
// ... 173 lines not shown
```

Before: 1229.

## Build depth-sort digits and histograms inside the projection kernel

After: 1247 (median of 6 runs). +1.5%, better.

```diff
diff --git a/brush_amd/csrc/api.hip b/brush_amd/csrc/api.hip
--- a/brush_amd/csrc/api.hip
+++ b/brush_amd/csrc/api.hip
@@ -345,6 +345,7 @@
     {"lpt_classes", "log|linear: work classes of the backward's longest-first tile order — two per octave of blended splats, or 1/64 of the mean list length wide"},
     {"generic_depth_sort", "0|1: depth order by the generic radix sort + scan instead of the fused split sort"},
     {"dsort_splitters", "0|1: the fused depth sort splits at the 254 depth quantiles of the view's previous frame (default 1) or always linearly over the frame's key range"},
+    {"dsort_k1_hist", "0|1: a frame whose view has a valid splitter table takes the depth sort's digits and histograms from the projection kernel (default 1) or from the sort's histogram launch"},
     {"tile_sort", "auto|bucket|lsd: the forward's tile sort (auto: bucket sort unless the view's pairs are concentrated in few tiles)"},
     {"spec_k5", "0|1: queue the list builder before the host has read the frame's counts (default 1; 0: behind the count readback)"},
     {"event_waits", "0|1: the host's mid-step waits use events behind the kernels instead of polled tag words"},
@@ -417,6 +418,7 @@
     }
     else if (k == "generic_depth_sort") ok = parse_flag(value, &ctx->knob_generic_depth_sort);
     else if (k == "dsort_splitters") ok = parse_flag(value, &ctx->knob_dsort_splitters);
+    else if (k == "dsort_k1_hist") ok = parse_flag(value, &ctx->knob_dsort_k1_hist);
     else if (k == "tile_sort") {
         const std::string v(value);
         if (v == "auto") { ctx->knob_tile_sort = 0; ok = true; }
@@ -681,6 +683,16 @@
     float4* spec_vc = nullptr;
     uint32_t *spec_tile_ids = nullptr, *spec_isect_gids = nullptr;
     if (n > 0) {
+        fused_scan = depth_sort_supported(n) && !ctx->knob_generic_depth_sort;
+        bool* spl_written = nullptr;
+        uint32_t* const spl = view_splitters(view, cut_active, &spl_written);
+        bool* const spl_valid = view ? &view->spl_valid[cut_active ? 1 : 0] : nullptr;
+        uint32_t* k1_table = nullptr;
+        if (fused_scan && ctx->knob_dsort_k1_hist && ctx->knob_dsort_splitters && spl && *spl_valid && n >= DSORT_K1_MIN_N) {
+            k1_table = (uint32_t*)ensure(ctx, SLOT_DSORT_K1, dsort_table_bytes(dsort_chunks(n)));
+            if (!k1_table) return BH_ERR_OOM;
+        }
+        if (spl_valid) *spl_valid = false;
         {
             ProfScope ps(ctx, "ProjectSplats");
             if (!ctx->counters_ready) BH_HIP(ctx, hipMemsetAsync(counter_pairs, 0, 2 * counter_set_bytes, ctx->stream));
@@ -718,13 +730,23 @@
                 prep.span_f4 = (uint32_t)(req.grad_floats / 4);
                 ctx->clears.k1_cleared_span();
             }
+            if (k1_table) {
+                const uint32_t chunks = dsort_chunks(n);
+                if (ctx->dsort_k1_zeroed != k1_table || ctx->dsort_k1_zeroed_chunks != chunks)
+                    BH_HIP(ctx, hipMemsetAsync(k1_table + dsort_hist_word(chunks), 0, (size_t)2 * 256 * chunks * 4, ctx->stream));
+                ctx->dsort_k1_zeroed = nullptr;
+                prep.ds_spl = spl;
+                prep.ds_hist = k1_table + dsort_hist_word(chunks);
+                prep.ds_csum = k1_table + dsort_csum_word(chunks);
+                prep.ds_digits = reinterpret_cast<uint8_t*>(k1_table + dsort_digits_word(chunks));
+                prep.ds_chunks = chunks;
+            }
             BH_TRY(launch_project_forward(ctx, u, n, mip, sh_degree, transforms, sh_coeffs, raw_opacities, depth_keys, isect_counts, max_radius,
                                           proj_by_gid, counters, prep, cut_active ? vtab : nullptr, near_counts));
             ctx->counter_phase ^= 1u;
             ctx->counters_ready = true;
         }
         auto* hslots = reinterpret_cast<unsigned long long*>(ctx->host_counters + 16);
-        fused_scan = depth_sort_supported(n) && !ctx->knob_generic_depth_sort;
         const bool sums_on_device = fused_scan && !ctx->knob_readback_copy;
         const bool poll_tag = sums_on_device && !ctx->knob_event_waits;
         if (!sums_on_device) {
@@ -737,11 +759,13 @@
                 cum_early = (uint32_t*)ensure(ctx, SLOT_CUM_TILES_HIT, npad * 4);
                 if (!cum_early) return BH_ERR_OOM;
                 if (poll_tag && ++ctx->readback_tag == 0u) ctx->readback_tag = 1u;
-                bool* spl_written = nullptr;
-                uint32_t* spl = view_splitters(view, cut_active, &spl_written);
                 BH_TRY(depth_sort_scan(ctx, depth_keys, counters + COUNTER_MINMAX_WORD, cut_active ? near_counts : isect_counts, n, depths_sorted, gfc, cum_early,
                                        sums_on_device ? counters : nullptr, ctx->host_counters + 16, ctx->readback_ev, poll_tag ? ctx->readback_tag : 0u,
-                                       sums_on_device ? dev_sums : nullptr, spl, spl_written));
+                                       sums_on_device ? dev_sums : nullptr, spl, spl_written, k1_table));
+                if (k1_table) {
+                    ctx->dsort_k1_zeroed = k1_table;
+                    ctx->dsort_k1_zeroed_chunks = dsort_chunks(n);
+                }
             } else {
                 BH_TRY(radix_argsort(ctx, depth_keys, nullptr, n, 32, depths_sorted, gfc));
             }
@@ -781,6 +805,7 @@
         ni = (uint32_t)hc[1];
         near_total = cut_active ? (uint32_t)hc[2] : ni;
         nv = cut_active ? (uint32_t)hc[3] : nv_true;
+        if (spl_valid) *spl_valid = fused_scan && ctx->knob_dsort_splitters && nv >= DSORT_SPL_MIN_KEYS;
     } else {
         BH_HIP(ctx, hipMemsetAsync(tile_offsets, 0, ((size_t)num_tiles * 2 + LPT_HEADER_WORDS) * 4, ctx->stream));
         if (visible_words) BH_HIP(ctx, hipMemsetAsync(visible, 0, visible_words * 4, ctx->stream));
diff --git a/brush_amd/csrc/context.h b/brush_amd/csrc/context.h
--- a/brush_amd/csrc/context.h
+++ b/brush_amd/csrc/context.h
@@ -11,6 +11,7 @@
 #include "../../include/brush_hip_lpips.h"
 #include "../../include/brush_hip_image.h"
 #include "device_math.h"
+#include "dsort_layout.h"
 
 namespace bh {
 
@@ -75,6 +76,7 @@
     SLOT_PLY_COMPRESS,
     SLOT_IMAGE,
     SLOT_DEPTH,
+    SLOT_DSORT_K1,
     SLOT_COUNT
 };
 
@@ -124,6 +126,7 @@
     uint32_t last_pairs = 0;
     uint32_t complete_frames = 0;
     bool spl_written[2] = {false, false};
+    bool spl_valid[2] = {false, false};
     bool casual = false;
 };
 constexpr uint32_t CUT_MIN_PAIRS = 1500000u;
@@ -151,6 +154,8 @@
 constexpr uint32_t BWD_CKPT_MAX_SLOTS = 96u * 1024u;
 constexpr uint32_t DSORT_SPL_STRIDE = 260;
 constexpr uint32_t VIEW_SPL_WORDS = 2 * DSORT_SPL_STRIDE;
+constexpr uint32_t DSORT_SPL_MIN_KEYS = 16384;
+constexpr uint32_t DSORT_K1_MIN_N = 1u << 17;
 constexpr size_t MAX_VIEW_STATES = 4096;
 constexpr uint64_t DIRECT_ALLREDUCE_MIN_FLOATS = 1u << 16;
 constexpr uint32_t AUTO_EXACT_FRAMES = 12;
@@ -335,6 +340,9 @@
     uint32_t* dsort_spl = nullptr;
     bool dsort_spl_written = false;
     bool knob_dsort_splitters = true;
+    bool knob_dsort_k1_hist = true;
+    const uint32_t* dsort_k1_zeroed = nullptr;
+    uint32_t dsort_k1_zeroed_chunks = 0;
     bool adam_lds_raised = false;
     bool knob_no_lpt = false;
     bool knob_bwd_jobs = true;
@@ -450,6 +458,11 @@
     uint32_t split_min = SPLIT_MIN_WORK;
     float split_of_max = 0.45f;
     bool list_all_visible = false;
+    const uint32_t* ds_spl = nullptr;
+    uint32_t* ds_hist = nullptr;
+    uint32_t* ds_csum = nullptr;
+    uint8_t* ds_digits = nullptr;
+    uint32_t ds_chunks = 0;
 };
 int launch_project_forward(bh_ctx* ctx, const ViewUniforms& u, uint32_t n, bool mip, uint32_t sh_degree, const float* transforms,
                            const float* sh, const float* raw_opac, uint32_t* depth_keys, uint32_t* isect_counts, float* max_radius,
@@ -477,7 +490,8 @@
 bool depth_sort_supported(uint32_t n);
 int depth_sort_scan(bh_ctx* ctx, const uint32_t* keys, const uint32_t* minmax, const uint32_t* counts, uint32_t n, uint32_t* out_keys,
                     uint32_t* out_vals, uint32_t* cum, const uint32_t* rb_set = nullptr, uint32_t* rb_host = nullptr, hipEvent_t rb_done = nullptr,
-                    uint32_t rb_tag = 0, uint32_t* rb_dev = nullptr, uint32_t* spl = nullptr, bool* spl_written = nullptr);
+                    uint32_t rb_tag = 0, uint32_t* rb_dev = nullptr, uint32_t* spl = nullptr, bool* spl_written = nullptr,
+                    uint32_t* k1_table = nullptr );
 int prefix_sum(bh_ctx* ctx, const uint32_t* in, const uint32_t* gather, uint32_t n, uint32_t* out, bool exclusive, const uint32_t* gate = nullptr);
 int launch_tile_offsets(bh_ctx* ctx, const uint32_t* tile_ids_sorted, uint32_t num_isect, uint32_t num_tiles,
                         uint32_t* tile_offsets, bool pre_zeroed = false);
diff --git a/brush_amd/csrc/depth_sort.hip b/brush_amd/csrc/depth_sort.hip
--- a/brush_amd/csrc/depth_sort.hip
+++ b/brush_amd/csrc/depth_sort.hip
@@ -10,6 +10,7 @@
 constexpr int DS_KPT = BH_DS_KPT;
 constexpr int DS_TILE = DS_WG * DS_KPT;
 constexpr int DS_RADIX = 256;
+static_assert((uint32_t)DS_TILE == DSORT_CHUNK, "K1 adds its blocks' histograms into the rows of these chunks (context.h DSORT_K1)");
 constexpr uint32_t CULLED_KEY = 0xFFFFFFFFu;
 
 struct DepthSplit {
@@ -20,7 +21,7 @@
 };
 constexpr uint32_t SPL_WORDS = 258;
 static_assert(SPL_WORDS <= DSORT_SPL_STRIDE, "context.h reserves the table");
-constexpr uint32_t SPL_MIN_KEYS = 16384;
+constexpr uint32_t SPL_MIN_KEYS = DSORT_SPL_MIN_KEYS;
 constexpr uint32_t SPL_SAMPLE_STRIDE = 64;
 constexpr uint32_t SPL_SAMPLE_MIN_N = 1u << 17;
 constexpr uint32_t SPL_SAMPLE_MIN_KEYS = 1024;
@@ -70,10 +71,7 @@
 BH_DEV uint32_t depth_digit(uint32_t key, const DepthSplit& sp) {
     if (key == CULLED_KEY) return 255u;
     if (sp.spl != nullptr) {
-        uint32_t d = 0;
-#pragma unroll
-        for (uint32_t step = 128u; step != 0u; step >>= 1) d += sp.spl[d + step - 1u] <= key ? step : 0u;
-        return d;
+        return dsort_splitter_digit(sp.spl, key);
     }
     return min(254u, (uint32_t)(((unsigned long long)(key - sp.kmin) * sp.scale) >> 32));
 }
@@ -177,9 +175,14 @@
 
 constexpr int DS_ROW_EPT = 16;
 __global__ __launch_bounds__(DS_WG) void dsort_rowscan_kernel(uint32_t* __restrict__ hist, const uint32_t* __restrict__ csum, uint32_t nblocks,
-                                                             uint32_t* __restrict__ digit_totals ) {
+                                                             uint32_t* __restrict__ digit_totals ,
+                                                             const uint32_t* __restrict__ rb_set, uint32_t* __restrict__ rb_host, uint32_t rb_tag, uint32_t* __restrict__ rb_dev) {
     const int tid = threadIdx.x, lane = tid & 63, wave = tid >> 6;
     const uint32_t d = blockIdx.x;
+    if (d == (uint32_t)DS_RADIX) {
+        if (wave == 0) counter_sums_to_host(rb_set, rb_host, tid, rb_tag, rb_dev);
+        return;
+    }
     uint32_t* row = hist + (size_t)d * nblocks;
     const uint32_t* crow = csum + (size_t)d * nblocks;
     uint32_t v[DS_ROW_EPT], incl[DS_ROW_EPT];
@@ -453,7 +456,9 @@
                                                             uint32_t* __restrict__ out_keys, uint32_t* __restrict__ out_vals,
                                                             const uint32_t* __restrict__ minmax, const uint32_t* __restrict__ digit_totals,
                                                             const uint32_t* __restrict__ counts, uint32_t* __restrict__ cum ,
-                                                            uint32_t* __restrict__ spl_out , uint32_t spl_min_keys) {
+                                                            uint32_t* __restrict__ spl_out , uint32_t spl_min_keys,
+                                                            uint32_t* __restrict__ zero_tab , uint32_t zero_words) {
+    for (uint32_t i = blockIdx.x * (uint32_t)BK_WG + threadIdx.x; i < zero_words; i += gridDim.x * (uint32_t)BK_WG) zero_tab[i] = 0u;
     extern __shared__ __attribute__((aligned(16))) uint32_t s_dyn[];
     __shared__ uint32_t s_base[DS_RADIX];
     __shared__ uint32_t s_hist[DS_RADIX];
@@ -658,17 +663,22 @@
 
 static int dsort_launches(bh_ctx* ctx, const uint32_t* keys, const uint32_t* minmax, const uint32_t* counts, uint32_t n, uint32_t* out_keys, uint32_t* out_vals,
                           uint32_t* cum, const uint32_t* rb_set, uint32_t* rb_host, hipEvent_t rb_done, uint32_t rb_tag, uint32_t* rb_dev, uint32_t* totals,
-                          uint32_t* a_keys, uint32_t* a_vals, const uint32_t* spl_in, uint32_t* spl_out, uint32_t spl_min_keys) {
-    const uint32_t nblocks = (n + DS_TILE - 1) / DS_TILE;
-    uint32_t* hist = totals + 2 * DS_RADIX;
-    uint32_t* csum = hist + (size_t)DS_RADIX * nblocks;
-    uint8_t* digits = reinterpret_cast<uint8_t*>(csum + (size_t)DS_RADIX * nblocks);
-    hipLaunchKernelGGL(dsort_hist_kernel, dim3(nblocks + (rb_set ? 1u : 0u)), dim3(DS_WG), 0, ctx->stream, keys, counts, n, nblocks, minmax, hist, csum,
-                       rb_set, rb_host, rb_tag, rb_dev, spl_in, digits);
-    BH_LAUNCH_CHECK(ctx, "dsort_hist_kernel");
-    if (rb_set && !rb_tag) BH_HIP(ctx, hipEventRecord(rb_done, ctx->stream));
-    hipLaunchKernelGGL(dsort_rowscan_kernel, dim3(DS_RADIX), dim3(DS_WG), 0, ctx->stream, hist, csum, nblocks, totals);
+                          uint32_t* a_keys, uint32_t* a_vals, const uint32_t* spl_in, uint32_t* spl_out, uint32_t spl_min_keys, bool by_k1 = false) {
+    const uint32_t nblocks = dsort_chunks(n);
+    uint32_t* hist = totals + dsort_hist_word(nblocks);
+    uint32_t* csum = totals + dsort_csum_word(nblocks);
+    uint8_t* digits = reinterpret_cast<uint8_t*>(totals + dsort_digits_word(nblocks));
+    if (!by_k1) {
+        hipLaunchKernelGGL(dsort_hist_kernel, dim3(nblocks + (rb_set ? 1u : 0u)), dim3(DS_WG), 0, ctx->stream, keys, counts, n, nblocks, minmax, hist, csum,
+                           rb_set, rb_host, rb_tag, rb_dev, spl_in, digits);
+        BH_LAUNCH_CHECK(ctx, "dsort_hist_kernel");
+        if (rb_set && !rb_tag) BH_HIP(ctx, hipEventRecord(rb_done, ctx->stream));
+    }
+    const uint32_t* no_set = nullptr;
+    hipLaunchKernelGGL(dsort_rowscan_kernel, dim3(DS_RADIX + (by_k1 && rb_set ? 1u : 0u)), dim3(DS_WG), 0, ctx->stream, hist, csum, nblocks, totals,
+                       by_k1 ? rb_set : no_set, rb_host, rb_tag, rb_dev);
     BH_LAUNCH_CHECK(ctx, "dsort_rowscan_kernel");
+    if (by_k1 && rb_set && !rb_tag) BH_HIP(ctx, hipEventRecord(rb_done, ctx->stream));
     hipLaunchKernelGGL(dsort_split_kernel, dim3(nblocks), dim3(DS_WG), 0, ctx->stream, keys, n, nblocks, hist, totals, a_keys, a_vals, out_keys, out_vals, digits);
     BH_LAUNCH_CHECK(ctx, "dsort_split_kernel");
     if (!ctx->dsort_lds_raised) {
@@ -676,14 +686,14 @@
         ctx->dsort_lds_raised = true;
     }
     hipLaunchKernelGGL(dsort_bucket_kernel, dim3(DS_RADIX - 1), dim3(BK_WG), FAST_LDS_WORDS * 4, ctx->stream, a_keys, a_vals, out_keys, out_vals, minmax, totals, counts, cum, spl_out,
-                       spl_min_keys);
+                       spl_min_keys, by_k1 ? hist : (uint32_t*)nullptr, by_k1 ? 2u * DS_RADIX * nblocks : 0u);
     BH_LAUNCH_CHECK(ctx, "dsort_bucket_kernel");
     return 0;
 }
 
 int depth_sort_scan(bh_ctx* ctx, const uint32_t* keys, const uint32_t* minmax, const uint32_t* counts, uint32_t n, uint32_t* out_keys,
                     uint32_t* out_vals, uint32_t* cum, const uint32_t* rb_set, uint32_t* rb_host, hipEvent_t rb_done, uint32_t rb_tag, uint32_t* rb_dev, uint32_t* spl,
-                    bool* spl_written) {
+                    bool* spl_written, uint32_t* k1_table) {
     if (n == 0) return 0;
     const uint32_t nblocks = (n + DS_TILE - 1) / DS_TILE;
     if (!ctx->knob_dsort_splitters) spl = nullptr;
@@ -696,10 +706,17 @@
         spl = ctx->dsort_spl;
         spl_written = &ctx->dsort_spl_written;
     }
-    uint32_t* totals = (uint32_t*)ensure(ctx, SLOT_SORT_HIST, ((size_t)2 * DS_RADIX * nblocks + 2 * DS_RADIX) * 4 + (size_t)nblocks * DS_TILE);
+    uint32_t* totals = (uint32_t*)ensure(ctx, SLOT_SORT_HIST, dsort_table_bytes(nblocks));
     uint32_t* a_keys = (uint32_t*)ensure(ctx, SLOT_SORT_KEYS_A, (size_t)n * 4);
     uint32_t* a_vals = (uint32_t*)ensure(ctx, SLOT_SORT_VALS_A, (size_t)n * 4);
     if (!totals || !a_keys || !a_vals) return BH_ERR_OOM;
+    if (k1_table) {
+        if (!spl) return set_error(ctx, BH_ERR_INVALID_ARG, "depth_sort_scan: K1's tables need the splitter table they were made with");
+        BH_TRY(dsort_launches(ctx, keys, minmax, counts, n, out_keys, out_vals, cum, rb_set, rb_host, rb_done, rb_tag, rb_dev, k1_table, a_keys, a_vals, spl, spl, SPL_MIN_KEYS,
+                              true));
+        if (spl_written) *spl_written = true;
+        return 0;
+    }
     if (spl && spl_written && !*spl_written && n >= SPL_SAMPLE_MIN_N) {
         const uint32_t m = n / SPL_SAMPLE_STRIDE;
         uint32_t* sample = (uint32_t*)ensure(ctx, SLOT_SORT_KEYS_B, (size_t)m * 4);
diff --git a/brush_amd/csrc/dsort_layout.h b/brush_amd/csrc/dsort_layout.h
--- /dev/null
+++ b/brush_amd/csrc/dsort_layout.h
@@ -0,0 +1,27 @@
+#pragma once
+#include <stddef.h>
+#include <stdint.h>
+
+
+namespace bh {
+
+constexpr uint32_t DSORT_CHUNK = 2048;
+constexpr uint32_t DSORT_K1_BLOCK = 256;
+constexpr uint32_t DSORT_CULLED_DIGIT = 255;
+static_assert(DSORT_CHUNK % DSORT_K1_BLOCK == 0, "whole K1 blocks per chunk: a block never straddles two columns");
+
+constexpr uint32_t dsort_splitter_digit(const uint32_t* spl, uint32_t key) {
+    uint32_t d = 0;
+    for (uint32_t step = 128u; step != 0u; step >>= 1) d += spl[d + step - 1u] <= key ? step : 0u;
+    return d < 254u ? d : 254u;
+}
+
+constexpr uint32_t dsort_chunks(uint32_t n) { return (n + DSORT_CHUNK - 1u) / DSORT_CHUNK; }
+constexpr uint32_t dsort_chunk_of_block(uint32_t block) { return block / (DSORT_CHUNK / DSORT_K1_BLOCK); }
+constexpr size_t dsort_table_at(uint32_t digit, uint32_t chunk, uint32_t chunks) { return (size_t)digit * chunks + chunk; }
+constexpr size_t dsort_hist_word(uint32_t) { return (size_t)2 * 256; }
+constexpr size_t dsort_csum_word(uint32_t chunks) { return (size_t)2 * 256 + (size_t)256 * chunks; }
+constexpr size_t dsort_digits_word(uint32_t chunks) { return (size_t)2 * 256 + (size_t)2 * 256 * chunks; }
+constexpr size_t dsort_table_bytes(uint32_t chunks) { return dsort_digits_word(chunks) * 4 + (size_t)chunks * DSORT_CHUNK; }
+
+}
diff --git a/brush_amd/csrc/project.hip b/brush_amd/csrc/project.hip
--- a/brush_amd/csrc/project.hip
+++ b/brush_amd/csrc/project.hip
@@ -204,9 +204,13 @@
     __shared__ uint32_t s_listed[PROJ_WAVES];
     __shared__ uint32_t s_kmax[PROJ_WAVES];
     __shared__ uint32_t s_nmax[PROJ_WAVES];
+    __shared__ uint32_t s_bins[ORDER_BINS];
+    static_assert(ORDER_BINS >= 3 * 256 && PROJ_WG == 256 && (uint32_t)PROJ_WG == DSORT_K1_BLOCK, "s_bins holds 256 splitters, 256 key counts and 256 tile-count sums");
+    uint32_t* const s_dspl = s_bins;
+    uint32_t* const s_dhist = s_bins + 256;
+    uint32_t* const s_dcsum = s_bins + 512;
     const uint32_t gid = blockIdx.x * PROJ_WG + threadIdx.x;
     if (prep.order_out && blockIdx.x < 8u) {
-        __shared__ uint32_t s_bins[ORDER_BINS];
         const uint32_t per = band_slots(prep.order_tiles);
         __shared__ uint32_t s_band_work, s_band_cnt, s_band_tail, s_band_max;
         for (uint32_t i = threadIdx.x; i < ORDER_BINS; i += PROJ_WG) s_bins[i] = 0u;
@@ -276,6 +280,11 @@
     if (gid < prep.slice_words) prep.slice_table[gid] = 0u;
     if (gid < COUNTER_SET_U64 && prep.next_counters) prep.next_counters[gid] = 0ull;
     for (size_t i = gid; i < prep.span_f4; i += (size_t)gridDim.x * PROJ_WG) prep.span[i] = make_float4(0.0f, 0.0f, 0.0f, 0.0f);
+    if (prep.ds_hist) {
+        s_dspl[threadIdx.x] = prep.ds_spl[threadIdx.x];
+        s_dhist[threadIdx.x] = 0u;
+        s_dcsum[threadIdx.x] = 0u;
+    }
     const int lane = threadIdx.x & 63, wave = threadIdx.x >> 6;
     uint32_t key = 0xFFFFFFFFu;
     float radius = 0.0f;
@@ -374,6 +383,16 @@
         max_radius[gid] = radius;
         if (zcut) near_counts[gid] = near_hit;
     }
+    if (prep.ds_hist) {
+        __syncthreads();
+        uint32_t d = 255u;
+        if (listed) {
+            d = dsort_splitter_digit(s_dspl, key);
+            atomicAdd(&s_dhist[d], 1u);
+            atomicAdd(&s_dcsum[d], zcut ? near_hit : tiles_hit);
+        }
+        if (gid < n) prep.ds_digits[gid] = (uint8_t)d;
+    }
     const unsigned long long ball = __ballot(visible);
     const unsigned long long lball = __ballot(listed);
     uint32_t wave_hits = tiles_hit;
@@ -414,6 +433,15 @@
             uint32_t* mm = reinterpret_cast<uint32_t*>(counters) + COUNTER_MINMAX_WORD + 2u * sl;
             atomicMax(&mm[0], km);
             atomicMax(&mm[1], nm);
+        }
+    }
+    if (prep.ds_hist) {
+        const uint32_t c = s_dhist[threadIdx.x];
+        if (c) {
+            const size_t at = dsort_table_at(threadIdx.x, dsort_chunk_of_block(blockIdx.x), prep.ds_chunks);
+            atomicAdd(&prep.ds_hist[at], c);
+            const uint32_t t = s_dcsum[threadIdx.x];
+            if (t) atomicAdd(&prep.ds_csum[at], t);
         }
     }
 }
```
